# nebarnix/Project-Desert-Tortoise

Hardware: AMD Instinct MI355X
Metric: IQ Msamples/s end-to-end (WAV→minorframes), 1-GPU + %HBM roofline (higher is better)
Workload: dtype f32

## Files before the change

include/pdt_dev.h:

```cpp
#ifndef PDT_DEV_H
#define PDT_DEV_H
#include <stdint.h>
#ifdef __cplusplus
extern "C" {
#endif
int pdt_dev_set(const char *name, const char *value);
struct pdt_ctx;
unsigned long long pdt_dev_span_rows(const struct pdt_ctx *ctx, unsigned *n_exits_out, unsigned long long max);
int pdt_dev_ddc(int device, uint32_t in_rate, int decim, double offset_hz, int sample_format, const void *x_dev, long long lo, long long hi,
                uint64_t n_out, uint64_t g0, void *out_dev);
#ifdef __cplusplus
}
#endif
#endif
```

project-desert-tortoise_amd/__init__.py:

```python
from __future__ import annotations

import collections
import ctypes as C
import os
import struct

import numpy as np

_HERE = os.path.dirname(os.path.abspath(__file__))
LIBPDT_PATH = os.environ.get("PDT_LIBPDT_PATH") or os.path.join(_HERE, "csrc", "libpdt.so")
LIBSYNTH_PATH = os.path.join(_HERE, "synth", "libpdtsynth.so")

MODE_POES, MODE_ARGOS = 0, 1
SAMPLER_GARDNER, SAMPLER_MM = 0, 1
CHAIN_FILE, CHAIN_LIVE = 0, 1
ST_PLL, ST_LOCK, ST_FIR, ST_AGC, ST_SYM, ST_SYMIDX, ST_BITS, ST_BITSYM, ST_AGC_RAW, ST_ANALYTIC, ST_CHANNEL = range(11)
FMT_PCM16, FMT_F32, FMT_REAL_PCM16, FMT_REAL_F32 = range(4)


FMT_WB_PCM16, FMT_WB_F32, FMT_WB_CU8, FMT_WB_CS8 = range(16, 20)


class PdtError(RuntimeError):
    pass
# ... 247 lines not shown


def _argos_cfg(min_run, rule=None):
    if min_run is None and rule is None:
        return None
    c = ArgosCfg(rule=int(rule or 0))
    if min_run is not None:
        c.min_run, c.zero_mask = int(min_run), ARGOS_ZERO_MIN_RUN if int(min_run) == 0 else 0
    return c


def argos_run_len(msgs):
    return np.asarray(msgs["reserved_"]) & 0xFF


def argos_slip(msgs):
    return (np.asarray(msgs["reserved_"]) >> 8) & 1


def _bit_string(bits) -> np.ndarray:
    if isinstance(bits, (bytes, bytearray)):
        return np.frombuffer(bytes(bits), dtype=np.uint8)
    return np.ascontiguousarray(bits, dtype=np.uint8).reshape(-1)


def argos_msg_tile() -> int:
    return lib().pdt_argos_msg_tile()


def host_argos_messages(bits, min_run=None, cap: int = 4096, with_count: bool = False, rule=None):
    a, c = _bit_string(bits), _argos_cfg(min_run, rule)
    out, count = np.zeros(max(cap, 1), dtype=ARGOS_MSG_DTYPE), C.c_int(0)
    _check(lib().pdt_host_argos_messages(a.ctypes.data, a.size, C.byref(c) if c else None, out.ctypes.data, cap, C.byref(count)),
           "pdt_host_argos_messages")
    got = out[:min(count.value, cap)]
    return (got, count.value) if with_count else got


def argos_messages_batch(ds, min_run=None, cap: int = 4096, rule=None):
    c = _argos_cfg(min_run, rule)
    hs = (C.c_void_p * max(len(ds), 1))(*[d._h for d in ds])
    out, counts = np.zeros((max(len(ds), 1), max(cap, 1)), dtype=ARGOS_MSG_DTYPE), (C.c_int * max(len(ds), 1))()
    _check(lib().pdt_argos_messages_batch(hs, len(ds), C.byref(c) if c else None, out.ctypes.data, cap, counts),
           "pdt_argos_messages_batch")
    return [out[i, :min(counts[i], cap)].copy() for i in range(len(ds))]


class FfCfg(C.Structure):
    _fields_ = [("rate_steps", C.c_int32), ("zero_mask", C.c_uint32), ("rate_step_ppm", C.c_double), ("residual_hz", C.c_double),
                ("flags", C.c_uint32), ("reserved_", C.c_uint32)]


class FfSync(C.Structure):
    _fields_ = [("residual_hz", C.c_double), ("tone_valid", C.c_int32), ("step", C.c_uint32), ("tau", C.c_int32), ("rate", C.c_int32),
                ("period", C.c_int64), ("metric", C.c_uint64), ("nbits", C.c_uint64)]


FF_ZERO_RATE_STEPS, FF_RESIDUAL_GIVEN = 1, 1
FF_SYNC_DTYPE = np.dtype([("residual_hz", "<f8"), ("tone_valid", "<i4"), ("step", "<u4"), ("tau", "<i4"), ("rate", "<i4"), ("period", "<i8"),
                          ("metric", "<u8"), ("nbits", "<u8")])
assert FF_SYNC_DTYPE.itemsize == C.sizeof(FfSync) == 48 and C.sizeof(FfCfg) == 32
FfBits = collections.namedtuple("FfBits", "sync bits soft index")


def _ff_cfg(rate_steps=None, rate_step_ppm=None, residual_hz=None):
    if rate_steps is None and rate_step_ppm is None and residual_hz is None:
        return None
    c = FfCfg()
    if rate_steps is not None:
        c.rate_steps, c.zero_mask = int(rate_steps), FF_ZERO_RATE_STEPS if int(rate_steps) == 0 else 0
    if rate_step_ppm is not None:
        c.rate_step_ppm = float(rate_step_ppm)
    if residual_hz is not None:
        c.residual_hz, c.flags = float(residual_hz), FF_RESIDUAL_GIVEN
    return c


def ff_max_bits(rate: int, n: int) -> int:
    return min(n, 2 * rate) * 800 // (rate * 18 // 10) + 2 if rate >= 800 else 2


def host_ff_mix(rate: int, residual_hz: float, iq: np.ndarray) -> np.ndarray:
    a = np.ascontiguousarray(iq, dtype="<f4").reshape(-1)
    out = np.zeros(max(a.size, 2), dtype="<f4")
    _check(lib().pdt_host_ff_mix(rate, float(residual_hz), a.ctypes.data, a.size // 2, out.ctypes.data), "pdt_host_ff_mix")
    return out[:a.size // 2 * 2].reshape(-1, 2)


def host_ff_bits(rate: int, iq: np.ndarray, rate_steps=None, rate_step_ppm=None, residual_hz=None) -> FfBits:
    a = np.ascontiguousarray(iq, dtype="<f4").reshape(-1)
    c, n = _ff_cfg(rate_steps, rate_step_ppm, residual_hz), a.size // 2
    cap = ff_max_bits(rate, n)
    sync, count = np.zeros(1, dtype=FF_SYNC_DTYPE), C.c_uint64(0)
    bits, soft, index = np.zeros(cap, dtype=np.uint8), np.zeros(cap, dtype="<f4"), np.zeros(cap, dtype="<i8")
    _check(lib().pdt_host_ff_bits(rate, a.ctypes.data, n, C.byref(c) if c else None, sync.ctypes.data, bits.ctypes.data, soft.ctypes.data,
                                  index.ctypes.data, cap, C.byref(count)), "pdt_host_ff_bits")
    k = min(count.value, cap)
    return FfBits(sync[0], bits[:k], soft[:k], index[:k])


def ff_bits_batch(ds, rate_steps=None, rate_step_ppm=None, residual_hz=None) -> np.ndarray:
    c = _ff_cfg(rate_steps, rate_step_ppm, residual_hz)
    hs = (C.c_void_p * max(len(ds), 1))(*[d._h for d in ds])
    syncs = np.zeros(max(len(ds), 1), dtype=FF_SYNC_DTYPE)
    _check(lib().pdt_ff_bits_batch(hs, len(ds), C.byref(c) if c else None, syncs.ctypes.data), "pdt_ff_bits_batch")
    return syncs[:len(ds)]


def ff_messages_batch(ds, min_run=None, cap: int = 64, rule=None, rate_steps=None, rate_step_ppm=None, residual_hz=None, with_sync: bool = False):
    c, a = _ff_cfg(rate_steps, rate_step_ppm, residual_hz), _argos_cfg(min_run, rule)
    hs = (C.c_void_p * max(len(ds), 1))(*[d._h for d in ds])
    syncs = np.zeros(max(len(ds), 1), dtype=FF_SYNC_DTYPE)
    out, counts = np.zeros((max(len(ds), 1), max(cap, 1)), dtype=ARGOS_MSG_DTYPE), (C.c_int * max(len(ds), 1))()
    _check(lib().pdt_ff_messages_batch(hs, len(ds), C.byref(c) if c else None, C.byref(a) if a else None, syncs.ctypes.data, out.ctypes.data, cap,
                                       counts), "pdt_ff_messages_batch")
    got = [out[i, :min(counts[i], cap)].copy() for i in range(len(ds))]
    return (got, syncs[:len(ds)]) if with_sync else got


def format_argos_messages(msgs: np.ndarray) -> bytes:
    a = np.ascontiguousarray(msgs, dtype=ARGOS_MSG_DTYPE)
    L = lib()
    n = L.pdt_format_argos_messages(a.ctypes.data, len(a), None, 0)
    buf = C.create_string_buffer(n + 1)
    L.pdt_format_argos_messages(a.ctypes.data, len(a), buf, n)
    return buf.raw[:n]


def _carriers(rec, count: int):
    return [Carrier(rec[i].offset_hz, rec[i].peak_db, rec[i].floor_power) for i in range(count)]


ABI_SYMBOLS = [
    "pdt_abi_version", "pdt_build_tag", "pdt_strerror", "pdt_device_count", "pdt_open", "pdt_close", "pdt_set_stream",
    "pdt_demod_pcm16", "pdt_demod_device", "pdt_demod_f32", "pdt_demod_device_f32", "pdt_demod_batch_device", "pdt_num_frames", "pdt_frames", "pdt_get_stats",
    "pdt_format_frames", "pdt_read_stage", "pdt_stage_len", "pdt_kernel_times", "pdt_make_lpf",
    "pdt_wav_parse_header", "pdt_time_axis", "pdt_stage_bytesync", "pdt_tip_check", "pdt_tip_frames",
    "pdt_stream_begin", "pdt_stream_push_pcm16", "pdt_stream_push_f32", "pdt_stream_end", "pdt_stream_frames",
    "pdt_keep_quality", "pdt_chunk_reports", "pdt_stage_manchester", "pdt_stage_fir", "pdt_stage_agc", "pdt_stage_squelch", "pdt_stage_pll", "pdt_stage_gardner", "pdt_stage_static_gain", "pdt_stage_mm",
    "pdt_keep_presquelch", "pdt_keep_pll", "pdt_stage_bytesync_from", "pdt_demod_fd", "pdt_format_records", "pdt_stream_retained", "pdt_host_math", "pdt_get_device",
    "pdt_write_frames", "pdt_write_records", "pdt_demod_file", "pdt_set_loop_params", "pdt_set_progress",
    "pdt_set_real_input", "pdt_demod_real", "pdt_demod_device_real", "pdt_stream_push_real", "pdt_host_analytic",
    "pdt_set_channel", "pdt_demod_channel", "pdt_demod_device_channel", "pdt_demod_channels_device", "pdt_demod_channels", "pdt_stream_push_channel", "pdt_host_ddc",
    "pdt_survey", "pdt_survey_device", "pdt_survey_spectrum", "pdt_host_survey",
    "pdt_bursts", "pdt_bursts_device", "pdt_burst_carriers", "pdt_waterfall_rows", "pdt_bursts_shape", "pdt_burst_peaks", "pdt_host_bursts",
    "pdt_device_math", "pdt_device_math_layout",
    "pdt_burst_windows", "pdt_demod_windows_device", "pdt_demod_windows", "pdt_demod_windows_held",
    "pdt_tones", "pdt_tones_batch", "pdt_host_tones",
    "pdt_argos_messages", "pdt_argos_messages_batch", "pdt_stage_argos_messages", "pdt_host_argos_messages", "pdt_argos_msg_tile",
    "pdt_format_argos_messages", "pdt_write_argos_messages",
    "pdt_ff_bits", "pdt_ff_bits_batch", "pdt_ff_read", "pdt_ff_messages", "pdt_ff_messages_batch", "pdt_stage_ff_bits", "pdt_host_ff_bits",
    "pdt_host_ff_mix",
]
DEV_SYMBOLS = ["pdt_dev_set", "pdt_dev_span_rows", "pdt_dev_ddc"]

_lib = None


def _share_torch_hip_runtime():
    import importlib.util
    import sys
    if "torch" in sys.modules:
        return
    try:
        spec = importlib.util.find_spec("torch")
    except (ImportError, ValueError):
        return
    if spec is None or not spec.submodule_search_locations:
        return
    path = os.path.join(list(spec.submodule_search_locations)[0], "lib", "libamdhip64.so")
    if os.path.exists(path):
        try:
            C.CDLL(path, mode=C.RTLD_GLOBAL)
        except OSError:
            pass


def lib():
    global _lib
    if _lib is not None:
        return _lib
    if not os.path.exists(LIBPDT_PATH):
        raise PdtError(
            f"{LIBPDT_PATH} is missing: build it with `make` (hipcc --offload-arch=gfx950). "
            "There is no CPU implementation to fall back to."
        )
    _share_torch_hip_runtime()
    L = C.CDLL(LIBPDT_PATH)
    L.pdt_abi_version.restype = C.c_int
    L.pdt_build_tag.restype = C.c_char_p
    L.pdt_strerror.restype = C.c_char_p
    L.pdt_strerror.argtypes = [C.c_int]
    L.pdt_device_count.restype = C.c_int
    L.pdt_open.argtypes = [C.POINTER(Config), C.POINTER(C.c_void_p)]
    L.pdt_close.argtypes = [C.c_void_p]
    L.pdt_close.restype = None
    L.pdt_set_stream.argtypes = [C.c_void_p, C.c_void_p]
    L.pdt_demod_pcm16.argtypes = [C.c_void_p, C.c_void_p, C.c_uint64]
    L.pdt_demod_device.argtypes = [C.c_void_p, C.c_void_p, C.c_uint64]
    L.pdt_demod_f32.argtypes = [C.c_void_p, C.c_void_p, C.c_uint64]
    L.pdt_demod_device_f32.argtypes = [C.c_void_p, C.c_void_p, C.c_uint64]
    L.pdt_demod_fd.argtypes = [C.c_void_p, C.c_int, C.c_uint64, C.c_uint64, C.c_int]
    L.pdt_format_records.argtypes = [C.c_void_p, C.c_uint64, C.c_char_p, C.c_uint64]
    L.pdt_format_records.restype = C.c_uint64
    L.pdt_num_frames.argtypes = [C.c_void_p]
    L.pdt_num_frames.restype = C.c_uint64
    L.pdt_frames.argtypes = [C.c_void_p, C.POINTER(Frame), C.c_uint64]
    L.pdt_frames.restype = C.c_uint64
    L.pdt_get_stats.argtypes = [C.c_void_p, C.POINTER(Stats)]
    L.pdt_format_frames.argtypes = [C.c_void_p, C.c_char_p, C.c_uint64]
    L.pdt_format_frames.restype = C.c_uint64
    L.pdt_read_stage.argtypes = [C.c_void_p, C.c_int, C.c_uint64, C.c_uint64, C.c_void_p]
    L.pdt_read_stage.restype = C.c_int64
    L.pdt_stage_len.argtypes = [C.c_void_p, C.c_int]
    L.pdt_stage_len.restype = C.c_uint64
    L.pdt_kernel_times.argtypes = [C.c_void_p, C.POINTER(KernelTime), C.c_int]
    L.pdt_make_lpf.argtypes = [C.c_int, C.c_uint32, C.c_void_p, C.POINTER(C.c_int), C.POINTER(C.c_int)]
    L.pdt_wav_parse_header.argtypes = [C.c_char_p] + [C.POINTER(C.c_uint32)] * 5
    L.pdt_time_axis.argtypes = [C.c_int, C.c_uint32, C.c_uint64]
    L.pdt_time_axis.restype = C.c_double
    L.pdt_stage_bytesync.argtypes = [C.c_void_p, C.c_void_p, C.c_uint64]
    L.pdt_demod_batch_device.argtypes = [C.POINTER(C.c_void_p), C.POINTER(C.c_void_p), C.POINTER(C.c_uint64), C.c_int]
    L.pdt_stream_begin.argtypes = [C.c_void_p]
    L.pdt_stream_push_pcm16.argtypes = [C.c_void_p, C.c_void_p, C.c_uint64, C.POINTER(C.c_uint64)]
    L.pdt_stream_push_f32.argtypes = [C.c_void_p, C.c_void_p, C.c_uint64, C.POINTER(C.c_uint64)]
    L.pdt_stream_end.argtypes = [C.c_void_p, C.POINTER(C.c_uint64)]
    L.pdt_stream_frames.argtypes = [C.c_void_p, C.c_void_p, C.c_uint64]
    L.pdt_stream_frames.restype = C.c_uint64
    L.pdt_host_math.argtypes = [C.c_int, C.c_void_p, C.c_uint64, C.c_void_p, C.c_void_p]
    L.pdt_stream_retained.argtypes = [C.c_void_p]
    L.pdt_stream_retained.restype = C.c_uint64
    L.pdt_stage_manchester.argtypes = [C.c_void_p, C.c_void_p, C.c_uint64, C.c_double, C.c_void_p, C.c_void_p, C.c_void_p, C.c_void_p]
    L.pdt_stage_manchester.restype = C.c_int
    L.pdt_stage_pll.argtypes = [C.c_void_p, C.c_void_p, C.c_uint64, C.c_int, C.c_void_p, C.c_void_p, C.c_void_p, C.c_void_p]
    L.pdt_stage_pll.restype = C.c_int
    L.pdt_stage_gardner.argtypes = [C.c_void_p, C.c_void_p, C.c_uint64, C.c_uint64, C.c_void_p, C.c_void_p, C.c_void_p, C.c_void_p,
                                    C.c_void_p]
    L.pdt_stage_gardner.restype = C.c_int
    L.pdt_stage_static_gain.argtypes = [C.c_void_p, C.c_void_p, C.c_uint64, C.c_int, C.c_double, C.c_void_p]
    L.pdt_stage_static_gain.restype = C.c_int
    L.pdt_stage_mm.argtypes = [C.c_void_p, C.c_void_p, C.c_uint64, C.c_void_p, C.c_void_p, C.c_void_p, C.c_void_p]
    L.pdt_stage_mm.restype = C.c_int
    L.pdt_stage_agc.argtypes = [C.c_void_p, C.c_void_p, C.c_uint64, C.c_double, C.c_double, C.c_double, C.c_void_p]
    L.pdt_stage_agc.restype = C.c_int
    L.pdt_stage_squelch.argtypes = [C.c_void_p, C.c_void_p, C.c_void_p, C.c_uint64, C.c_double]
    L.pdt_stage_squelch.restype = C.c_int
    L.pdt_stage_fir.argtypes = [C.c_void_p, C.c_void_p, C.c_uint64, C.c_void_p, C.c_void_p]
    L.pdt_stage_fir.restype = C.c_int
    L.pdt_keep_quality.argtypes = [C.c_void_p, C.c_int]
    L.pdt_keep_quality.restype = C.c_int
    L.pdt_keep_pll.argtypes = [C.c_void_p, C.c_int]
    L.pdt_keep_pll.restype = C.c_int
    L.pdt_chunk_reports.argtypes = [C.c_void_p, C.c_void_p, C.c_uint64]
    L.pdt_chunk_reports.restype = C.c_uint64
    L.pdt_set_progress.argtypes = [C.c_void_p, C.c_void_p, C.c_void_p]
    L.pdt_tip_check.argtypes = [C.c_void_p, C.POINTER(TipSummary)]
    L.pdt_tip_frames.argtypes = [C.c_void_p, C.c_void_p, C.c_uint64]
    L.pdt_tip_frames.restype = C.c_uint64
    L.pdt_write_frames.argtypes = [C.c_void_p, C.c_int, C.POINTER(C.c_uint64)]
    L.pdt_write_records.argtypes = [C.c_void_p, C.c_uint64, C.c_int, C.POINTER(C.c_uint64)]
    L.pdt_dev_set.argtypes = [C.c_char_p, C.c_char_p]
    L.pdt_set_loop_params.argtypes = [C.c_void_p, C.POINTER(LoopParams)]
    L.pdt_demod_file.argtypes = [C.c_void_p, C.c_int, C.c_uint64, C.c_uint64, C.c_int, C.c_int, C.POINTER(C.c_uint64)]
    L.pdt_set_real_input.argtypes = [C.c_void_p, C.c_double]
    L.pdt_demod_real.argtypes = [C.c_void_p, C.c_void_p, C.c_uint64, C.c_int]
    L.pdt_demod_device_real.argtypes = [C.c_void_p, C.c_void_p, C.c_uint64, C.c_int]
    L.pdt_stream_push_real.argtypes = [C.c_void_p, C.c_void_p, C.c_uint64, C.c_int, C.POINTER(C.c_uint64)]
    L.pdt_host_analytic.argtypes = [C.c_uint32, C.c_double, C.c_void_p, C.c_uint64, C.c_int, C.c_void_p]
    L.pdt_set_channel.argtypes = [C.c_void_p, C.c_int, C.c_double]
    L.pdt_demod_channel.argtypes = [C.c_void_p, C.c_void_p, C.c_uint64, C.c_int]
    L.pdt_demod_device_channel.argtypes = [C.c_void_p, C.c_void_p, C.c_uint64, C.c_int]
    L.pdt_demod_channels_device.argtypes = [C.POINTER(C.c_void_p), C.c_int, C.c_void_p, C.c_uint64, C.c_int]
    L.pdt_demod_channels.argtypes = [C.POINTER(C.c_void_p), C.c_int, C.c_void_p, C.c_uint64, C.c_int]
    L.pdt_stream_push_channel.argtypes = [C.c_void_p, C.c_void_p, C.c_uint64, C.c_int, C.POINTER(C.c_uint64)]
    L.pdt_host_ddc.argtypes = [C.c_uint32, C.c_int, C.c_double, C.c_void_p, C.c_uint64, C.c_int, C.c_void_p]
    L.pdt_dev_ddc.argtypes = [C.c_int, C.c_uint32, C.c_int, C.c_double, C.c_int, C.c_void_p, C.c_longlong, C.c_longlong, C.c_uint64, C.c_uint64, C.c_void_p]
    L.pdt_survey.argtypes = [C.c_void_p, C.c_void_p, C.c_uint64, C.c_int, C.POINTER(SurveyCfg), C.POINTER(CarrierRec), C.c_int, C.POINTER(C.c_int)]
    L.pdt_survey_device.argtypes = L.pdt_survey.argtypes
    L.pdt_survey_spectrum.argtypes = [C.c_void_p, C.c_void_p, C.c_int]
    L.pdt_bursts.argtypes = [C.c_void_p, C.c_void_p, C.c_uint64, C.c_int, C.POINTER(BurstsCfg), C.POINTER(BurstRec), C.c_int, C.POINTER(C.c_int)]
    L.pdt_bursts_device.argtypes = L.pdt_bursts.argtypes
    L.pdt_burst_carriers.argtypes = [C.POINTER(BurstRec), C.c_int, C.c_double, C.POINTER(CarrierRec), C.c_int, C.POINTER(C.c_int)]
    L.pdt_waterfall_rows.argtypes = [C.c_void_p, C.c_uint64, C.c_uint64, C.c_void_p]
    L.pdt_bursts_shape.argtypes = [C.c_void_p, C.POINTER(C.c_int), C.POINTER(C.c_int), C.POINTER(C.c_uint64)]
    L.pdt_burst_peaks.argtypes = [C.c_void_p, C.c_uint64, C.c_uint64, C.c_void_p, C.c_void_p]
    L.pdt_host_bursts.argtypes = [C.c_uint32, C.c_double, C.c_uint32, C.c_int, C.c_void_p, C.c_uint64, C.POINTER(BurstsCfg), C.c_void_p, C.c_void_p,
                                  C.c_void_p, C.POINTER(BurstRec), C.c_int, C.POINTER(C.c_int)]
    L.pdt_host_survey.argtypes = [C.c_uint32, C.c_double, C.c_uint32, C.c_int, C.c_void_p, C.c_uint64, C.POINTER(SurveyCfg), C.c_void_p,
                                  C.POINTER(CarrierRec), C.c_int, C.POINTER(C.c_int)]
    L.pdt_burst_windows.argtypes = [C.POINTER(BurstRec), C.c_int, C.c_uint32, C.c_uint64, C.c_double, C.c_double, C.POINTER(WindowRec)]
    L.pdt_demod_windows_device.argtypes = [C.POINTER(C.c_void_p), C.c_int, C.POINTER(WindowRec), C.c_void_p, C.c_uint64, C.c_int]
    L.pdt_demod_windows.argtypes = L.pdt_demod_windows_device.argtypes
    L.pdt_demod_windows_held.argtypes = [C.c_void_p, C.POINTER(C.c_void_p), C.c_int, C.POINTER(WindowRec)]
    L.pdt_tones.argtypes = [C.c_void_p, C.POINTER(ToneCfg), C.c_void_p, C.c_int, C.POINTER(C.c_int)]
    L.pdt_tones_batch.argtypes = [C.POINTER(C.c_void_p), C.c_int, C.POINTER(ToneCfg), C.c_void_p, C.c_int, C.POINTER(C.c_int)]
    L.pdt_host_tones.argtypes = [C.c_uint32, C.c_double, C.c_void_p, C.c_uint64, C.POINTER(ToneCfg), C.c_void_p, C.c_int, C.POINTER(C.c_int)]
    L.pdt_argos_messages.argtypes = [C.c_void_p, C.POINTER(ArgosCfg), C.c_void_p, C.c_int, C.POINTER(C.c_int)]
    L.pdt_argos_messages_batch.argtypes = [C.POINTER(C.c_void_p), C.c_int, C.POINTER(ArgosCfg), C.c_void_p, C.c_int, C.POINTER(C.c_int)]
    L.pdt_stage_argos_messages.argtypes = [C.c_void_p, C.c_void_p, C.c_uint64, C.POINTER(ArgosCfg), C.c_void_p, C.c_int, C.POINTER(C.c_int)]
    L.pdt_host_argos_messages.argtypes = [C.c_void_p, C.c_uint64, C.POINTER(ArgosCfg), C.c_void_p, C.c_int, C.POINTER(C.c_int)]
    L.pdt_format_argos_messages.argtypes = [C.c_void_p, C.c_uint64, C.c_char_p, C.c_uint64]
    L.pdt_format_argos_messages.restype = C.c_uint64
    L.pdt_write_argos_messages.argtypes = [C.c_void_p, C.c_uint64, C.c_int, C.POINTER(C.c_uint64)]
    L.pdt_ff_bits.argtypes = [C.c_void_p, C.POINTER(FfCfg), C.c_void_p]
    L.pdt_ff_bits_batch.argtypes = [C.POINTER(C.c_void_p), C.c_int, C.POINTER(FfCfg), C.c_void_p]
    L.pdt_ff_read.argtypes = [C.c_void_p, C.c_void_p, C.c_void_p, C.c_void_p, C.c_void_p, C.c_uint64, C.POINTER(C.c_uint64)]
    L.pdt_ff_messages.argtypes = [C.c_void_p, C.POINTER(FfCfg), C.POINTER(ArgosCfg), C.c_void_p, C.c_void_p, C.c_int, C.POINTER(C.c_int)]
# ... 712 lines not shown
```

project-desert-tortoise_amd/csrc/pdt_api.hip:

```cpp
#include "pdt_rt.h"
#include "pdt_analytic.h"
#include "pdt_ddc.h"
#include "pdt_survey.h"
#include "pdt_bursts.h"
#include "pdt_tone.h"
#include "pdt_argos_msg.h"
#include "pdt_ff.h"

#include <sys/stat.h>

namespace pdtrt {
PDT_CHAIN_INSTANCES(extern, float)
PDT_CHAIN_INSTANCES(extern, double)
std::atomic<long long> g_alloc_ns{0};
hipError_t analytic_launch(hipStream_t st, int fmt, const void *x, long long lo, long long hi, unsigned long long n_out, unsigned long long g0,
                           uint32_t step, const float *tab_dev, void *out);
size_t survey_part_floats(uint64_t nseg, int nfft);
hipError_t survey_launch(hipStream_t st, int fmt, const void *x, uint64_t nseg, int nfft, const float *win, const float *tw, float *part, float *out);
int survey_plan(const pdt_survey_cfg *cfg, double mode_range_hz, double channel_rate, uint64_t nframes, int cap, pdt::SurveyPlan *p);
int survey_carriers(const float *P, const pdt::SurveyPlan &p, double in_rate, pdt_carrier *found);
hipError_t waterfall_launch(hipStream_t st, int fmt, const void *x, uint64_t nrows, int rows_per, int nfft, const float *win, const float *tw, float *rows);
hipError_t row_peaks_launch(hipStream_t st, const float *rows, uint64_t nrows, int nfft, float level, int gb, void *peaks, int *counts);
int bursts_plan(const pdt_bursts_cfg *cfg, double mode_range_hz, double channel_rate, double in_rate, uint64_t nframes, int cap, pdt::BurstPlan *p);
pdt::SurveyPlan bursts_survey_plan(const pdt::BurstPlan &p, const pdt_bursts_cfg *cfg, uint64_t nframes);
int bursts_link(const void *peaks, const int *counts, bool compact, const pdt::BurstPlan &p, double floor, double in_rate, pdt_burst *found, int cap);
hipError_t tones_launch(hipStream_t st, int nfft, const void *segs_dev, uint64_t nsegs, int lo, int hi, const float *win, const float *tw, void *out);
int tone_plan(const pdt_tone_cfg *cfg, double fs, double range_hz, uint64_t len, int cap, pdt::TonePlan *p);
void tone_sums(int nfft, double *sw, double *sw2);
void tones_derive(const void *raw, const pdt::TonePlan &p, double fs, double offset_hz, double sw, double sw2, pdt_tone *out);
hipError_t argos_msgs_launch(hipStream_t st, const void *table_dev, int nctx, long long tiles, int K, int rule, hipEvent_t mid);
int argos_min_run(const pdt_argos_cfg *cfg, int *K, int *rule);
hipError_t ff_launch(hipStream_t st, const void *table_dev, int nwin, long long mix_tiles, long long groups, const long long *periods_dev, int R,
                     int H, long long pmax, const float *tab_dev, void *metric_dev, size_t metric_bytes, void *syncs_dev, hipEvent_t *ev);
int ff_plan(const pdt_ff_cfg *cfg, uint32_t rate, int *H, int *R, double *ppm, int *given, double *residual);
long long ddc_windows_table(int decim, pdt::DdcWindow *win, int count, std::vector<unsigned char> &table);
hipError_t ddc_windows_launch(hipStream_t st, int fmt, int decim, const float *taps_dev, const float *tab_dev, const void *table_dev, int count,
                              long long tiles);
hipError_t ddc_launch(hipStream_t st, int fmt, int decim, const float *taps_dev, const float *tab_dev, pdt::DdcWindow w);
}

static std::mutex g_dev_mu;
static std::map<std::string, std::string> g_dev;
void Tuning::load()
{
    std::lock_guard<std::mutex> lock(g_dev_mu);
    if (g_dev.empty()) return;
    auto get = [&](const char *n) -> const char * { auto it = g_dev.find(n); return it == g_dev.end() ? nullptr : it->second.c_str(); };
    if (const char *e = get("PDT_PLL_WARM_SCALE")) pll_warm_scale = atof(e);
    if (const char *e = get("PDT_HEAD_TAUS")) head_taus = atof(e);
    if (const char *e = get("PDT_BAND_PAD")) band_pad = atof(e);
    if (const char *e = get("PDT_PLL_WARM_S")) pll_warm_s = atof(e);
    if (const char *e = get("PDT_AGC_WARM_S")) agc_warm_s = atof(e);
    if (const char *e = get("PDT_AGC_K")) agc_k = atof(e);
    if (const char *e = get("PDT_AGC_TPB")) agc_tpb = std::max(1, atoi(e));
    if (const char *e = get("PDT_PLL_BLOCK")) pll_block = atoi(e);
    if (const char *e = get("PDT_HBM_LIMIT_MB")) hbm_limit_mb = std::max(1ll, atoll(e));
    if (const char *e = get("PDT_BURST_SLAB_ROWS")) burst_slab_rows = std::max(1ll, atoll(e));
    if (const char *e = get("PDT_WINDOW_PIECE")) window_piece = std::max(1ll, atoll(e));
    if (const char *e = get("PDT_SCOUT_SYMS")) scout_syms = std::max(16, atoi(e));
    if (const char *e = get("PDT_FIR_WG_PER_CU")) fir_wg_per_cu = std::min(4096, std::max(1, atoi(e)));
    if (const char *e = get("PDT_INGEST_THREADS")) ingest_threads = std::min(128, std::max(1, atoi(e)));
    if (const char *e = get("PDT_INGEST_SPAN_MB")) ingest_span_mb = std::min(256, std::max(1, atoi(e)));
    if (const char *e = get("PDT_INGEST_STREAMS")) ingest_streams = std::min(4, std::max(1, atoi(e)));
    if (const char *e = get("PDT_INGEST_DIRECT")) ingest_direct = atoi(e) ? 1 : 0;
    if (const char *e = get("PDT_INGEST_NUMA")) ingest_numa = atoi(e) ? 1 : 0;
    if (const char *e = get("PDT_FIX_PASSES")) fix_passes = atoi(e);
    if (const char *e = get("PDT_GSEG")) gseg = std::min(64, std::max(2, atoi(e)));
    if (const char *e = get("PDT_GSPAN")) gspan = std::min(256, std::max(1, atoi(e)));
    if (const char *e = get("PDT_GSPAN_CAP")) gspan_cap = std::max(64, atoi(e));
    fir_generic = get("PDT_FIR_GENERIC") != nullptr;
    mix_unfused = get("PDT_MIX_UNFUSED") != nullptr;
    quality_inline = get("PDT_QUALITY_INLINE") != nullptr;
    gardner_nostride = get("PDT_GARDNER_NOSTRIDE") != nullptr;
    gemit_groups = get("PDT_GEMIT_GROUPS") != nullptr;
    agc_unfused = get("PDT_AGC_UNFUSED") != nullptr;
    manch_3pass = get("PDT_MANCH_3PASS") != nullptr;
    sync_serial = get("PDT_SYNC_SERIAL") != nullptr;
    agc_lanes = get("PDT_AGC_LANES") != nullptr;
    no_excl = get("PDT_NO_EXCL") != nullptr;
    gardner_onebuf = get("PDT_GARDNER_ONEBUF") != nullptr;
    gardner_noring = get("PDT_GARDNER_NORING") != nullptr;
    ema_noguess = get("PDT_EMA_NOGUESS") != nullptr;
    gardner_sequential = get("PDT_GARDNER_SEQUENTIAL") != nullptr;
    seg_sequential = get("PDT_SEG_SEQUENTIAL") != nullptr;
    overlap = get("PDT_NO_OVERLAP") == nullptr;
    if (const char *e = get("PDT_OVERLAP_SPLIT")) {
        int k = 0;
        for (const char *q = e; *q && k < 8; k++) {
            char *end = nullptr;
            overlap_split[k] = strtod(q, &end);
            if (end == q) break;
            q = (*end == ',') ? end + 1 : end;
        }
    }
    chain_one_range = get("PDT_CHAIN_ONE_RANGE") != nullptr;
    debug_overlap = get("PDT_DEBUG_OVERLAP") != nullptr;
    if (const char *e = get("PDT_OVERLAP_SEGMENTS")) overlap_segments = std::min(64, std::max(1, atoi(e)));
    if (const char *e = get("PDT_OVERLAP_MIN_MB")) overlap_min_mb = std::min(1 << 20, std::max(1, atoi(e)));
    debug_sync = get("PDT_DEBUG_SYNC") != nullptr;
    pll_noshort = get("PDT_PLL_NOSHORT") != nullptr;
    pll_nockpt = get("PDT_PLL_NOCKPT") != nullptr;
    pll_noconsensus = get("PDT_PLL_NOCONSENSUS") != nullptr;
    pll_notail = get("PDT_PLL_NOTAIL") != nullptr;
    seg_plain = get("PDT_SEG_PLAIN") != nullptr;
    sync_block = get("PDT_SYNC_BLOCK") != nullptr;
}

namespace pdtrt {

int execute_plans(pdt_ctx *const *ctxs, int M)
{
    pdt_ctx *L0 = ctxs[0];
    HIP_TRY(hipSetDevice(L0->cfg.device));
    const Plan &P0 = L0->plan;
    for (int m = 1; m < M; m++)
        if (!P0.same_shape(ctxs[m]->plan)) return PDT_ERR_STATE;
    const size_t per = P0.packs.size();
    const size_t total = per * (size_t)M;
    int rc;
    if ((rc = L0->packs_dev.ensure(total + 64))) return rc;
    if (total + 64 > L0->packs_pin_cap) {
        if (L0->packs_pin) (void)hipHostFree(L0->packs_pin);
        L0->packs_pin = nullptr;
        L0->packs_pin_cap = 0;
        const size_t want = 2 * total + 4096;
        if (timed_host_malloc((void **)&L0->packs_pin, want) != hipSuccess) { (void)hipGetLastError(); return PDT_ERR_NOMEM; }
        L0->packs_pin_cap = want;
    }
    unsigned char *pin = (unsigned char *)L0->packs_pin;
    for (const PlanOp &o : P0.ops) {
        if (o.op != OP_LAUNCH) continue;
        for (int m = 0; m < M; m++)
            memcpy(pin + (size_t)M * o.pack_off + (size_t)m * o.pack_size, ctxs[m]->plan.packs.data() + o.pack_off, o.pack_size);
    }
    hipStream_t st[2] = { L0->stream, L0->stream2 };
    if (total) HIP_TRY(hipMemcpyAsync(L0->packs_dev.p, pin, total, hipMemcpyHostToDevice, st[0]));
    Launcher T(L0);
    const unsigned char *dev = (const unsigned char *)L0->packs_dev.p;
    for (size_t i = 0; i < P0.ops.size(); i++) {
        const PlanOp &o = P0.ops[i];
        switch (o.op) {
        case OP_LAUNCH: {
            dim3 g = o.grid;
            for (int m = 1; m < M; m++) {
                const dim3 gm = ctxs[m]->plan.ops[i].grid;
                g.x = std::max(g.x, gm.x);
                g.y = std::max(g.y, gm.y);
            }
            g.z = (unsigned)M;
            o.go(g, o.block, o.shmem, st[o.side], dev + (size_t)M * o.pack_off);
            if (L0->tune.debug_sync) {
                const hipError_t e = hipStreamSynchronize(st[o.side]);
                fprintf(stderr, "libpdt: [%zu] %s grid (%u,%u,%u) block %u lds %zu: %s\n", i, o.name, g.x, g.y, g.z, o.block.x, o.shmem,
                        hipGetErrorString(e));
            }
            break;
        }
        case OP_MEMSET:
            for (int m = 0; m < M; m++) {
                const PlanOp &om = ctxs[m]->plan.ops[i];
                if (om.bytes) HIP_TRY(hipMemsetAsync(om.dst, om.value, om.bytes, st[om.side]));
            }
            T.gap();
            break;
        case OP_D2H:
        case OP_H2D:
            for (int m = 0; m < M; m++) {
                const PlanOp &om = ctxs[m]->plan.ops[i];
                if (om.bytes)
                    HIP_TRY(hipMemcpyAsync(om.dst, om.src, om.bytes, o.op == OP_D2H ? hipMemcpyDeviceToHost : hipMemcpyHostToDevice, st[0]));
            }
            T.gap();
            break;
        case OP_FORK:
            HIP_TRY(hipEventRecord(L0->ev_fork, st[0]));
            HIP_TRY(hipStreamWaitEvent(st[1], L0->ev_fork, 0));
            break;
        case OP_JOIN_RECORD: HIP_TRY(hipEventRecord(L0->ev_join, st[1])); break;
        case OP_JOIN_WAIT: HIP_TRY(hipStreamWaitEvent(st[0], L0->ev_join, 0)); break;
        case OP_TBEGIN: T.begin(o.name, st[o.side]); break;
        case OP_TEND: T.end(); break;
        case OP_TGAP: T.gap(); break;
        case OP_EV0: HIP_TRY(hipEventRecord(L0->ev0, st[0])); break;
        case OP_EV1: HIP_TRY(hipEventRecord(L0->ev1, st[0])); break;
        }
    }
    HIP_TRY(hipGetLastError());
    for (int m = 0; m < M; m++) ctxs[m]->leader = L0;
    return PDT_OK;
}

void launch_bytesync(pdt_ctx *ctx, Plan &PL, hipStream_t st, const SyncParams &SP, DevScalars *d_sc, long long bit_cap, uint32_t hit_cap,
                     uint32_t frame_cap, long long min_pos)
{
    unsigned char *d_bits = (unsigned char *)ctx->bits.p;
    unsigned *d_bitsym = (unsigned *)ctx->bitsym.p;
    long long *d_symidx = (long long *)ctx->symidx.p;
    unsigned *d_hits = (unsigned *)ctx->hits.p;
    FrameRec *d_frames = (FrameRec *)ctx->frames.p;
    const long long n_stiles = (bit_cap + 4095) / 4096;
    SyncTile *d_stiles = (SyncTile *)ctx->stiles.p;
    PDT_LAUNCH(256, k_sync_hits_tile, dim3((unsigned)n_stiles), dim3(256), 0, st, d_bits, &d_sc->nbits, SP, d_stiles,
                       &d_sc->sync_overflow, min_pos);
    unsigned *d_scr = (unsigned *)ctx->sync_scr.p;
    if (ctx->tune.sync_serial) {
        PDT_LAUNCH(PDT_SYNC_THREADS, k_sync_frames_tiles, dim3(1), dim3(PDT_SYNC_THREADS), 0, st, (const SyncTile *)d_stiles, &d_sc->nbits, SP, d_hits,
                           hit_cap, d_frames, &d_sc->nframes, frame_cap, &d_sc->sync_overflow, d_scr);
    } else {
        const unsigned n_batch = (unsigned)std::min<long long>(256, ((long long)hit_cap + PDT_SYNC_PB - 1) / PDT_SYNC_PB);
        PDT_LAUNCH(PDT_SYNC_THREADS, k_sync_dense, dim3(1), dim3(PDT_SYNC_THREADS), 0, st, (const SyncTile *)d_stiles, &d_sc->nbits, n_stiles,
                           hit_cap, &d_sc->sync_overflow, d_scr);
        PDT_LAUNCH(256, k_sync_gather, dim3((unsigned)std::min<long long>(1024, (n_stiles + 255) / 256)), dim3(256), 0, st,
                           (const SyncTile *)d_stiles, &d_sc->nbits, n_stiles, d_hits, hit_cap, &d_sc->sync_overflow, (const unsigned *)d_scr);
        PDT_LAUNCH(PDT_SYNC_PT, k_sync_links, dim3(n_batch), dim3(PDT_SYNC_PT), 0, st, SP, (const unsigned *)d_hits, &d_sc->sync_overflow, d_scr,
                           hit_cap);
        PDT_LAUNCH(PDT_SYNC_PT, k_sync_mark, dim3(n_batch), dim3(PDT_SYNC_PT), 0, st, SP, (const unsigned *)d_hits, d_frames, &d_sc->nframes,
                           frame_cap, &d_sc->sync_overflow, (const unsigned *)d_scr, hit_cap);
    }
    const long long grid = std::min<long long>(2048, (bit_cap + 255) / 256);
    PDT_LAUNCH(256, k_sync_hits, dim3((unsigned)grid), dim3(256), 0, st, d_bits, &d_sc->nbits, SP, d_hits, &d_sc->nhits, hit_cap,
                       &d_sc->sync_overflow, min_pos);
    PDT_LAUNCH(256, k_sync_frames, dim3(1), dim3(256), 0, st, d_hits, &d_sc->nhits, hit_cap, SP, d_frames, &d_sc->nframes,
                       frame_cap, &d_sc->sync_overflow);
    PDT_LAUNCH(128, k_frame_pack, dim3(std::min<uint32_t>(frame_cap, 16384)), dim3(128), 0, st, d_bits, &d_sc->nbits, d_bitsym, d_symidx, SP,
                       d_frames, &d_sc->nframes, frame_cap);
}

void chunk_reports_range(const pdt_ctx *ctx, uint64_t c0, uint64_t c1, uint64_t total, pdt_chunk_report *out, const pdt_frame *open_frame)
{
    const bool argos = ctx->cfg.mode == PDT_MODE_ARGOS;
    const uint64_t chunk = ctx->cfg.chunk;
    uint64_t sym_prev = c0 ? ctx->chunk_host[(size_t)c0 - 1].sym_upto : 0, bits_prev = c0 ? ctx->chunk_host[(size_t)c0 - 1].bits_upto : 0;
    size_t f = 0;
    if (c0) {
        size_t lo = 0, hi = ctx->frames_host.size();
        while (lo < hi) {
            const size_t mid = (lo + hi) / 2;
            if ((uint64_t)ctx->frames_host[mid].bit_index < bits_prev) lo = mid + 1; else hi = mid;
        }
        f = lo;
    }
    for (uint64_t c = c0; c < c1; c++) {
        const pdt::ChunkInfo &ci = ctx->chunk_host[(size_t)c];
        pdt_chunk_report &o = out[c - c0];
        memset(&o, 0, sizeof o);
        o.samples = std::min<uint64_t>(chunk, total - c * chunk);
        o.avg_phase = ci.avg_phase;
        o.symbols = ci.sym_upto - sym_prev;
        o.bits = ci.bits_upto - bits_prev;
        while (f < ctx->frames_host.size() && (uint64_t)ctx->frames_host[f].bit_index < ci.bits_upto) { o.frames++; f++; }
        if (open_frame && (uint64_t)open_frame->bit_index >= bits_prev && (uint64_t)open_frame->bit_index < ci.bits_upto) o.frames++;
        o.time0 = (argos && ctx->elem == 8) ? const_cast<pdt_ctx *>(ctx)->axis_d.at((uint64_t)ci.t0_src + 1)
                  : argos ? (double)const_cast<pdt_ctx *>(ctx)->axis_f.at((uint64_t)ci.t0_src + 1)
                          : (double)const_cast<pdt_ctx *>(ctx)->axis_f.at(c * chunk + 1);
        sym_prev = ci.sym_upto;
        bits_prev = ci.bits_upto;
    }
}


}

extern "C" {

int pdt_abi_version(void) { return PDT_ABI_VERSION; }
#ifndef PDT_BUILD_TAG
#define PDT_BUILD_TAG "untagged"
#endif
const char *pdt_build_tag(void) { return PDT_BUILD_TAG; }

int pdt_dev_set(const char *name, const char *value)
{
    try {
        std::lock_guard<std::mutex> lock(g_dev_mu);
        if (!name) g_dev.clear();
        else if (!value) g_dev.erase(name);
        else g_dev[name] = value;
    } catch (const std::exception &) { return PDT_ERR_NOMEM; }
    return PDT_OK;
}

unsigned long long pdt_dev_span_rows(const pdt_ctx *ctx, unsigned *n_exits_out, unsigned long long max)
{
    if (!ctx || ctx->gspan_nrows <= 0 || !ctx->gspan_rows.p) return 0;
    const unsigned long long n = (unsigned long long)ctx->gspan_nrows, m = std::min(n, max);
    if (n_exits_out && m) {
        std::vector<GardnerSpanRow> rows((size_t)m);
        if (hipSetDevice(ctx->cfg.device) != hipSuccess ||
            hipMemcpy(rows.data(), ctx->gspan_rows.p, (size_t)m * sizeof(GardnerSpanRow), hipMemcpyDeviceToHost) != hipSuccess) {
            (void)hipGetLastError();
            return 0;
        }
        for (size_t k = 0; k < (size_t)m; k++) n_exits_out[k] = rows[k].n;
    }
    return n;
}

int pdt_dev_ddc(int device, uint32_t in_rate, int decim, double offset_hz, int sample_format, const void *x_dev, long long lo, long long hi,
                uint64_t n_out, uint64_t g0, void *out_dev)
{
    if (in_rate == 0 || decim < DDC_MIN_DECIM || decim > DDC_MAX_DECIM || !ddc_fmt(sample_format) || !x_dev || !out_dev) return PDT_ERR_ARG;
    if (!(std::isfinite(offset_hz) && std::fabs(offset_hz) < 0.5 * (double)in_rate)) return PDT_ERR_ARG;
    HIP_TRY(hipSetDevice(device));
    const std::vector<float> taps = ddc_taps(decim);
    std::vector<float> tab(2 * AN_TAB);
    analytic_table(tab.data());
    DevBuf dtaps, dtab;
    auto run = [&]() -> int {
        int rc;
        if ((rc = dtaps.ensure(taps.size() * sizeof(float) + 16)) || (rc = dtab.ensure(tab.size() * sizeof(float) + 16))) return rc;
        HIP_TRY(hipMemcpy(dtaps.p, taps.data(), taps.size() * sizeof(float), hipMemcpyHostToDevice));
        HIP_TRY(hipMemcpy(dtab.p, tab.data(), tab.size() * sizeof(float), hipMemcpyHostToDevice));
        const DdcWindow r = { x_dev, out_dev, lo, hi, (long long)n_out, ddc_step((double)in_rate, offset_hz), (uint32_t)g0, 0 };
        HIP_TRY(ddc_launch(nullptr, sample_format, decim, (const float *)dtaps.p, (const float *)dtab.p, r));
        HIP_TRY(hipStreamSynchronize(nullptr));
        return PDT_OK;
    };
    const int rc = run();
    dtaps.release();
    dtab.release();
    return rc;
}

const char *pdt_strerror(int code)
{
    switch (code) {
    case PDT_OK: return "ok";
    case PDT_ERR_ARG: return "bad argument";
    case PDT_ERR_NOGPU: return "no usable HIP device / HIP runtime error";
    case PDT_ERR_NOMEM: return "out of device memory";
    case PDT_ERR_FORMAT: return "unsupported WAV format (need 16-bit PCM, 2 channels)";
    case PDT_ERR_RATE: return "sample rate too high: interpolation factor would be 0";
    case PDT_ERR_STATE: return "call sequence / internal capacity error";
    case PDT_ERR_IO: return "read error on the capture file";
    default: return "unknown error";
    }
}

int pdt_get_device(const pdt_ctx *ctx) { return ctx ? ctx->cfg.device : -1; }

int pdt_device_count(void)
{
    int n = 0;
    if (hipGetDeviceCount(&n) != hipSuccess) {
        (void)hipGetLastError();
        return 0;
    }
    return n;
}

int pdt_host_math(int fn, const double *x, uint64_t n, double *out0, double *out1)
{
    if (!x || !out0) return PDT_ERR_ARG;
    for (uint64_t i = 0; i < n; i++) {
        switch (fn) {
        case 0: { double sv, cv; sincos_glibc(x[i], sv, cv); out0[i] = sv; if (out1) out1[i] = cv; break; }
        case 1: out0[i] = sin_glibc(x[i]); break;
        case 2: out0[i] = cos_glibc(x[i]); break;
        case 3: { float sf, cf; sincosf_glibc((float)x[i], sf, cf); out0[i] = sf; if (out1) out1[i] = cf; break; }
        case 4: out0[i] = hypot_glibc(x[2 * i], x[2 * i + 1]); break;
        case 5: out0[i] = hypotf_glibc((float)x[2 * i], (float)x[2 * i + 1]); break;
        case 6: { float sf, cf; sincosf_flat((float)x[i], sf, cf); out0[i] = sf; if (out1) out1[i] = cf; break; }
        case 7: out0[i] = pll_wrap_error_f32((float)x[i]); break;
        case 8: out0[i] = pll_wrap_phase_f32((float)x[i]); break;
        case 9: { const float v = (float)x[i]; out0[i] = ((double)v > M_PI) ? (float)((double)v - 2 * M_PI) : ((double)v < -M_PI) ? (float)((double)v + 2 * M_PI) : v; break; }
        case 10: out0[i] = (x[i] > M_PI) ? x[i] - 2 * M_PI : (x[i] < -M_PI) ? x[i] + 2 * M_PI : x[i]; break;
        case 11: out0[i] = arctan2_ref((float)x[2 * i], (float)x[2 * i + 1]); break;
        case 12: out0[i] = arctan2_ref(x[2 * i], x[2 * i + 1]); break;
        case 13: out0[i] = q_rsqrt((float)x[i]); break;
        default: return PDT_ERR_ARG;
        }
    }
    return PDT_OK;
}

int pdt_make_lpf(int mode, uint32_t sample_rate, void *taps_out, int *ntaps, int *interp)
{
    if (!sample_rate) return PDT_ERR_ARG;
    if (mode == PDT_MODE_ARGOS) {
        if (ntaps) *ntaps = 50;
        if (interp) *interp = 1;
        if (taps_out) make_lpf<double>((double *)taps_out, 50, 700.0, (double)sample_rate, 1);
        return PDT_OK;
    }
    const int ip = poes_interp(sample_rate);
    if (ip < 1) return PDT_ERR_RATE;
    const int N = 26 * ip;
    if (ntaps) *ntaps = N;
    if (interp) *interp = ip;
    if (taps_out) {
        const float Fs = (float)sample_rate;
        make_lpf<float>((float *)taps_out, N, (float)11000.0, Fs * (float)ip, ip);
    }
    return PDT_OK;
}

int pdt_wav_parse_header(const uint8_t h[44], uint32_t *sample_rate, uint32_t *channels, uint32_t *bits_per_sample,
                         uint32_t *format, uint32_t *data_bytes)
{
    if (!h) return PDT_ERR_ARG;
    auto r32 = [&](int o) { return (uint32_t)h[o] | ((uint32_t)h[o + 1] << 8) | ((uint32_t)h[o + 2] << 16) | ((uint32_t)h[o + 3] << 24); };
    auto r16 = [&](int o) { return (uint32_t)h[o] | ((uint32_t)h[o + 1] << 8); };
    if (format) *format = r16(20);
    if (channels) *channels = r16(22);
    if (sample_rate) *sample_rate = r32(24);
    if (bits_per_sample) *bits_per_sample = r16(34);
    if (data_bytes) *data_bytes = r32(40);
    return PDT_OK;
}

double pdt_time_axis(int mode, uint32_t sample_rate, uint64_t m)
{
    if (mode == PDT_MODE_ARGOS) {
        TimeAxis<double> ax;
        ax.init(1.0 / (double)sample_rate);
        return ax.at(m);
    }
    TimeAxis<float> ax;
    ax.init((float)(1.0 / (double)(float)sample_rate));
    return (double)ax.at(m);
}

int pdt_open(const pdt_config *cfg, pdt_ctx **out)
{
    if (!cfg || !out) return PDT_ERR_ARG;
    if (cfg->mode != PDT_MODE_POES && cfg->mode != PDT_MODE_ARGOS) return PDT_ERR_ARG;
    if (!cfg->sample_rate) return PDT_ERR_ARG;
    if (cfg->chain != PDT_CHAIN_FILE && cfg->chain != PDT_CHAIN_LIVE) return PDT_ERR_ARG;
    int ndev = 0;
    if (hipGetDeviceCount(&ndev) != hipSuccess || ndev <= 0) {
        (void)hipGetLastError();
        fprintf(stderr, "libpdt: no HIP device available -- this library has no CPU path\n");
        return PDT_ERR_NOGPU;
    }
    if (cfg->device < 0 || cfg->device >= ndev) return PDT_ERR_ARG;
    HIP_TRY(hipSetDevice(cfg->device));
    pdt_ctx *ctx = new pdt_ctx();
    ctx->cfg = *cfg;
    ctx->tune.load();
    if (ctx->tune.pll_block && !ctx->cfg.pll_block) ctx->cfg.pll_block = (uint32_t)ctx->tune.pll_block;
    if (ctx->tune.pll_warm_s > 0 && !ctx->cfg.pll_warm) ctx->cfg.pll_warm = (uint32_t)(ctx->tune.pll_warm_s * cfg->sample_rate);
    if (ctx->tune.agc_warm_s > 0 && !ctx->cfg.agc_warm) ctx->cfg.agc_warm = (uint32_t)(ctx->tune.agc_warm_s * cfg->sample_rate);
    if (!ctx->cfg.chunk) ctx->cfg.chunk = (cfg->mode == PDT_MODE_ARGOS || cfg->chain == PDT_CHAIN_LIVE) ? 2400 : 10000;
    const bool argos_twin = cfg->mode == PDT_MODE_ARGOS && cfg->chain == PDT_CHAIN_LIVE;
    ctx->elem = (int)((cfg->mode == PDT_MODE_ARGOS && !argos_twin) ? sizeof(double) : sizeof(float));
    int nt = 0, ip = 0;
    int rc = pdt_make_lpf(cfg->mode, cfg->sample_rate, nullptr, &nt, &ip);
    if (rc) { pdt_close(ctx); return rc; }
    ctx->interp = (uint32_t)ip;
    ctx->ntaps = (uint32_t)nt;
    ctx->taps_host.resize((size_t)nt * ctx->elem);
    if (argos_twin)
        make_lpf<float>((float *)ctx->taps_host.data(), 50, (float)700, (float)cfg->sample_rate, 1);
    else
    pdt_make_lpf(cfg->mode, cfg->sample_rate, ctx->taps_host.data(), nullptr, nullptr);
    if ((rc = ctx->taps.ensure(ctx->taps_host.size()))) { pdt_close(ctx); return rc; }
    if (hipMemcpy(ctx->taps.p, ctx->taps_host.data(), ctx->taps_host.size(), hipMemcpyHostToDevice) != hipSuccess) {
        pdt_close(ctx);
        return PDT_ERR_NOGPU;
    }
    if (cfg->mode == PDT_MODE_POES && nt == 26 * ip) {
        const int K = 26, rs = ip;
        const int cs = (K * rs + 15) & ~15;
        std::vector<float> rot((size_t)K * cs, 0.0f);
        const float *h = (const float *)ctx->taps_host.data();
        for (int c = 0; c < K; c++)
            for (int t = 0; t < K; t++)
                for (int r = 0; r < ip; r++) rot[(size_t)c * cs + (size_t)t * rs + r] = h[nt - 1 - r - ((c - t + K) % K) * ip];
        if ((rc = ctx->taps_rot.ensure(rot.size() * sizeof(float)))) { pdt_close(ctx); return rc; }
        if (hipMemcpy(ctx->taps_rot.p, rot.data(), rot.size() * sizeof(float), hipMemcpyHostToDevice) != hipSuccess) {
            pdt_close(ctx);
            return PDT_ERR_NOGPU;
        }
    }
    std::thread side_stream_task;
    auto make_side_stream = [ctx]() {
        if (hipSetDevice(ctx->cfg.device) != hipSuccess) { (void)hipGetLastError(); return; }
        int least = 0, greatest = 0;
        (void)hipDeviceGetStreamPriorityRange(&least, &greatest);
        if (hipStreamCreateWithPriority(&ctx->stream2, hipStreamNonBlocking, greatest) != hipSuccess) {
            (void)hipGetLastError();
            if (hipStreamCreateWithFlags(&ctx->stream2, hipStreamNonBlocking) != hipSuccess) { (void)hipGetLastError(); ctx->stream2 = nullptr; }
        }
    };
    try { side_stream_task = std::thread(make_side_stream); } catch (const std::exception &) { make_side_stream(); }
    auto join_side = [&]() { if (side_stream_task.joinable()) side_stream_task.join(); };
    if (hipStreamCreate(&ctx->stream) != hipSuccess) { ctx->stream = nullptr; join_side(); pdt_close(ctx); return PDT_ERR_NOGPU; }
    ctx->own_stream = true;
    {
        void *small = nullptr;
        if (timed_host_malloc((void **)&small, sizeof(DevScalars) + 128 + 32768) != hipSuccess) { join_side(); pdt_close(ctx); return PDT_ERR_NOMEM; }
        ctx->pend_sc = (DevScalars *)small;
        ctx->pend_info = (unsigned char *)small + ((sizeof(DevScalars) + 15) & ~(size_t)15);
        ctx->seg_pin = ctx->pend_info + 128;
    }
    (void)hipEventCreate(&ctx->ev0);
    (void)hipEventCreate(&ctx->ev1);
    (void)hipEventCreateWithFlags(&ctx->ev_fork, hipEventDisableTiming);
    (void)hipEventCreateWithFlags(&ctx->ev_join, hipEventDisableTiming);
    join_side();
    if (!ctx->stream2) { pdt_close(ctx); return PDT_ERR_NOGPU; }
    memset(&ctx->stats, 0, sizeof ctx->stats);
    memset(ctx->stage_len, 0, sizeof ctx->stage_len);
    ctx->axis_f.init((float)(1.0 / (double)(float)cfg->sample_rate));
    if (argos_twin) ctx->axis_f.init(1 / (float)cfg->sample_rate);
    ctx->axis_d.init(1.0 / (double)cfg->sample_rate);
    ctx->counted = true;
    ingest_open_contexts().fetch_add(1);
    *out = ctx;
    return PDT_OK;
}

void pdt_close(pdt_ctx *ctx)
{
    if (!ctx) return;
    (void)hipSetDevice(ctx->cfg.device);
    DevBuf *bufs[] = { &ctx->pcm, &ctx->pll, &ctx->lock, &ctx->fir, &ctx->agc, &ctx->sym, &ctx->symidx, &ctx->bits, &ctx->bitsym,
                       &ctx->hits, &ctx->frames, &ctx->taps, &ctx->mag, &ctx->seams_pll, &ctx->seams_agc, &ctx->scal, &ctx->lockinfo,
                       &ctx->term, &ctx->seams_ema, &ctx->gtable, &ctx->gentries, &ctx->gcand,
                       &ctx->gmfirst, &ctx->stiles, &ctx->gsegmap, &ctx->gsegstart, &ctx->gbands, &ctx->gclist, &ctx->gspan_keys, &ctx->gspan_tails, &ctx->gspan_rows, &ctx->gspan_items, &ctx->gspan_ctl, &ctx->gspan_recs, &ctx->gcentries, &ctx->gflags, &ctx->agc_maps, &ctx->pll_head, &ctx->taps_rot, &ctx->pll_scratch, &ctx->tip, &ctx->stream_in, &ctx->sync_scr, &ctx->agc_raw, &ctx->agc_ckpt, &ctx->pll_ckpt, &ctx->packs_dev, &ctx->seg_dev, &ctx->lt_theta, &ctx->lt_phi,
                       &ctx->avgph, &ctx->term_ap, &ctx->seams_q, &ctx->chunkinfo, &ctx->an_tab, &ctx->analytic, &ctx->halo.buf[0], &ctx->halo.buf[1],
                       &ctx->ddc_taps, &ctx->channel, &ctx->survey_win, &ctx->survey_tw, &ctx->survey_part, &ctx->survey_out,
                       &ctx->bursts_rows, &ctx->bursts_peaks, &ctx->bursts_counts, &ctx->win_table, &ctx->tone_table, &ctx->tone_out,
                       &ctx->argos_work, &ctx->argos_bits, &ctx->ff_work, &ctx->ff_in, &ctx->ff_out };
    for (DevBuf *b : bufs) b->release();
    for (hipEvent_t e : ctx->event_pool) (void)hipEventDestroy(e);
    if (ctx->pinned) (void)hipHostFree(ctx->pinned);
    if (ctx->qual_pin) (void)hipHostFree(ctx->qual_pin);
    if (ctx->packs_pin) (void)hipHostFree(ctx->packs_pin);
    ctx->ingest.release();
    if (ctx->pend_sc) (void)hipHostFree(ctx->pend_sc);
    for (auto &t : ctx->timers) { if (!t.shared_a) (void)hipEventDestroy(t.a); (void)hipEventDestroy(t.b); }
    if (ctx->ev0) (void)hipEventDestroy(ctx->ev0);
    if (ctx->ev1) (void)hipEventDestroy(ctx->ev1);
    if (ctx->ev_fork) (void)hipEventDestroy(ctx->ev_fork);
    if (ctx->ev_join) (void)hipEventDestroy(ctx->ev_join);
    if (ctx->stream2) (void)hipStreamDestroy(ctx->stream2);
    if (ctx->own_stream && ctx->stream) (void)hipStreamDestroy(ctx->stream);
    if (ctx->counted) ingest_open_contexts().fetch_sub(1);
    delete ctx;
}

int pdt_set_stream(pdt_ctx *ctx, void *hip_stream)
{
    if (!ctx) return PDT_ERR_ARG;
    HIP_TRY(hipSetDevice(ctx->cfg.device));
    if (ctx->own_stream && ctx->stream) (void)hipStreamDestroy(ctx->stream);
    ctx->own_stream = false;
    ctx->stream = (hipStream_t)hip_stream;
    if (!hip_stream) {
        if (hipStreamCreate(&ctx->stream) != hipSuccess) return PDT_ERR_NOGPU;
        ctx->own_stream = true;
    }
    return PDT_OK;
}

int pdt_set_loop_params(pdt_ctx *ctx, const pdt_loop_params *p)
{
    if (!ctx || !p) return PDT_ERR_ARG;
    if (ctx->stream_open) return PDT_ERR_STATE;
    const double v[] = { p->pll_freq_range_hz, p->pll_lock_threshold, p->pll_lock_alpha, p->pll_loopbw_acq, p->pll_loopbw_track, p->agc_attack,
                         p->agc_decay, p->gardner_baud, p->gardner_step_range, p->gardner_kp, p->manchester_threshold };
    for (double x : v)
        if (!(x >= 0.0) || !std::isfinite(x)) return PDT_ERR_ARG;
    if (p->gardner_baud != 0 && (double)ctx->cfg.sample_rate * (double)ctx->interp / p->gardner_baud < 2.0) return PDT_ERR_ARG;
    if (p->pll_freq_range_hz != 0 && p->pll_freq_range_hz >= 0.5 * (double)ctx->cfg.sample_rate) return PDT_ERR_ARG;
    if ((float)p->gardner_step_range > 0.1f) return PDT_ERR_ARG;
    if (p->zero_mask & ~(uint32_t)(PDT_LP_ZERO_LOCK_THRESHOLD | PDT_LP_ZERO_GARDNER_KP | PDT_LP_ZERO_GARDNER_STEP_RANGE | PDT_LP_ZERO_MANCHESTER_THRESHOLD))
        return PDT_ERR_ARG;
    if (p->gardner_baud != 0 && !((double)ctx->cfg.sample_rate * (double)ctx->interp / p->gardner_baud <= 4096.0)) return PDT_ERR_ARG;
    ctx->lp = *p;
    ctx->gcand_key = -1;
    return PDT_OK;
}

int pdt_keep_quality(pdt_ctx *ctx, int enable)
{
    if (!ctx) return PDT_ERR_ARG;
    ctx->keep_quality = enable != 0;
    if (!enable) ctx->chunk_host.clear();
    return PDT_OK;
}

uint64_t pdt_chunk_reports(const pdt_ctx *ctx, pdt_chunk_report *out, uint64_t max_chunks)
{
    if (!ctx) return 0;
    const uint64_t nc = ctx->chunk_host.size();
    if (!out) return nc;
    const uint64_t m = std::min<uint64_t>(nc, max_chunks);
    chunk_reports_range(ctx, 0, m, ctx->report_samples, out, nullptr);
    return m;
}

int pdt_set_progress(pdt_ctx *ctx, pdt_progress_fn fn, void *user)
{
    if (!ctx) return PDT_ERR_ARG;
    ctx->progress_fn = fn;
    ctx->progress_user = user;
    return PDT_OK;
}

int pdt_keep_pll(pdt_ctx *ctx, int enable)
{
    if (!ctx) return PDT_ERR_ARG;
    ctx->keep_pll = enable != 0;
    ctx->keep_pll_asked = enable != 0;
    return PDT_OK;
}

int pdt_keep_presquelch(pdt_ctx *ctx, int enable)
{
    if (!ctx) return PDT_ERR_ARG;
    ctx->keep_agc_raw = enable != 0;
    if (!enable) ctx->stage_len[PDT_ST_AGC_RAW] = 0;
    return PDT_OK;
}

static int demod_common(pdt_ctx *ctx, uint64_t nframes, int phase = RUN_ALL)
{
    if (phase == RUN_ALL) ctx->batch_hint = 1;
    HIP_TRY(hipSetDevice(ctx->cfg.device));
    ctx->n_samples = nframes;
    ctx->n_out = nframes * ctx->interp;
    ctx->stage_len[PDT_ST_ANALYTIC] = ctx->analytic_len;
    ctx->analytic_len = 0;
    if (phase != RUN_FINISH) {
        ctx->stage_len[PDT_ST_CHANNEL] = ctx->channel_len;
        ctx->channel_len = 0;
    }
    if (ctx->elem == 8) return run_capture<double>(ctx, nframes, phase);
    return run_capture<float>(ctx, nframes, phase);
}

static int demod_overlapped(pdt_ctx *ctx, const IngestSrc &src, uint64_t nframes, const InFmt &f, int text_fd, uint64_t *text_bytes);
static int demod_windowed(pdt_ctx *ctx, const IngestSrc &src, uint64_t nframes, const InFmt &f, int text_fd, uint64_t *text_bytes, uint64_t piece);
static int demod_batch(pdt_ctx *const *ctxs, const void *const *iq_device, const uint64_t *nframes, int count, int fmt);
static uint64_t stream_history(const pdt_ctx *ctx);

static int table_upload(pdt_ctx *ctx, const std::vector<float> &host, DevBuf &buf, int key, int *slot)
{
    *slot = 0;
    const int rc = buf.ensure(host.size() * sizeof(float) + 16);
    if (rc) return rc;
    HIP_TRY(hipStreamSynchronize(ctx->stream));
    HIP_TRY(hipMemcpy(buf.p, host.data(), host.size() * sizeof(float), hipMemcpyHostToDevice));
    *slot = key;
    return PDT_OK;
}

static int real_table(pdt_ctx *ctx)
{
    if (ctx->an_tab_ready) return PDT_OK;
    std::vector<float> tab(2 * AN_TAB);
    analytic_table(tab.data());
    return table_upload(ctx, tab, ctx->an_tab, 1, &ctx->an_tab_ready);
}

static int channel_tables(pdt_ctx *ctx)
{
    const int rc = real_table(ctx);
    if (rc || ctx->ddc_taps_decim == ctx->ch_decim) return rc;
    return table_upload(ctx, ddc_taps(ctx->ch_decim), ctx->ddc_taps, ctx->ch_decim, &ctx->ddc_taps_decim);
}

static uint64_t channel_count(const pdt_ctx *ctx, uint64_t n) { return (n + (uint64_t)ctx->ch_decim - 1) / (uint64_t)ctx->ch_decim; }

static int channel_prepare(pdt_ctx *ctx, uint64_t n)
{
    const int rc = ctx->channel.ensure((size_t)channel_count(ctx, n) * 8 + 16);
    return rc ? rc : channel_tables(ctx);
}

static DdcWindow channel_record(const pdt_ctx *ctx, const void *x, long long lo, long long hi, uint64_t n_out, uint64_t g0, void *out)
// ... 2022 lines not shown
```

project-desert-tortoise_amd/csrc/pdt_chain.inc:

```
#include "pdt_rt.h"

namespace pdtrt {
PDT_WIDE_INSTANCES(extern, float)
PDT_WIDE_INSTANCES(extern, double)

template <typename T> int finish_capture(pdt_ctx *ctx, uint64_t n, const FinishArgs &FA)
{
    const bool argos = FA.argos, need_lock = FA.need_lock, fuse_mix = FA.fuse_mix;
    const long long N = FA.N, n_out = FA.n_out, chunk = FA.chunk, chunk_out = FA.chunk_out, first = FA.first, first_out = FA.first_out,
                    sym_cap = FA.sym_cap;
    const int interp = FA.interp, ntaps = FA.ntaps;
    const uint32_t hit_cap = FA.hit_cap, frame_cap = FA.frame_cap;
    const SyncParams &SP = FA.SP;
    const T Fs = (T)ctx->cfg.sample_rate;
    StreamCarry *seg = ctx->sc.active ? &ctx->sc : nullptr;
    FrameRec *d_frames = (FrameRec *)ctx->frames.p;
    (void)first_out;
    if (!ctx->pending || ctx->pend_n != n) return PDT_ERR_STATE;
    ctx->pending = false;
    pdt_ctx *lead = ctx->leader ? ctx->leader : ctx;
    if (seg && seg->in_place && !ctx->tune.sync_block) {
        for (;;) {
            const hipError_t e = hipEventQuery(lead->ev1);
            if (e == hipSuccess) break;
// ... 326 lines not shown
        if (rc) return rc;
        *ckpt = (T *)ctx->agc_ckpt.p;
    }
    PDT_LAUNCH(64, k_agc_block<T>, dim3((unsigned)((nb + 63) / 64)), dim3(64), 0, st, a_in, na, AP, d_norm, Ba, Wa, (const double *)d_guess, a_lock,
               a_out, (AgcSeam<T> *)ctx->seams_agc.p, agc_K, *ckpt);
    return PDT_OK;
}

template <typename T> void rec_agc_fix(pdt_ctx *ctx, Plan &PL, hipStream_t st, const T *a_in, long long na, const AgcParams<T> &AP, long long Ba,
                                       const T *a_lock, T *a_out, DevScalars *d_sc, T *ckpt)
{
    PDT_LAUNCH(1024, k_agc_scan<T>, dim3(1), dim3(1024), 0, st, na, Ba, (const AgcSeam<T> *)ctx->seams_agc.p, &d_sc->agc_first_bad);
    PDT_LAUNCH(64, k_agc_fix<T>, dim3(1), dim3(64), 0, st, a_in, na, AP, Ba, a_lock, a_out, (AgcSeam<T> *)ctx->seams_agc.p, d_sc->counters,
               (const long long *)&d_sc->agc_first_bad, ckpt);
}

template <typename T> void rec_mm(Plan &PL, hipStream_t st, const T *in, const MmParams<T> &MP, T *d_sym, long long *d_symidx, DevScalars *d_sc,
                                  long long sym_cap, const SamplerCarry<T> &carry_in, int have_carry, SamplerCarry<T> *carry_out)
{
    PDT_LAUNCH(PDT_GARDNER_THREADS, (k_mm<T, 8192, 1024>), dim3(1), dim3(PDT_GARDNER_THREADS), 0, st, in, MP, d_sym, d_symidx, &d_sc->nsym, sym_cap,
               carry_in, have_carry, carry_out);
}

template <typename T> void rec_gardner_walk(Plan &PL, hipStream_t st, const T *in, const T *lock, const GardnerParams<T> &GP, T *d_sym, long long *d_symidx,
                                            DevScalars *d_sc, long long sym_cap, const SamplerCarry<T> &carry_in, SamplerCarry<T> *carry_out)
{
    PDT_LAUNCH(256, (k_gardner<T, GardnerLds<T>::LEN, GardnerLds<T>::OUT>), dim3(1), dim3(256), 0, st, in, lock, GP, d_sym, d_symidx, &d_sc->nsym,
               sym_cap, (const GardnerEntry<T> *)nullptr, carry_in, carry_out, 0ll, 1, (const unsigned char *)nullptr);
}

template <typename T> void rec_manch_3pass(Plan &PL, hipStream_t st, const T *d_sym, DevScalars *d_sc, T thr, ManchTile *d_tiles, long long n_tiles,
                                           long long pad, unsigned clock0, unsigned long long bit0, unsigned *clock_out, unsigned char *d_bits,
                                           unsigned *d_bitsym, long long bit_cap)
{
    const unsigned long long *d_nsym = &d_sc->nsym;
    PDT_LAUNCH(PDT_TILE_THREADS, k_manch_tile<T>, dim3((unsigned)n_tiles), dim3(PDT_TILE_THREADS), 0, st, d_sym, d_nsym, thr, d_tiles, pad);
    PDT_LAUNCH(1024, k_manch_scan, dim3(1), dim3(1024), 0, st, d_tiles, d_nsym, &d_sc->nbits, pad, clock0, bit0, clock_out);
    PDT_LAUNCH(PDT_TILE_THREADS, k_manch_emit<T>, dim3((unsigned)n_tiles), dim3(PDT_TILE_THREADS), 0, st, d_sym, d_nsym, thr, d_tiles, d_bits, d_bitsym,
               bit_cap, pad);
}

template <typename T> struct Chain {
    pdt_ctx *ctx;
    uint64_t n;
    int phase;
    Plan &PL;
    PlanGroups L;
    Chain(pdt_ctx *c, uint64_t n_, int ph) : ctx(c), n(n_), phase(ph), PL(c->plan), L{c->plan, c->cfg.profile != 0} {}
    static long long round4(long long v) { return (v + 3) / 4 * 4; }

    bool argos = false;
    bool live = false;
    bool inject = false;
    bool need_lock = false;
    long long N = 0;
    int interp = 0;
    int ntaps = 0;
    long long n_out = 0;
    long long chunk = 0;
    long long chunk_out = 0;
    hipStream_t st = nullptr;
    StreamCarry *seg = nullptr;
    long long first = 0;
    long long first_out = 0;
    T Fs = 0;
    PllParams<T> PP{};
    AgcParams<T> AP{};
    T fsi = 0;
    GardnerParams<T> GP{};
    T baud = 0;
    bool argos_twin = false;
    T manch_thr = 0;
    SyncParams SP{};
    double fs_d = 0;
    long long Bp = 0;
    long long Wp = 0;
    long long Wacq = 0;
    long long Ba = 0;
    long long Wa = 0;
    bool seg_fast = false;
    bool fuse_mix = false;
    long long agc_tiles_per_block = 0;
    long long fused_tiles = 0;
    long long agc_maps_per_block = 0;
    double sym_rate = 0;
    double f_lim = 0;
    int lag = 0;
    long long nb_pll = 0;
    long long nb_agc = 0;
    double min_step = 0;
    long long n_chunks = 0;
    long long sym_cap = 0;
    long long bit_cap = 0;
    uint32_t hit_cap = 0;
    uint32_t frame_cap = 0;
    long long n_tiles = 0;
    long long n0 = 0;
    long long lt_tiles = 0;
    long long lt_elems = 0;
    bool quality = false;
    T avg_alpha = 0;
    long long tau_q = 0;
    long long Bq = 0;
    long long Wq = 0;
    long long nb_q = 0;
    double *d_q_zresp = nullptr;
    double *d_q_guess = nullptr;
    T *d_avgph = nullptr;
    bool ema_guess = false;
    long long We = 0;
    long long Be = 0;
    long long nb_ema = 0;
    double *d_ema_zresp = nullptr;
    double *d_ema_guess = nullptr;
    IqSrc d_pcm{};
    T *d_pll = nullptr;
    T *d_lock = nullptr;
    T *d_fir = nullptr;
    T *d_agc = nullptr;
    T *d_sym = nullptr;
    long long *d_symidx = nullptr;
    unsigned char *d_bits = nullptr;
    unsigned *d_bitsym = nullptr;
    ManchTile *d_tiles = nullptr;
    FrameRec *d_frames = nullptr;
    DevScalars *d_sc = nullptr;
    PllLockInfo<T> *d_info = nullptr;
    T *d_norm = nullptr;
    T *d_taps = nullptr;
    unsigned char *spin = nullptr;
    T *d_theta = nullptr;
    T *d_phi = nullptr;
    long long lt_groups = 0;
    long long grid_pll = 0;
    bool short_pays = false;
    int short_group = 0;
    T pll_consensus = 0;
    long long phase_groups = 0;
    double worst = 0;
    bool slow_wrap = false;
    T *d_ckpt = nullptr;
    PllPhaseHint *d_hint = nullptr;
    bool serial_excl = false;
    long long fix_regions = 0;
    long long fix_region_blocks = 0;
    bool quality_side = false;
    bool quality_term_fused = false;
    bool quality_after_fir = false;
    size_t ops_after_pll = 0;
    long long agc_last_block = 0;
    bool use_mm = false;
    bool use_table = false;
    GardnerDomain GD{};
    SamplerCarry<T> carry_in{};
    SegTail<T> *d_tail = nullptr;
    SamplerCarry<T> *d_carry_out = nullptr;
    long long sym_pad = 0;
    unsigned clock0 = 0;
    unsigned long long bit0 = 0;
    long long sync_min_pos = 0;

    int params()
    {
        int rc = PDT_OK;
        (void)rc;
        argos = ctx->cfg.mode == PDT_MODE_ARGOS;
        live = !argos && ctx->cfg.chain == PDT_CHAIN_LIVE;
        inject = ctx->inj.active && !ctx->sc.active;
        need_lock = argos || live || inject;
        N = (long long)n;
        interp = (int)ctx->interp;
        ntaps = (int)ctx->ntaps;
        n_out = N * interp;
        chunk = (long long)ctx->cfg.chunk;
        chunk_out = chunk * interp;
        st = ctx->stream;
        seg = ctx->sc.active ? &ctx->sc : nullptr;
        first = seg ? seg->first : 0;
        first_out = first * interp;

        Fs = (T)ctx->cfg.sample_rate;
        PP = make_pll_params<T>(ctx);
        if (inject) {
            PP.want_lock = 1;
            if (ctx->inj.started && !ctx->inj.locked) {
                PP.phase0 = (T)ctx->inj.phase; PP.freq0 = (T)ctx->inj.freq; PP.avg0 = (T)ctx->inj.avg; PP.locksig0 = (T)ctx->inj.locksig;
                PP.sweep0 = (T)ctx->inj.sweep; PP.i0 = 0;
            }
        }
        if (seg && first > 0 && !seg->locked) {
            PP.phase0 = (T)seg->phase; PP.freq0 = (T)seg->freq; PP.avg0 = (T)seg->avg; PP.locksig0 = (T)seg->locksig;
            PP.sweep0 = (T)seg->sweep; PP.i0 = first;
        }
        fsi = output_rate<T>(ctx);
        AP = make_agc_params<T>(ctx);
        AP.squelch = argos ? 1 : 0;
        AP.squelch_thr = (T)0.15;
        baud = sampler_baud<T>(ctx);
        GP = make_gardner_params<T>(ctx, n_out, chunk_out);
        if (argos && (size_t)chunk * sizeof(T) < 128 * 1024) {
            const unsigned long long req = (unsigned long long)sizeof(T) * (unsigned long long)chunk;
            const unsigned long long csz = (req + 8 + 15) & ~15ull;
            GP.argos_heap = 1;
            GP.argos_field_bits = csz | 1ull;
            GP.argos_even = (int)((csz - 8 - req) / sizeof(T));
        }
        argos_twin = argos && ctx->cfg.chain == PDT_CHAIN_LIVE;
        manch_thr = manchester_threshold<T>(ctx, argos, live);
        SP = make_sync_params(argos, argos_twin);

        return PDT_OK;
    }

    int geometry()
    {
        int rc = PDT_OK;
        (void)rc;
        fs_d = (double)ctx->cfg.sample_rate;
        Bp = ctx->cfg.pll_block ? ctx->cfg.pll_block : (long long)((argos ? 0.5 : 0.05) * fs_d);
        Wp = ctx->cfg.pll_warm ? ctx->cfg.pll_warm : (long long)((argos ? 2.0 : 0.3) * fs_d);
        if (!ctx->cfg.pll_warm && !argos) {
            const double tau = 2.0 / (double)PP.alpha_trk;
            const double nb = std::max(1.0, (double)N / (double)std::max<long long>(1, Bp));
            double w = 2.82 * tau * log(2000.0 * nb);
            w *= ctx->tune.pll_warm_scale;
            Wp = (long long)std::min(std::max(w, 0.15 * fs_d), 0.6 * fs_d);
        }
        Wacq = (long long)(0.02 * fs_d);
        agc_block_warm(ctx, &Ba, &Wa);
        if (argos && !ctx->cfg.agc_block && ctx->batch_hint >= 8) Ba = (long long)(1.0 * fs_d * interp);
        if (!ctx->cfg.pll_block) {
            const long long groups_max = ctx->batch_hint > 1 ? 240 : 150;
            const long long share = std::max<long long>(1, groups_max / std::max(1, ctx->batch_hint));
            const long long b_min = (N + share * 256 - 1) / (share * 256);
            Bp = std::max(Bp, b_min);
        }
        Bp = std::min<long long>(Bp, std::max<long long>(N, 1));
        Bp = std::max<long long>(64, (Bp + 63) / 64 * 64);
        seg_fast = seg && first_out % PDT_MF_RUN == 0 && first_out % 32 == 0 && !ctx->tune.seg_plain;
        fuse_mix = false;
        if constexpr (std::is_same<T, float>::value) {
            fuse_mix = !argos && !live && !inject && (!seg || seg_fast) && interp == 1 && ntaps == 26 && ctx->taps_rot.p && !ctx->tune.fir_generic &&
                       !ctx->tune.mix_unfused && N >= 832;
            if (fuse_mix && !ctx->cfg.pll_block) Bp = (Bp + 831) / 832 * 832;
            if (fuse_mix && Bp % 832 != 0) fuse_mix = false;
        }
        Ba = std::max<long long>(64, round4(Ba));
        agc_tiles_per_block = 0;
        fused_tiles = 0;
        agc_maps_per_block = 0;
        if (!argos && !ctx->cfg.agc_block && ntaps == 26 * interp && ctx->taps_rot.p && !ctx->tune.fir_generic &&
            !ctx->tune.agc_unfused && (!seg || (seg_fast && first_out % (64ll * 26 * interp) == 0) || (seg_fast && fuse_mix))) {
            const long long tile_out = 64ll * 26 * interp;
            agc_tiles_per_block = std::max<long long>(1, (Ba + tile_out / 2) / tile_out);
            {
                const long long tiles = (n_out - first_out + tile_out - 1) / tile_out;
                const long long one_round = (tiles + 500ll * 64 - 1) / (500ll * 64);
                if (ctx->batch_hint <= 1 && tiles / agc_tiles_per_block > 512ll * 64 && one_round <= 4 * agc_tiles_per_block)
                    agc_tiles_per_block = one_round;
            }
            if (ctx->tune.agc_tpb) agc_tiles_per_block = ctx->tune.agc_tpb;
            Ba = agc_tiles_per_block * tile_out;
        }
        Wp = round4(Wp);
        Wa = round4(Wa);
        Wacq = round4(Wacq);
        sym_rate = (double)baud;
        f_lim = (double)PP.max_freq * fs_d / (2.0 * M_PI);
        lag = (int)ceil(fs_d / sym_rate);
        lag = std::max(1, std::min(lag, (int)(fs_d / (2.2 * f_lim))));
        lag = std::min(lag, 64);
        nb_pll = N / Bp + 2;
        nb_agc = (n_out - first_out + Ba - 1) / Ba + 1;

        return PDT_OK;
    }

    int allocate()
    {
        int rc = PDT_OK;
        (void)rc;
        min_step = (double)GP.step - 0.25;
        if (ctx->cfg.sampler == PDT_SAMPLER_MM) {
            if ((rc = make_mm_params<T>(ctx, n_out, chunk_out, nullptr))) return rc;
            min_step = (double)(int)fsi / ((double)baud + mm_step_range(ctx)) * 0.999;
        }
        n_chunks = chunk_out > 0 ? (n_out + chunk_out - 1) / chunk_out : 0;
        sym_cap = (long long)((double)n_out / min_step) + n_chunks + 64 + (seg ? 2 * PDT_SEG_KEEP : 0);
        bit_cap = sym_cap;
        hit_cap = next_pow2((uint32_t)(bit_cap / 10 + 4096));
        frame_cap = (uint32_t)(bit_cap / SP.span + 16);
        n_tiles = (sym_cap + PDT_TILE - 1) / PDT_TILE;
        n0 = std::min<long long>(chunk, N);

        if (seg) {
            if ((rc = ctx->pll.ensure_keep((size_t)(N + 1) * sizeof(T), (size_t)first * sizeof(T)))) return rc;
            if (need_lock && (rc = ctx->lock.ensure_keep((size_t)(N + 1) * sizeof(T), (size_t)first * sizeof(T)))) return rc;
        }
        if ((rc = ctx->pll.ensure((size_t)(N + 1) * sizeof(T)))) return rc;
        if (need_lock && (rc = ctx->lock.ensure((size_t)(N + 1) * sizeof(T)))) return rc;
        lt_tiles = (N / Bp + 1 + 63) / 64;
        lt_elems = lt_tiles * 64 * Bp + 48 * 64 * (16 / (long long)sizeof(T)) + 64;
        if (seg) {
            if ((rc = ctx->agc.ensure_keep((size_t)(n_out + 1) * sizeof(T), (size_t)first_out * sizeof(T)))) return rc;
            if ((rc = ctx->lt_theta.ensure((size_t)(lt_elems + 1) * sizeof(T)))) return rc;
            if ((rc = ctx->lt_phi.ensure((size_t)(lt_elems + 1) * sizeof(T)))) return rc;
// ... 295 lines not shown
                quality_side = !inject && !ctx->tune.quality_inline;
                quality_term_fused = quality_side && fuse_mix && std::is_same<T, float>::value;
                }
            if (quality && !quality_term_fused) rec_quality_walkers(true);
            quality_after_fir = quality && quality_term_fused;
            if (live) {
                L.begin("squelch");
                rec_squelch<T>(PL, st, d_pll, d_lock, N, (T)0.05);
                L.end();
            }
        }

        return PDT_OK;
    }

    void rec_quality_walkers(bool term_here)
    {
        hipStream_t sq = quality_side ? ctx->stream2 : st;
        if (quality_side) PL.simple(OP_FORK);
        L.begin("quality", sq);
        T *d_tap = (T *)ctx->term_ap.p;
        if (term_here)
        PDT_LAUNCH(256, (k_pll_mix<T, false, true>), dim3((unsigned)lt_groups), dim3(256), 0, sq, d_pcm, d_phi, N, Bp, PP,
                           d_info, (T *)nullptr, d_tap);
        if (quality_side && term_here) PL.simple(OP_JOIN_RECORD);
        PDT_LAUNCH(64, k_lock_ema_zero_wave<T>, dim3((unsigned)nb_q), dim3(64), 0, sq, (const T *)d_tap, N,
                           avg_alpha, d_info, Bq, d_q_zresp);
        PDT_LAUNCH(1024, (k_lock_ema_guess<T, true>), dim3(1), dim3(1024), 0, sq, (const double *)d_q_zresp, N, avg_alpha, d_info, Bq,
                           pow(1.0 - (double)avg_alpha, (double)Bq), d_q_guess);
        PDT_LAUNCH(64, (k_lock_ema<T, true>), dim3((unsigned)((nb_q + 63) / 64)), dim3(64), 0, sq, (const T *)d_tap, N, avg_alpha,
                           d_info, Bq, Wq, d_avgph, (EmaSeam<T> *)ctx->seams_q.p, (const double *)d_q_guess, (long long)chunk);
        PDT_LAUNCH(64, k_lock_ema_fix<T>, dim3(1), dim3(64), 0, sq, (const T *)d_tap, N, avg_alpha, d_info,
                           Bq, d_avgph, (EmaSeam<T> *)ctx->seams_q.p, &d_sc->pad0_);
        L.end();
    }

    int rec_fir()
    {
        int rc = PDT_OK;
        (void)rc;
        if (n_out > 0) {
            L.begin(fuse_mix ? "mix_fir" : "fir");
            bool done = false;
            AgcMap *fir_tile_maps = nullptr;
            if (!argos && agc_tiles_per_block > 0) {
                const int K = ntaps / interp;
                const long long tiles_rt = (N + 64ll * K - 1) / (64ll * K);
                if ((rc = ctx->agc_maps.ensure((size_t)(tiles_rt + 1) * sizeof(AgcMap) + (size_t)(nb_agc + 2) * (sizeof(double) + sizeof(AgcMap))))) return rc;
                fir_tile_maps = (AgcMap *)ctx->agc_maps.p;
                fused_tiles = tiles_rt;
            }
            if constexpr (std::is_same<T, float>::value) if (fuse_mix) {
                const long long runs_nat = (N + PDT_MF_RUN - 1) / PDT_MF_RUN;
                AgcMap *run_maps = nullptr;
                if (agc_tiles_per_block > 0) {
                    if ((rc = ctx->agc_maps.ensure((size_t)(runs_nat + 1) * sizeof(AgcMap) + (size_t)(nb_agc + 2) * (sizeof(double) + sizeof(AgcMap))))) return rc;
                    run_maps = (AgcMap *)ctx->agc_maps.p;
                    fused_tiles = runs_nat;
                    agc_maps_per_block = agc_tiles_per_block * (64 * 26 / PDT_MF_RUN);
                }
                const unsigned mf_grid = (unsigned)(lt_tiles * (Bp / PDT_MF_RUN));
                float *mf_pll = (ctx->keep_pll || seg) ? (float *)d_pll : (float *)nullptr;
                const long long mf_pll_from = (seg && !ctx->keep_pll) ? std::max<long long>(0, N - 256) : 0ll;
#define PDT_MF_ARGS d_pcm, (const float *)d_phi, (const float *)d_pll, N, Bp, (const PllLockInfo<float> *)d_info, (const float *)ctx->taps_rot.p, (float *)d_fir, mf_pll, run_maps, (float)AP.decay
                if (quality_after_fir) {
                    float *d_tap = (float *)ctx->term_ap.p;
                    if (d_pcm.fmt == 0) PDT_LAUNCH(512, (k_mix_fir<26, 0, 8, true>), dim3(mf_grid), dim3(512), 0, st, PDT_MF_ARGS, d_tap, mf_pll_from);
                    else PDT_LAUNCH(512, (k_mix_fir<26, 1, 8, true>), dim3(mf_grid), dim3(512), 0, st, PDT_MF_ARGS, d_tap, mf_pll_from);
                } else {
                    if (d_pcm.fmt == 0) PDT_LAUNCH(512, (k_mix_fir<26, 0, 8>), dim3(mf_grid), dim3(512), 0, st, PDT_MF_ARGS, (float *)nullptr, mf_pll_from);
                    else PDT_LAUNCH(512, (k_mix_fir<26, 1, 8>), dim3(mf_grid), dim3(512), 0, st, PDT_MF_ARGS, (float *)nullptr, mf_pll_from);
                }
#undef PDT_MF_ARGS
                done = true;
            }
            if (!done) done = rec_fir_unfused<T>(ctx, PL, st, (const T *)d_pll, N, d_fir, fir_tile_maps, AP.decay);
            if (!done) fused_tiles = 0;
            L.end();
        }

        return PDT_OK;
    }

    int rec_agc()
    {
        int rc = PDT_OK;
        (void)rc;
        agc_last_block = -1;
        if (n_out - first_out > 0) {
            const long long na = n_out - first_out;
            const T *a_in = d_fir + first_out;
            T *a_out = d_agc + first_out;
            const T *a_lock = d_lock ? d_lock + first_out : nullptr;
            AgcParams<T> APs = AP;
            if (APs.raw_out) APs.raw_out += first_out;
            const long long nb = (na + Ba - 1) / Ba;
            agc_last_block = nb - 1;
            const bool fused = fused_tiles > 0;
            if (!fused && (rc = ctx->agc_maps.ensure((size_t)(nb + 1) * (sizeof(AgcMap) + sizeof(double))))) return rc;
            AgcMap *d_maps = (AgcMap *)ctx->agc_maps.p;
            double *d_guess = (double *)(d_maps + (fused ? fused_tiles : nb) + 1);
            const long long map_len_fused = fuse_mix ? (long long)PDT_MF_RUN : 64ll * 26 * interp;
            const long long map_first = fused ? first_out / map_len_fused : 0;
            const AgcMap *d_maps_in = d_maps + map_first;
            const long long n_maps_in = fused ? fused_tiles - map_first : nb;
            if (quality_side && !quality_term_fused) PL.simple(OP_JOIN_WAIT);
            L.begin("agc_block");
            if (agc_maps_per_block == 0) agc_maps_per_block = agc_tiles_per_block;
            if (fused && agc_maps_per_block > 1) {
                AgcMap *d_bmaps = (AgcMap *)(d_guess + nb + 1);
                PDT_LAUNCH(256, k_agc_blockmaps, dim3((unsigned)((nb + 255) / 256)), dim3(256), 0, st, d_maps_in, nb,
                                   (int)agc_maps_per_block, n_maps_in, d_bmaps);
                PDT_LAUNCH(1024, k_agc_guess<T>, dim3(1), dim3(1024), 0, st, (const AgcMap *)d_bmaps, nb, (const T *)d_norm, d_guess, 1, nb);
            } else if (fused)
                PDT_LAUNCH(1024, k_agc_guess<T>, dim3(1), dim3(1024), 0, st, d_maps_in, nb, (const T *)d_norm, d_guess, (int)agc_maps_per_block, n_maps_in);
            bool agc_tr = false;
            float *agc_ckpt = nullptr;
            if constexpr (std::is_same<T, float>::value) {
                agc_tr = fused && !ctx->tune.agc_lanes && !APs.squelch && !APs.raw_out && first_out % 32 == 0 && Ba % 32 == 0 &&
                         agc_maps_per_block > 0 && Ba % agc_maps_per_block == 0;
                if (agc_tr) {
                    const long long tile_len = 64ll * 26 * interp;
                    const long long map_len = Ba / agc_maps_per_block;
                    agc_tr = tile_len % 32 == 0 && tile_len % map_len == 0 && Ba % tile_len == 0;
                    if (agc_tr) {
                        const double agc_K = ctx->tune.agc_k > 0 ? ctx->tune.agc_k : 12.0;
                        const size_t ck_bytes = (size_t)(nb + 64) * (size_t)(Ba / PDT_AGC_CKPT + 1) * sizeof(float);
                        if ((rc = ctx->agc_ckpt.ensure(ck_bytes))) return rc;
                        agc_ckpt = (float *)ctx->agc_ckpt.p;
                        PDT_LAUNCH(64, (k_agc_block_tr<PDT_AGC_TR_R>), dim3((unsigned)((nb + 63) / 64)), dim3(64), 0, st, (const float *)a_in, na, APs,
                                   (const float *)d_norm, Ba, Wa, (const double *)d_guess, d_maps_in, (int)agc_maps_per_block,
                                   (int)(tile_len / map_len), n_maps_in, tile_len, (float *)a_out, (AgcSeam<float> *)ctx->seams_agc.p, agc_K, agc_ckpt);
                    }
                }
            }
            T *agc_ckpt_any = (T *)agc_ckpt;
            if (!agc_tr && (rc = rec_agc_lanes<T>(ctx, PL, st, a_in, na, APs, d_norm, Ba, Wa, !fused, d_maps, d_guess, a_lock, a_out, &agc_ckpt_any))) return rc;
            L.end();
            L.begin("agc_fix");
            rec_agc_fix<T>(ctx, PL, st, a_in, na, APs, Ba, a_lock, a_out, d_sc, agc_ckpt_any);
            L.end();
        }

        return PDT_OK;
    }

    int sampler_domain()
    {
        int rc = PDT_OK;
        (void)rc;
        use_mm = ctx->cfg.sampler == PDT_SAMPLER_MM;
        use_table = false;
        GD.q_min = 0; GD.u = 0; GD.n_q = 0; GD.n_cand = 0; GD.pad_q = 0; GD.idx_bits = 20; GD.span = 1;
        if constexpr (std::is_same<T, float>::value) {
            const int table_len = 1 << 22;
            const float nT = (float)chunk_out, stepf = (float)GP.step;
            const long long seg_c_first = (seg && chunk > 0) ? first / chunk : 0;
            if (!argos && !use_mm && !ctx->tune.gardner_sequential && n_chunks - seg_c_first >= 4 && chunk_out >= 256 &&
                !(seg && ctx->tune.seg_sequential) &&
                chunk_out + 2 * (long long)stepf + 24 <= table_len && 8 * (long long)stepf + 256 < PDT_GTAB_WIN && chunk_out < (1 << 22)) {
                int e;
                (void)frexpf(nT - stepf - 1.0f, &e);
                const float u = ldexpf(1.0f, e - 24);
                const float q_min = u * floorf((nT - stepf - 1.0f) / u);
                const int n_q = (int)ceilf((stepf + 1.8f) / u);
                const float q_max = q_min + (float)n_q * u;
                const double max_count = (double)chunk_out / ((double)stepf - 0.11) + 2.0;
                int idx_bits = 1;
                while ((1ll << idx_bits) < 2 * (long long)n_q) idx_bits++;
                if (q_min >= ldexpf(1.0f, e - 1) && q_max < ldexpf(1.0f, e) && idx_bits <= 20 &&
                    max_count < (double)((1u << (32 - idx_bits)) - 2u) && max_count < 65000.0) {
                    use_table = true;
                    GD.q_min = q_min;
                    GD.u = u;
                    GD.n_q = n_q;
                    GD.idx_bits = idx_bits;
                    const double pad = ctx->cfg.gardner_band_pad > 0 ? ctx->cfg.gardner_band_pad : (ctx->tune.band_pad > 0 ? ctx->tune.band_pad : 1.0 / 8.0);
                    GD.pad_q = std::max(2, (int)(pad / (double)u));
                    const int span_fit = (int)std::min(16.0, std::max(2.0, std::round(std::sqrt(138000.0 / ((double)chunk_out / (double)stepf)))));
                    int span = ctx->tune.gspan > 0 ? ctx->tune.gspan : ((n_chunks - seg_c_first >= 4096 && (!seg || seg_fast)) ? span_fit : 1);
                    if (2 * n_q > 32 * PDT_GSPAN_BITMAP_WORDS || 8 * (long long)stepf + 256 >= PDT_GSUB_WIN) span = 1;
                    while (span > 1 && ((double)span * max_count >= (double)((1u << (32 - idx_bits)) - 2u) || (n_chunks - 1) / span - seg_c_first / span < 4))
                        span /= 2;
                    auto row_aligned = [&](int sp) { return !seg || seg_c_first % sp == 0; };
                    if (span >= 3 && !ctx->tune.gspan) {
                        int best = span;
                        long long best_left = row_aligned(span) ? n_chunks - ((n_chunks - 1) / span) * span : (1ll << 62);
                        for (int sp = span - std::max(1, span / 4); sp <= span + std::max(1, span / 4); sp++) {
                            const long long left = n_chunks - ((n_chunks - 1) / sp) * sp;
                            if (left < best_left && row_aligned(sp) && (double)sp * max_count < (double)((1u << (32 - idx_bits)) - 2u)) { best = sp; best_left = left; }
                        }
                        span = best;
                    }
                    if (!row_aligned(span)) span = 1;
                    GD.span = span;
                }
            }
        }
        return PDT_OK;
    }

    int sampler_carry()
    {
        int rc = PDT_OK;
        (void)rc;
        ctx->gardner_mode = use_table ? 1 : 0;
        ctx->gspan_nrows = (use_table && GD.span > 1 && chunk_out > 0) ? (n_out + chunk_out - 1) / chunk_out > 0 ? ((n_out + chunk_out - 1) / chunk_out - 1) / GD.span : 0 : 0;
        carry_in.a = 0; carry_in.b = 0; carry_in.c = 0; carry_in.c_first = 0; carry_in.count0 = 0;
        d_tail = seg ? (SegTail<T> *)ctx->seg_dev.p : nullptr;
        d_carry_out = seg ? &d_tail->sampler : nullptr;
        sym_pad = 0;
        clock0 = 0;
        bit0 = 0;
        sync_min_pos = 0;
        if (seg) {
            sym_pad = 2 + (long long)(seg->nsym_total & 1u);
            carry_in.c_first = chunk > 0 ? first / chunk : 0;
            carry_in.count0 = sym_pad;
            if (seg->have_sampler) { carry_in.a = (T)seg->sa; carry_in.b = (T)seg->sb; carry_in.c = (T)seg->sc; }
            T hist[4] = { 0, 0, 0, 0 };
            hist[sym_pad - 2] = (T)seg->sym_m2;
            hist[sym_pad - 1] = (T)seg->sym_m1;
            memcpy(spin + 256, hist, sizeof hist);
            PL.copy(OP_H2D, d_sym, spin + 256, (size_t)sym_pad * sizeof(T));
            if (quality) PL.memset_async(d_symidx, 0, (size_t)sym_pad * sizeof(long long));
            clock0 = seg->clockmod;
            bit0 = seg->kept_bits.size();
            if (bit0) {
                memcpy(spin + 512, seg->kept_bits.data(), (size_t)bit0);
                PL.copy(OP_H2D, d_bits, spin + 512, (size_t)bit0);
                PL.memset_async(d_bitsym, 0, (size_t)bit0 * sizeof(unsigned));
            }
            sync_min_pos = std::max<long long>(0, seg->next_free - (long long)seg->bit_base);
            if (seg->bit_base > 0) sync_min_pos = std::max<long long>(sync_min_pos, (long long)SP.len - 1);
        }
        return PDT_OK;
    }

    int rec_sampler_table()
    {
        int rc = PDT_OK;
        (void)rc;
        if constexpr (std::is_same<T, float>::value) {
            std::vector<unsigned> cand;
            std::vector<int> mfirst((size_t)GD.n_q + 1);
            cand.reserve((size_t)GD.n_q * 2);
            for (int m = 0; m < GD.n_q; m++) {
                mfirst[(size_t)m] = (int)cand.size();
                const float q = GD.q_min + (float)m * GD.u;
                const float fr = q - floorf(q);
                if (fr <= 0.61f) cand.push_back((unsigned)(2 * m));
                if (fr >= 0.39f) cand.push_back((unsigned)(2 * m + 1));
            }
            mfirst[(size_t)GD.n_q] = (int)cand.size();
            GD.n_cand = (int)cand.size();
            const long long key = chunk_out * 1000003ll + (long long)llround((double)GP.step * 4096.0);
            if ((rc = ctx->gcand.ensure(cand.size() * sizeof(unsigned)))) return rc;
            if ((rc = ctx->gmfirst.ensure(mfirst.size() * sizeof(int)))) return rc;
            if (ctx->gcand_key != key) {
                HIP_TRY(hipMemcpyAsync(ctx->gcand.p, cand.data(), cand.size() * sizeof(unsigned), hipMemcpyHostToDevice, st));
                HIP_TRY(hipMemcpyAsync(ctx->gmfirst.p, mfirst.data(), mfirst.size() * sizeof(int), hipMemcpyHostToDevice, st));
                HIP_TRY(hipStreamSynchronize(st));
                ctx->gcand_key = key;
            }
            const long long n_tab = (n_chunks - 1) / GD.span;
            const long long n_groups = n_tab + 1;
            SamplerCarry<float> tab_carry;
            tab_carry.a = (float)carry_in.a; tab_carry.b = (float)carry_in.b; tab_carry.c = (float)carry_in.c;
            tab_carry.c_first = carry_in.c_first; tab_carry.count0 = carry_in.count0;
            SamplerCarry<float> chain_carry = tab_carry;
            chain_carry.c_first = tab_carry.c_first / GD.span;
            const long long g_first = chain_carry.c_first;
            if ((rc = ctx->gtable.ensure((size_t)n_tab * (size_t)(2 * GD.n_q) * sizeof(unsigned)))) return rc;
            if ((rc = ctx->gentries.ensure((size_t)n_chunks * sizeof(GardnerEntry<float>)))) return rc;
            if ((rc = ctx->gbands.ensure((size_t)n_tab * sizeof(GardnerBand)))) return rc;
            L.begin("gardner_table");
            if ((rc = ctx->gclist.ensure((size_t)n_tab * PDT_GTAB_LIST * sizeof(unsigned)))) return rc;
            const int scout_syms = ctx->tune.scout_syms > 0 ? ctx->tune.scout_syms : 455;
            const int scout_tail = (int)std::min<long long>(PDT_GTAB_TAIL, std::max<long long>(256, (long long)((double)scout_syms * (double)GP.step) + 16));
            PDT_LAUNCH(64, k_gardner_scout, dim3((unsigned)n_tab), dim3(64), 0, st, (const float *)d_agc, GP, GD, n_tab,
                               (const int *)ctx->gmfirst.p, (const unsigned *)ctx->gcand.p, (unsigned *)ctx->gtable.p,
                               (GardnerBand *)ctx->gbands.p, (unsigned *)ctx->gclist.p, d_sc->gstats, scout_tail);
            {
                {
                    const unsigned parts = (unsigned)((GD.n_cand + PDT_GTM_SLOTS - 1) / PDT_GTM_SLOTS);
                    PDT_LAUNCH(PDT_GTM_THREADS, (k_gardner_table_merge<PDT_GTAB_WIN>), dim3((unsigned)n_tab, parts), dim3(PDT_GTM_THREADS), 0, st,
                                       (const float *)d_agc, GP, GD, n_tab, (const unsigned *)ctx->gcand.p,
                                       (const GardnerBand *)ctx->gbands.p, (const unsigned *)ctx->gclist.p,
                                       (unsigned *)ctx->gtable.p, d_sc->gstats);
                }
                if (GD.span > 1) {
                    const unsigned cap_keys = ctx->tune.gspan_cap ? (unsigned)ctx->tune.gspan_cap
                                                                  : (unsigned)std::min<long long>(std::max<long long>(n_tab * 128, 1ll << 20), 1ll << 28);
                    const size_t cap_items = (size_t)cap_keys / PDT_GSUB_KEYS + (size_t)n_tab + 1;
                    if ((rc = ctx->gspan_keys.ensure((size_t)cap_keys * sizeof(unsigned)))) return rc;
                    if ((rc = ctx->gspan_tails.ensure((size_t)cap_keys * sizeof(unsigned)))) return rc;
                    if ((rc = ctx->gspan_recs.ensure((size_t)cap_keys * (size_t)(GD.span - 1) * sizeof(GardnerSpanRec)))) return rc;
                    if ((rc = ctx->gspan_rows.ensure((size_t)n_tab * sizeof(GardnerSpanRow)))) return rc;
                    if ((rc = ctx->gspan_items.ensure(cap_items * sizeof(GardnerSpanItem)))) return rc;
                    if ((rc = ctx->gspan_ctl.ensure(sizeof(GardnerSpanCtl)))) return rc;
                    PL.memset_async(ctx->gspan_ctl.p, 0, sizeof(GardnerSpanCtl));
                    PDT_LAUNCH(256, k_gardner_span_keys, dim3((unsigned)n_tab), dim3(256), 0, st, GD, n_tab, (const unsigned *)ctx->gcand.p,
                                       (GardnerBand *)ctx->gbands.p, (const unsigned *)ctx->gclist.p, (const unsigned *)ctx->gtable.p,
                                       (unsigned *)ctx->gspan_keys.p, cap_keys, (GardnerSpanRow *)ctx->gspan_rows.p,
                                       (GardnerSpanItem *)ctx->gspan_items.p, (GardnerSpanCtl *)ctx->gspan_ctl.p);
                    const unsigned walkers = (unsigned)std::min<long long>(n_tab / PDT_GSUB + 64, 256ll * 16);
                    PDT_LAUNCH(64, (k_gardner_span_walk<PDT_GSUB_WIN>), dim3(walkers), dim3(64), 0, st, (const float *)d_agc, GP, GD,
                                       (const unsigned *)ctx->gspan_keys.p, (const GardnerSpanItem *)ctx->gspan_items.p,
                                       (GardnerSpanCtl *)ctx->gspan_ctl.p, (unsigned *)ctx->gspan_tails.p, (GardnerSpanRec *)ctx->gspan_recs.p);
                    PDT_LAUNCH(128, k_gardner_span_join, dim3((unsigned)n_tab), dim3(128), 0, st, GD, n_tab, (const unsigned *)ctx->gcand.p,
                                       (const GardnerBand *)ctx->gbands.p, (const unsigned *)ctx->gclist.p, (unsigned *)ctx->gtable.p,
                                       (const unsigned *)ctx->gspan_keys.p, (const unsigned *)ctx->gspan_tails.p,
                                       (const GardnerSpanRow *)ctx->gspan_rows.p, d_sc->gstats);
                }
            }
            L.end();
            int G = (n_groups < 8000) ? 32 : 64;
            if (ctx->tune.gseg) G = ctx->tune.gseg;
            const long long n_seg = (n_groups + G - 1) / G;
            if ((rc = ctx->gsegmap.ensure((size_t)n_seg * (size_t)(2 * GD.n_q) * sizeof(GardnerSegCell)))) return rc;
            if ((rc = ctx->gsegstart.ensure((size_t)n_seg * sizeof(GardnerSegStart)))) return rc;
            L.begin("gardner_chain");
            PL.memset_async(ctx->gsegstart.p, 0, (size_t)n_seg * sizeof(GardnerSegStart));
            PDT_LAUNCH(1024, k_gardner_segmap, dim3((unsigned)n_seg), dim3(1024), 0, st, (const unsigned *)ctx->gtable.p, GD, n_groups,
                               G, (GardnerSegCell *)ctx->gsegmap.p, (const GardnerBand *)ctx->gbands.p);
            const int n_ranges = (!seg && n_groups >= 8192 && GD.span == 1 && !ctx->tune.chain_one_range) ? 4 : 1;
            if ((rc = ctx->gchain.ensure(sizeof(GardnerChainState)))) return rc;
            const bool side = n_ranges > 1;
            hipStream_t st_emit = side ? ctx->stream2 : st;
            L.end();
            long long c_lo = 0;
            for (int r = 0; r < n_ranges; r++) {
                const long long c_hi = (r == n_ranges - 1) ? n_groups : (n_groups * (r + 1) / n_ranges) / G * G;
                L.begin("gardner_chain");
                PDT_LAUNCH(256, k_gardner_chain, dim3(1), dim3(256), 0, st,
                                   (const float *)d_agc, GP, GD, n_groups,
                                   (const unsigned *)ctx->gtable.p, (const GardnerSegCell *)ctx->gsegmap.p, G,
                                   (GardnerSegStart *)ctx->gsegstart.p, (GardnerEntry<float> *)ctx->gentries.p, d_sc->gstats,
                                   (const GardnerBand *)ctx->gbands.p, n_tab, chain_carry, (seg && seg->have_sampler) ? 1 : 0, c_hi,
                                   (GardnerChainState *)ctx->gchain.p, r == 0 ? 1 : 0,
                                   (const unsigned *)(GD.span > 1 ? ctx->gspan_keys.p : nullptr), (const unsigned *)(GD.span > 1 ? ctx->gspan_tails.p : nullptr),
                                   (const GardnerSpanRow *)(GD.span > 1 ? ctx->gspan_rows.p : nullptr));
                L.end();
                if (side) PL.simple(OP_FORK);
                const long long s_lo = c_lo / G, s_hi = (c_hi + G - 1) / G;
                L.begin("gardner", st_emit);
                if (s_hi > s_lo)
                    PDT_LAUNCH(64, k_gardner_segfill, dim3((unsigned)(s_hi - s_lo)), dim3(64), 0, st_emit, (const float *)d_agc, GP, GD, n_groups,
                                       (const unsigned *)ctx->gtable.p, G, (const GardnerSegStart *)ctx->gsegstart.p,
                                       (GardnerEntry<float> *)ctx->gentries.p, s_lo);
                const unsigned char *d_flags = nullptr;
                if (GD.span > 1 && 8 * (long long)GP.step + 256 < PDT_GEMIT_SUB_WIN && !ctx->tune.gemit_groups &&
                    (double)PDT_GEMIT_SUB_WIN / ((double)GP.step - 0.2) + 2.0 < (double)PDT_GSUB_OUT) {
                    if ((rc = ctx->gcentries.ensure((size_t)n_chunks * sizeof(GardnerEntry<float>)))) return rc;
                    if ((rc = ctx->gflags.ensure((size_t)n_groups + 64))) return rc;
                    PL.memset_async(ctx->gflags.p, 1, (size_t)n_groups, PL.side_of(st_emit));
                    PDT_LAUNCH(64, (k_gardner_emit_first<PDT_GEMIT_SUB_WIN>), dim3((unsigned)((n_tab - g_first + 3) / 4)), dim3(64), 0, st_emit, (const float *)d_agc, GP, GD,
                                       n_tab, (const GardnerEntry<float> *)ctx->gentries.p, (const unsigned *)ctx->gspan_keys.p,
                                       (const GardnerSpanRow *)ctx->gspan_rows.p, (const GardnerSpanRec *)ctx->gspan_recs.p,
                                       (GardnerEntry<float> *)ctx->gcentries.p, (unsigned char *)ctx->gflags.p, (float *)d_sym, d_symidx, sym_cap, g_first);
                    PDT_LAUNCH(64, (k_gardner_emit_rest<PDT_GEMIT_SUB_WIN>), dim3((unsigned)(((n_tab - g_first) * (GD.span - 1) + 3) / 4)), dim3(64), 0, st_emit,
                                       (const float *)d_agc, GP, GD, n_tab, (const GardnerEntry<float> *)ctx->gcentries.p,
                                       (const unsigned char *)ctx->gflags.p, (float *)d_sym, d_symidx, sym_cap, g_first);
                    d_flags = (const unsigned char *)ctx->gflags.p;
                }
                if (c_hi > c_lo)
                    PDT_LAUNCH(256, (k_gardner<float, PDT_GEMIT_LEN, PDT_GEMIT_OUT>), dim3((unsigned)(c_hi - c_lo)), dim3(PDT_GARDNER_THREADS), 0, st_emit,
                                       (const float *)d_agc, (const float *)d_lock, GP, (float *)d_sym, d_symidx, &d_sc->nsym, sym_cap,
                                       (const GardnerEntry<float> *)ctx->gentries.p, tab_carry, (SamplerCarry<float> *)d_carry_out, c_lo, GD.span, d_flags);
                L.end();
                c_lo = c_hi;
            }
            if (side) {
                PL.simple(OP_JOIN_RECORD);
                PL.simple(OP_JOIN_WAIT);
            }
        }
        return PDT_OK;
    }

    int rec_sampler()
    {
        int rc = PDT_OK;
        (void)rc;
        if (use_table) {
            if ((rc = rec_sampler_table())) return rc;
        } else if (use_mm) {
            MmParams<T> MP;
            if ((rc = make_mm_params<T>(ctx, n_out, chunk_out, &MP))) return rc;
            L.begin("gardner");
            if (seg && !seg->have_sampler) carry_in.b = MP.step0;
            rec_mm<T>(PL, st, d_agc, MP, d_sym, d_symidx, d_sc, sym_cap, carry_in, seg ? 1 : 0, d_carry_out);
            L.end();
        } else {
            L.begin("gardner");
            constexpr int SMALL_LEN = 32768 / (int)sizeof(T), SMALL_OUT = 1024;
            const long long small_need = chunk_out + 2 * (long long)GP.step + 24;
            const double small_syms = (double)chunk_out / ((double)GP.step - 0.25) + 4.0;
            constexpr int RING_LEN = 20480 / (int)sizeof(T), RING_NB = 6, RING_OUT = 256;
            if (small_need <= RING_LEN && small_syms < RING_OUT && chunk_out >= 4 * (long long)GP.step + 8 && n_chunks >= 8 && !seg &&
                !ctx->tune.gardner_onebuf && !ctx->tune.gardner_noring) {
                const size_t need_bytes = ((size_t)n_chunks + 64 + 15) & ~(size_t)15;
                if ((rc = ctx->gneed.ensure(need_bytes + (size_t)n_chunks * sizeof(CalmEntry<T>)))) return rc;
                CalmEntry<T> *d_calm = (CalmEntry<T> *)((char *)ctx->gneed.p + need_bytes);
                PDT_LAUNCH(256, k_chunk_need<T>, dim3((unsigned)n_chunks), dim3(256), 0, st, (const T *)d_agc, n_out, chunk_out, n_chunks,
                                   (unsigned char *)ctx->gneed.p);
                T gran_scale = 0;
                if (!ctx->tune.gardner_nostride) {
                    const double top = (double)chunk_out + 2.0 * (double)GP.step + 2.0;
                    const int E = ilogb(top) + 1, p = sizeof(T) == 8 ? 53 : 24;
                    const T sc = (T)ldexp(1.0, p - E);
                    const T gstep = GP.step * sc;
                    if (E < p && gstep == (T)rint((double)gstep) && (double)gstep < ldexp(1.0, p - 1)) gran_scale = sc;
                }
                PDT_LAUNCH(64 * (RING_NB + 1), (k_gardner_ring<T, RING_LEN, RING_NB, RING_OUT>), dim3(1), dim3(64 * (RING_NB + 1)), 0, st,
                                   (const T *)d_agc, (const T *)d_lock, GP, (const unsigned char *)ctx->gneed.p, d_sym, d_symidx, &d_sc->nsym,
                                   sym_cap, d_calm, gran_scale);
                PDT_LAUNCH(256, k_calm_emit<T>, dim3((unsigned)((n_chunks + 255) / 256)), dim3(256), 0, st, (const unsigned char *)ctx->gneed.p,
                                   (const CalmEntry<T> *)d_calm, GP, d_sym, d_symidx, sym_cap);
            } else if (small_need <= SMALL_LEN && small_syms < SMALL_OUT && !ctx->tune.gardner_onebuf && !seg)
                PDT_LAUNCH(256, (k_gardner_small<T, SMALL_LEN, SMALL_OUT>), dim3(1), dim3(256), 0, st, (const T *)d_agc, (const T *)d_lock, GP,
                                   d_sym, d_symidx, &d_sc->nsym, sym_cap);
            else
                rec_gardner_walk<T>(PL, st, d_agc, d_lock, GP, d_sym, d_symidx, d_sc, sym_cap, carry_in, d_carry_out);
            L.end();
        }

        return PDT_OK;
    }

    int rec_bits()
    {
        int rc = PDT_OK;
        (void)rc;
        L.begin("manchester");
        if (ctx->tune.manch_3pass) {
            rec_manch_3pass<T>(PL, st, d_sym, d_sc, manch_thr, d_tiles, n_tiles, sym_pad, clock0, bit0, seg ? &d_tail->clock : (unsigned *)nullptr,
                               d_bits, d_bitsym, bit_cap);
        } else {
            constexpr int ONE_NT = ManchOnePass<T>::NT, ONE_TILE = ManchOnePass<T>::TILE;
            const long long n_one = (sym_cap + ONE_TILE - 1) / ONE_TILE;
            unsigned long long *d_mstat = (unsigned long long *)d_tiles;
            PL.memset_async(d_mstat, 0, (size_t)(n_one + 1) * sizeof(unsigned long long), PL.side_of(st));
            PDT_LAUNCH(ONE_NT, k_manch_onepass<T>, dim3((unsigned)n_one), dim3(ONE_NT), 0, st, d_sym, &d_sc->nsym,
                               manch_thr, d_mstat, d_bits, d_bitsym, bit_cap, sym_pad, clock0, bit0, &d_sc->nbits,
                               seg ? &d_tail->clock : (unsigned *)nullptr, sym_cap);
        }
        L.end();

        L.begin("bytesync");
        launch_bytesync(ctx, PL, st, SP, d_sc, bit_cap, hit_cap, frame_cap, sync_min_pos);
        L.end();
        if (seg) {
            const long long last_pll = (N > 0) ? (N - 1) / Bp : -1;
            PDT_LAUNCH(256, (k_seg_tail<T, PllSeam<T>, AgcSeam<T>>), dim3(1), dim3(256), 0, st, (const PllSeam<T> *)ctx->seams_pll.p, last_pll,
                       (const T *)d_lock, N, (const AgcSeam<T> *)ctx->seams_agc.p, agc_last_block, (const T *)d_sym, &d_sc->nsym,
                       (const unsigned char *)d_bits, (const unsigned *)d_bitsym, (const long long *)d_symidx, &d_sc->nbits,
                       (long long)bit0, d_tail);
            PL.copy(OP_D2H, spin + 4096, d_tail, sizeof(SegTail<T>));
        }
        ctx->pend_chunks = 0;
        if (inject) {
// ... 417 lines not shown
```

project-desert-tortoise_amd/csrc/pdt_kernels_back.h:

```cpp
#pragma once
#include "pdt_device_math.h"

namespace pdt {

template <typename T> struct alignas(16) Vec16 {
    static constexpr int N = 16 / sizeof(T);
    T v[N];
};

template <typename T> struct GardnerParams {
    T step, kp, lim;
    long long n_total;
    long long chunk_out;
    int argos_heap;
    unsigned long long argos_field_bits;
    int argos_even;
};

template <typename T>
__device__ __forceinline__ T gardner_beyond(const T *__restrict__ in, const T *__restrict__ lock, const GardnerParams<T> &P,
                                            long long c, long long n_cur, long long idx)
{
    const long long C = P.chunk_out;
    if (idx < C)
// ... 1067 lines not shown
#pragma unroll
                for (int l = 0; l < 2; l++) {
                    const float rn = __builtin_rintf(L[l].ns);
                    if (rn < nT) {
                        const unsigned i_cur = (unsigned)rn;
                        const unsigned i_half = (unsigned)__builtin_rintf(L[l].half);
                        const float cur = win[i_cur];
                        float mid;
                        if (i_half < (unsigned)WIN) mid = win[i_half];
                        else mid = (i_half < (unsigned)n_cur) ? in[base + i_half]
                                                              : gardner_beyond(in, (const float *)nullptr, P, c, (long long)n_cur, (long long)i_half);
                        const float err = __builtin_amdgcn_fmed3f(kp * (cur - L[l].prev) * mid, -lim, lim);
                        L[l].ns = L[l].ns - err;
                        L[l].q_last = L[l].ns;
                        L[l].half = L[l].ns + hs;
                        L[l].ns = L[l].ns + step;
                        L[l].prev = cur;
                        L[l].i_last = i_cur;
                        L[l].count = 1;
                    }
                }
            }
            if (L[0].count >= 1 && L[1].count >= 1) {
                int k_min = (int)((stop - 4.0f - enter_hi) / (step + 0.101f)) - 1;
                if (k_min < 0) k_min = 0;
                if (two) {
                    for (int it = 0; it < k_min; it++) {
                        gardner_lane_step(L[0], wrel, kp, lim, hs, step);
                        gardner_lane_step(L[1], wrel, kp, lim, hs, step);
                    }
                    L[0].count += (unsigned)k_min;
                    L[1].count += (unsigned)k_min;
                    gardner_lane_tail(L[0], wrel, stop, kp, lim, hs, step);
                    gardner_lane_tail(L[1], wrel, stop, kp, lim, hs, step);
                } else {
                    for (int it = 0; it < k_min; it++) gardner_lane_step(L[0], wrel, kp, lim, hs, step);
                    L[0].count += (unsigned)k_min;
                    gardner_lane_tail(L[0], wrel, stop, kp, lim, hs, step);
                }
            }
        }
        if (last_window) break;
        enter_hi = stop + step + 1.2f;
        wbase = wend - margin - back;
        if (n_alive <= 64) continue;
        __syncthreads();
#pragma unroll
        for (int l = 0; l < 2; l++) {
            const int p = tid + l * PDT_GTM_THREADS;
            if (p < n_alive) { x_ns[p] = L[l].ns; x_prev[p] = L[l].prev; x_half[p] = L[l].half; x_cnt[p] = L[l].count; }
        }
        for (int t = tid; t < PDT_GTM_HASH; t += PDT_GTM_THREADS) htab[t] = 0xffffffffu;
        __syncthreads();
        bool surv[2];
#pragma unroll
        for (int l = 0; l < 2; l++) {
            const int p = tid + l * PDT_GTM_THREADS;
            surv[l] = false;
            if (p < n_alive) {
                const unsigned a = __float_as_uint(L[l].ns), b = __float_as_uint(L[l].half), d = __float_as_uint(L[l].prev);
                unsigned h = (a * 2654435761u) ^ (b * 40503u) ^ (d * 2246822519u);
                h = (h >> 7) & (PDT_GTM_HASH - 1);
                for (;;) {
                    const unsigned old = atomicCAS(&htab[h], 0xffffffffu, (unsigned)p);
                    if (old == 0xffffffffu) { dupof[p] = (unsigned short)p; surv[l] = true; break; }
                    if (__float_as_uint(x_ns[old]) == a && __float_as_uint(x_half[old]) == b && __float_as_uint(x_prev[old]) == d) {
                        dupof[p] = (unsigned short)old;
                        break;
                    }
                    h = (h + 1) & (PDT_GTM_HASH - 1);
                }
            }
        }
        unsigned long long bal[2];
        bal[0] = __ballot(surv[0]);
        bal[1] = __ballot(surv[1]);
        if ((tid & 63) == 0) {
            s_wcnt[wave] = (unsigned)__popcll(bal[0]);
            s_wcnt[PDT_GTM_THREADS / 64 + wave] = (unsigned)__popcll(bal[1]);
        }
        __syncthreads();
#pragma unroll
        for (int l = 0; l < 2; l++) {
            const int q = tid + l * PDT_GTM_THREADS;
            if (q < n_slots) {
                const unsigned o = own[q];
                const unsigned dd = dupof[o];
                if (dd != o) {
                    extra[q] += (int)x_cnt[o] - (int)x_cnt[dd];
                    own[q] = (unsigned short)dd;
                }
            }
        }
        unsigned before[2] = {0, 0};
        unsigned total = 0;
        for (int g = 0; g < 2 * (PDT_GTM_THREADS / 64); g++) {
            const unsigned v = s_wcnt[g];
            if (g < wave) before[0] += v;
            if (g < PDT_GTM_THREADS / 64 + wave) before[1] += v;
            total += v;
        }
        const unsigned long long lt = (1ull << (tid & 63)) - 1ull;
        unsigned np[2];
        np[0] = before[0] + (unsigned)__popcll(bal[0] & lt);
        np[1] = before[1] + (unsigned)__popcll(bal[1] & lt);
#pragma unroll
        for (int l = 0; l < 2; l++)
            if (surv[l]) newidx[tid + l * PDT_GTM_THREADS] = (unsigned short)np[l];
        __syncthreads();
#pragma unroll
        for (int l = 0; l < 2; l++) {
            if (surv[l]) {
                const unsigned q = np[l];
                x_ns[q] = L[l].ns; x_prev[q] = L[l].prev; x_half[q] = L[l].half; x_q[q] = L[l].q_last;
                x_cnt[q] = L[l].count; x_il[q] = L[l].i_last;
            }
            const int q = tid + l * PDT_GTM_THREADS;
            if (q < n_slots) own[q] = newidx[own[q]];
        }
        __syncthreads();
        n_alive = (int)total;
#pragma unroll
        for (int l = 0; l < 2; l++) {
            const int p = tid + l * PDT_GTM_THREADS;
            const int src = (p < n_alive) ? p : 0;
            L[l].ns = x_ns[src]; L[l].prev = x_prev[src]; L[l].half = x_half[src]; L[l].q_last = x_q[src];
            L[l].count = x_cnt[src]; L[l].i_last = x_il[src];
        }
    }
    __syncthreads();
#pragma unroll
    for (int l = 0; l < 2; l++) {
        const int p = tid + l * PDT_GTM_THREADS;
        if (p < n_alive) { x_q[p] = L[l].q_last; x_il[p] = L[l].i_last; x_cnt[p] = L[l].count; }
    }
    __syncthreads();
#pragma unroll
    for (int l = 0; l < 2; l++) {
        const int q = tid + l * PDT_GTM_THREADS;
        if (q < n_slots) {
            const unsigned o = own[q];
            const unsigned cnt = (unsigned)((int)x_cnt[o] + extra[q]);
            const unsigned cell = gardner_encode_exit(D, x_q[o], x_il[o], cnt);
            if (cell == PDT_GTAB_MISS) atomicAdd(&stats[0], 1u);
            row[my_k[l]] = cell;
        }
    }
}

#define PDT_GSPAN_BITMAP_WORDS 8192
#define PDT_GSUB 1
#define PDT_GSUB_WIN 2048
#define PDT_GSUB_KEYS (64 / PDT_GSUB)
struct GardnerSpanRow { unsigned off, n; };
struct GardnerSpanItem { unsigned row, first, cnt; };
struct GardnerSpanRec { float ns, prev, half; unsigned count; };
struct GardnerSpanCtl { unsigned long long keys; unsigned items, cursor, overflow, pad_; };

__device__ __forceinline__ void k_gardner_span_keys(GardnerDomain D, long long n_rows, const unsigned *__restrict__ cand_k,
                                                    GardnerBand *__restrict__ bands, const unsigned *__restrict__ clist,
                                                    const unsigned *__restrict__ table, unsigned *__restrict__ keys,
                                                    unsigned cap_keys, GardnerSpanRow *__restrict__ rows,
                                                    GardnerSpanItem *__restrict__ items, GardnerSpanCtl *__restrict__ ctl)
{
    __shared__ unsigned s_bits[PDT_GSPAN_BITMAP_WORDS];
    __shared__ unsigned s_scan[256];
    __shared__ unsigned s_off, s_item;
    const long long r = blockIdx.x;
    if (r >= n_rows) return;
    const long long c0 = r * D.span;
    const GardnerBand bd = bands[r];
    const unsigned *cand = bd.listed ? (clist + (size_t)r * PDT_GTAB_LIST) : cand_k;
    const unsigned *row = table + (size_t)r * (size_t)(2 * D.n_q);
    const int tid = threadIdx.x;
    const int n_words = (2 * D.n_q + 31) >> 5;
    const unsigned kmask = (1u << D.idx_bits) - 1u;
    for (int t = tid; t < n_words; t += 256) s_bits[t] = 0u;
    __syncthreads();
    for (int j = bd.j_lo + tid; j < bd.j_hi; j += 256) {
        const unsigned cell = row[(c0 == 0) ? 0u : cand[j]];
        if (cell != PDT_GTAB_MISS) {
            const unsigned k1 = cell & kmask;
            atomicOr(&s_bits[k1 >> 5], 1u << (k1 & 31u));
        }
    }
    __syncthreads();
    const int per = (n_words + 255) / 256;
    const int w0 = tid * per, w1 = (w0 + per < n_words) ? w0 + per : n_words;
    unsigned mine = 0;
    for (int t = w0; t < w1; t++) mine += (unsigned)__popc(s_bits[t]);
    s_scan[tid] = mine;
    __syncthreads();
    for (int d = 1; d < 256; d <<= 1) {
        const unsigned v = (tid >= d) ? s_scan[tid - d] : 0u;
        __syncthreads();
        s_scan[tid] += v;
        __syncthreads();
    }
    const unsigned total = s_scan[255];
    if (tid == 0) {
        unsigned off = ~0u;
        {
            const unsigned long long got = atomicAdd(&ctl->keys, (unsigned long long)total);
            if (got + total <= (unsigned long long)cap_keys) off = (unsigned)got;
        }
        if (off == ~0u) atomicAdd(&ctl->overflow, 1u);
        else s_item = atomicAdd(&ctl->items, (total + (unsigned)PDT_GSUB_KEYS - 1u) / (unsigned)PDT_GSUB_KEYS);
        s_off = off;
    }
    __syncthreads();
    const unsigned off = s_off;
    if (off == ~0u) {
        if (tid == 0) {
            GardnerSpanRow rw;
            rw.off = 0; rw.n = ~0u;
            rows[r] = rw;
            GardnerBand nb = bd;
            nb.k_lo = 1u; nb.k_hi = 0u;
            bands[r] = nb;
        }
        return;
    }
    unsigned at = off + s_scan[tid] - mine;
    for (int t = w0; t < w1; t++) {
        unsigned bits = s_bits[t];
        while (bits) {
            const int b = __ffs((int)bits) - 1;
            bits &= bits - 1u;
            keys[at++] = ((unsigned)t << 5) + (unsigned)b;
        }
    }
    for (unsigned q = tid; q < (total + (unsigned)PDT_GSUB_KEYS - 1u) / (unsigned)PDT_GSUB_KEYS; q += 256u) {
        GardnerSpanItem it;
        it.row = (unsigned)r;
        it.first = off + (unsigned)PDT_GSUB_KEYS * q;
        it.cnt = (total - (unsigned)PDT_GSUB_KEYS * q < (unsigned)PDT_GSUB_KEYS) ? total - (unsigned)PDT_GSUB_KEYS * q : (unsigned)PDT_GSUB_KEYS;
        items[s_item + q] = it;
    }
    if (tid == 0) {
        GardnerSpanRow rw;
        rw.off = off; rw.n = total;
        rows[r] = rw;
    }
}

#define PDT_GSUB_OUT 64
template <int WIN, int NSUB, bool EMIT>
__device__ __forceinline__ void gardner_sub_chunk(float *win, const float *__restrict__ in, const GardnerParams<float> &P,
                                                  const long long (&c_sub)[NSUB], GardnerLane &L, float *__restrict__ sym,
                                                  long long *__restrict__ symidx, long long sym_at, long long sym_cap,
                                                  float *o_val = nullptr, unsigned *o_idx = nullptr )
{
    constexpr int SUBW = 64 / NSUB;
    const int lane = (int)threadIdx.x;
    const int mysub = lane / SUBW;
    float *ov = o_val + mysub * PDT_GSUB_OUT;
    unsigned *oi = o_idx + mysub * PDT_GSUB_OUT;
    int nout = 0;
    const long long C = P.chunk_out;
    const int n_cur = (int)C;
    const float hs = (float)((double)P.step / 2.0);
    const float kp = P.kp, lim = P.lim, step = P.step, nT = (float)n_cur;
    const int margin = 2 * (int)step + 24;
    const int back = (int)step + 8;
    long long my_base = 0;
#pragma unroll
    for (int u = 0; u < NSUB; u++) my_base = (mysub == u) ? c_sub[u] * C : my_base;
    int wbase = 0;
    float enter_hi = step + 1.2f;
    auto emit = [&](float cur, unsigned i_cur) {
        if (EMIT) {
            ov[nout] = cur;
            oi[nout] = i_cur;
            nout++;
        }
    };
    auto flush = [&]() {
        if (EMIT) {
            const long long k0 = sym_at + (long long)L.count - (long long)nout;
            if (L.active)
                for (int t = lane % SUBW; t < nout; t += SUBW) {
                    const long long k = k0 + t;
                    if (k < sym_cap) {
                        sym[k] = ov[t];
                        symidx[k] = my_base + (long long)oi[t];
                    }
                }
            nout = 0;
        }
    };
#pragma unroll 1
    for (;;) {
        __syncthreads();
        if (wbase + WIN <= n_cur) {
            struct __attribute__((packed, aligned(4))) Q { float v[4]; };
#pragma unroll
            for (int u = 0; u < NSUB; u++) {
                const float *src = in + c_sub[u] * C + wbase;
                float *wu = win + u * WIN;
#pragma unroll
                for (int v = 0; v < WIN / 256; v++) {
                    const int t = (v * 64 + lane) * 4;
                    const Q r = *reinterpret_cast<const Q *>(src + t);
                    *reinterpret_cast<float4 *>(wu + t) = make_float4(r.v[0], r.v[1], r.v[2], r.v[3]);
                }
            }
        } else {
#pragma unroll 1
            for (int t = lane; t < NSUB * WIN; t += 64) {
                const int u = t / WIN, tt = t - u * WIN;
                long long cu = c_sub[0];
#pragma unroll
                for (int q = 1; q < NSUB; q++) cu = (u == q) ? c_sub[q] : cu;
                const int idx = wbase + tt;
                float r = 0.0f;
                if (idx < n_cur) r = in[cu * C + idx];
                else if (idx < n_cur + margin) r = gardner_beyond(in, (const float *)nullptr, P, cu, (long long)n_cur, (long long)idx);
                win[t] = r;
            }
        }
        __syncthreads();
        const int wend = wbase + WIN;
        const bool last_window = (wend - margin >= n_cur);
        const float stop = last_window ? nT : (float)(wend - margin);
        const float *wrel = win + mysub * WIN - wbase;
        if (wbase == 0) {
            const float rn = __builtin_rintf(L.ns);
            const unsigned i_cur = (unsigned)rn;
            const unsigned i_half = (unsigned)__builtin_rintf(L.half);
            const float cur = wrel[i_cur];
            float mid;
            if (i_half < (unsigned)WIN) mid = wrel[i_half];
            else mid = (i_half < (unsigned)n_cur) ? in[my_base + i_half]
                                                  : gardner_beyond(in, (const float *)nullptr, P, my_base / C, (long long)n_cur, (long long)i_half);
            emit(cur, i_cur);
            const float err = __builtin_amdgcn_fmed3f(kp * (cur - L.prev) * mid, -lim, lim);
            L.ns = L.ns - err;
            L.q_last = L.ns;
            L.half = L.ns + hs;
            L.ns = L.ns + step;
            L.prev = cur;
            L.i_last = i_cur;
            L.count += 1;
        }
        int k_min = (int)((stop - 4.0f - enter_hi) / (step + 0.101f)) - 1;
        if (k_min < 0) k_min = 0;
#pragma unroll 4
        for (int it = 0; it < k_min; it++) {
            if (EMIT) {
                const int ic = rint_index(L.ns);
                const float cur = lds_rel_at(wrel, L.ns);
                const float mid = lds_rel_at(wrel, L.half);
                emit(cur, (unsigned)ic);
                const float err = __builtin_amdgcn_fmed3f(kp * (cur - L.prev) * mid, -lim, lim);
                L.ns = L.ns - err;
                L.half = L.ns + hs;
                L.ns = L.ns + step;
                L.prev = cur;
                L.count += 1;
            } else
                gardner_lane_step(L, wrel, kp, lim, hs, step);
        }
        if (!EMIT) L.count += (unsigned)k_min;
        for (;;) {
            const float rn = __builtin_rintf(L.ns);
            if (!(rn < stop)) break;
            const float cur = wrel[(int)rn];
            const float mid = wrel[rint_index(L.half)];
            emit(cur, (unsigned)rn);
            const float err = __builtin_amdgcn_fmed3f(kp * (cur - L.prev) * mid, -lim, lim);
            L.ns = L.ns - err;
            L.q_last = L.ns;
            L.half = L.ns + hs;
            L.ns = L.ns + step;
            L.prev = cur;
            L.i_last = (unsigned)rn;
            L.count++;
        }
        flush();
        if (last_window) break;
        enter_hi = stop + step + 1.2f;
        wbase = wend - margin - back;
    }
}


template <int WIN>
__device__ __forceinline__ void k_gardner_span_walk(const float *__restrict__ in, GardnerParams<float> P, GardnerDomain D,
                                                    const unsigned *__restrict__ keys, const GardnerSpanItem *__restrict__ items,
                                                    GardnerSpanCtl *__restrict__ ctl, unsigned *__restrict__ tails,
                                                    GardnerSpanRec *__restrict__ recs )
{
    __shared__ __attribute__((aligned(16))) float win[PDT_GSUB * WIN];
    __shared__ float s_ref[3];
    __shared__ unsigned s_next;
    const int lane = threadIdx.x;
    const int mysub = lane / PDT_GSUB_KEYS, sublane = lane % PDT_GSUB_KEYS;
    const float nT = (float)P.chunk_out;
    const unsigned n_items = ctl->items;
    for (;;) {
        __syncthreads();
        if (lane == 0) s_next = atomicAdd(&ctl->cursor, (unsigned)PDT_GSUB);
        __syncthreads();
        const unsigned q0 = s_next;
        if (q0 >= n_items) break;
        long long c_sub[PDT_GSUB];
        GardnerSpanItem mine = items[q0];
#pragma unroll
        for (int u = 0; u < PDT_GSUB; u++) {
            const GardnerSpanItem it = (q0 + (unsigned)u < n_items) ? items[q0 + u] : items[q0];
            c_sub[u] = (long long)it.row * D.span + 1;
            if (mysub == u) {
                mine = it;
                if (q0 + (unsigned)u >= n_items) mine.cnt = 0;
            }
        }
        GardnerLane L;
        L.q_last = 0; L.i_last = 0; L.count = 0; L.k = 0;
        L.active = (unsigned)sublane < mine.cnt;
        L.ns = L.prev = L.half = 0;
        long long my_c = 0;
#pragma unroll
        for (int u = 0; u < PDT_GSUB; u++) my_c = (mysub == u) ? c_sub[u] : my_c;
        if (L.active) gardner_entry_from_candidate(in, P, D, my_c, (int)keys[mine.first + sublane], L.ns, L.prev, L.half);
        if (lane == 0) { s_ref[0] = L.ns; s_ref[1] = L.prev; s_ref[2] = L.half; }
        __syncthreads();
        if (!L.active) { L.ns = s_ref[0]; L.prev = s_ref[1]; L.half = s_ref[2]; }
        for (int g = 1; g < D.span; g++) {
            long long cc[PDT_GSUB];
#pragma unroll
            for (int u = 0; u < PDT_GSUB; u++) cc[u] = c_sub[u] + (g - 1);
            if (L.active) {
                GardnerSpanRec rc;
                rc.ns = L.ns; rc.prev = L.prev; rc.half = L.half; rc.count = L.count;
                recs[(size_t)(mine.first + sublane) * (size_t)(D.span - 1) + (size_t)(g - 1)] = rc;
            }
            gardner_sub_chunk<WIN, PDT_GSUB, false>(win, in, P, cc, L, nullptr, nullptr, 0, 0);
            if (g + 1 < D.span) L.ns = L.ns - nT;
        }
        if (L.active) tails[mine.first + sublane] = gardner_encode_exit(D, L.q_last, L.i_last, L.count);
    }
}

#define PDT_GEMIT_SUB_WIN 512
template <int WIN>
__device__ __forceinline__ void k_gardner_emit_first(const float *__restrict__ in, GardnerParams<float> P, GardnerDomain D,
                                                     long long n_rows, const GardnerEntry<float> *__restrict__ entries,
                                                     const unsigned *__restrict__ keys, const GardnerSpanRow *__restrict__ rows,
                                                     const GardnerSpanRec *__restrict__ recs,
                                                     GardnerEntry<float> *__restrict__ centries, unsigned char *__restrict__ flags,
                                                     float *__restrict__ sym, long long *__restrict__ symidx, long long sym_cap,
                                                     long long g_first = 0 )
{
    __shared__ __attribute__((aligned(16))) float win[4 * WIN];
    const int lane = threadIdx.x;
    const int mysub = lane >> 4;
    const long long g0 = g_first + (long long)blockIdx.x * 4;
    if (g0 >= n_rows) return;
    long long c_sub[4];
#pragma unroll
    for (int u = 0; u < 4; u++) c_sub[u] = ((g0 + u < n_rows) ? g0 + u : g0) * D.span;
    const long long my_g = (g0 + mysub < n_rows) ? g0 + mysub : g0;
    const GardnerEntry<float> e = entries[my_g];
    GardnerLane L;
    L.ns = e.ns; L.prev = e.prev; L.half = e.half; L.q_last = 0; L.i_last = 0; L.count = 0; L.k = 0;
    L.active = g0 + mysub < n_rows;
    __shared__ float o_val[4 * PDT_GSUB_OUT];
    __shared__ unsigned o_idx[4 * PDT_GSUB_OUT];
    gardner_sub_chunk<WIN, 4, true>(win, in, P, c_sub, L, sym, symidx, e.offset, sym_cap, o_val, o_idx);
    if (L.active && (lane & 15) == 0) {
        unsigned char flag = 1;
        const GardnerSpanRow rw = rows[my_g];
        const unsigned cell = gardner_encode_exit(D, L.q_last, L.i_last, L.count);
        if (rw.n != ~0u && rw.n > 0 && cell != PDT_GTAB_MISS) {
            const unsigned k1 = cell & ((1u << D.idx_bits) - 1u);
            unsigned lo = 0, hi = rw.n;
            while (lo < hi) {
                const unsigned mid = (lo + hi) >> 1;
                if (keys[rw.off + mid] < k1) lo = mid + 1;
                else hi = mid;
            }
            if (lo < rw.n && keys[rw.off + lo] == k1) {
                const GardnerSpanRec *rc = recs + (size_t)(rw.off + lo) * (size_t)(D.span - 1);
                for (int q = 1; q < D.span; q++) {
                    GardnerEntry<float> ce;
                    ce.ns = rc[q - 1].ns; ce.prev = rc[q - 1].prev; ce.half = rc[q - 1].half;
                    ce.offset = e.offset + (long long)L.count + (long long)rc[q - 1].count;
                    centries[my_g * D.span + q] = ce;
                }
                flag = 0;
            }
        }
        flags[my_g] = flag;
    }
}

template <int WIN>
__device__ __forceinline__ void k_gardner_emit_rest(const float *__restrict__ in, GardnerParams<float> P, GardnerDomain D,
                                                    long long n_rows, const GardnerEntry<float> *__restrict__ centries,
                                                    const unsigned char *__restrict__ flags, float *__restrict__ sym,
                                                    long long *__restrict__ symidx, long long sym_cap, long long g_first = 0)
{
    __shared__ __attribute__((aligned(16))) float win[4 * WIN];
    const int lane = threadIdx.x;
    const int mysub = lane >> 4;
    const long long per = D.span - 1;
    const long long total = n_rows * per;
    const long long i0 = g_first * per + (long long)blockIdx.x * 4;
    if (i0 >= total) return;
    long long c_sub[4];
    bool live[4];
    long long c_any = -1;
#pragma unroll
    for (int u = 0; u < 4; u++) {
        const long long i = i0 + u;
        const long long g = (i < total) ? i / per : 0;
        live[u] = i < total && !flags[g];
        c_sub[u] = g * D.span + 1 + (i - g * per);
        if (live[u] && c_any < 0) c_any = c_sub[u];
    }
    if (c_any < 0) return;
#pragma unroll
    for (int u = 0; u < 4; u++) c_sub[u] = live[u] ? c_sub[u] : c_any;
    long long my_c = c_any;
    bool mine_live = false;
#pragma unroll
    for (int u = 0; u < 4; u++)
        if (mysub == u) { my_c = c_sub[u]; mine_live = live[u]; }
    const GardnerEntry<float> e = centries[my_c];
    GardnerLane L;
    L.ns = e.ns; L.prev = e.prev; L.half = e.half; L.q_last = 0; L.i_last = 0; L.count = 0; L.k = 0;
    L.active = mine_live;
    __shared__ float o_val[4 * PDT_GSUB_OUT];
    __shared__ unsigned o_idx[4 * PDT_GSUB_OUT];
    gardner_sub_chunk<WIN, 4, true>(win, in, P, c_sub, L, sym, symidx, e.offset, sym_cap, o_val, o_idx);
}

__device__ __forceinline__ void k_gardner_span_join(GardnerDomain D, long long n_rows, const unsigned *__restrict__ cand_k,
                                                    const GardnerBand *__restrict__ bands, const unsigned *__restrict__ clist,
                                                    unsigned *__restrict__ table, const unsigned *__restrict__ keys,
                                                    const unsigned *__restrict__ tails, const GardnerSpanRow *__restrict__ rows,
                                                    unsigned *__restrict__ stats )
{
    const long long r = blockIdx.x;
    if (r >= n_rows) return;
    const GardnerSpanRow rw = rows[r];
    if (rw.n == ~0u) return;
    const long long c0 = r * D.span;
    const GardnerBand bd = bands[r];
    const unsigned *cand = bd.listed ? (clist + (size_t)r * PDT_GTAB_LIST) : cand_k;
    unsigned *row = table + (size_t)r * (size_t)(2 * D.n_q);
    const unsigned kmask = (1u << D.idx_bits) - 1u;
    for (int j = bd.j_lo + (int)threadIdx.x; j < bd.j_hi; j += (int)blockDim.x) {
        const unsigned k = (c0 == 0) ? 0u : cand[j];
        const unsigned cell = row[k];
        if (cell == PDT_GTAB_MISS) continue;
        const unsigned k1 = cell & kmask;
        unsigned lo = 0, hi = rw.n;
        while (lo < hi) {
            const unsigned mid = (lo + hi) >> 1;
            if (keys[rw.off + mid] < k1) lo = mid + 1;
            else hi = mid;
        }
        unsigned out = PDT_GTAB_MISS;
        if (lo < rw.n && keys[rw.off + lo] == k1) {
            const unsigned tail = tails[rw.off + lo];
            if (tail != PDT_GTAB_MISS) {
                const unsigned cnt = (cell >> D.idx_bits) + (tail >> D.idx_bits);
                if (cnt < (1u << (32 - D.idx_bits)) - 1u) out = (tail & kmask) | (cnt << D.idx_bits);
            }
        }
        if (out == PDT_GTAB_MISS) atomicAdd(&stats[0], 1u);
        row[k] = out;
    }
}

__device__ __forceinline__ unsigned gardner_cell(const unsigned *__restrict__ table, size_t stride, const GardnerBand &b,
                                                 long long c, unsigned key)
{
    const unsigned cell = table[(size_t)c * stride + key];
    return (key >= b.k_lo && key <= b.k_hi) ? cell : PDT_GTAB_MISS;
}

struct GardnerSegCell { unsigned next, count; };
struct GardnerSegStart { unsigned key; unsigned hopped; long long offset; };

__device__ __forceinline__ void k_gardner_segmap(const unsigned *__restrict__ table, GardnerDomain D, long long n_groups,
                                                          int G, GardnerSegCell *__restrict__ segmap,
                                                          const GardnerBand *__restrict__ bands)
{
    const long long s = blockIdx.x;
    const long long c0 = s * G;
    if (c0 + G > n_groups - 1) return;
// ... 1310 lines not shown
```

project-desert-tortoise_amd/csrc/pdt_rt.h:

```cpp
#ifndef PDT_RT_H
#define PDT_RT_H
#include <hip/hip_runtime.h>
#include <math.h>
#include <stdio.h>
#include <stdlib.h>
#include <string.h>

#include <errno.h>
#include <fcntl.h>
#include <unistd.h>

#include <algorithm>
#include <functional>
#include <map>
#include <mutex>
#include <atomic>
#include <chrono>
#include <memory>
#include <new>
#include <string>
#include <thread>
#include <type_traits>
#include <vector>

// ... 74 lines not shown
struct KTimer {
    std::string name;
    hipEvent_t a, b;
    bool shared_a = false;
};

struct DevScalars {
    unsigned long long nsym;
    unsigned long long nbits;
    unsigned nhits;
    unsigned nframes;
    unsigned counters[4];
    unsigned sync_overflow;
    unsigned pad0_;
    unsigned gstats[4];
    double norm;
    long long agc_first_bad;
    PllPhaseHint phase_hint;
    PllTailList tail_list;
};

template <typename... A> struct Pack {};
template <typename H, typename... R> struct Pack<H, R...> { H h; Pack<R...> r; };
template <typename Sig> struct BodyTraits;
template <typename... P> struct BodyTraits<void (*)(P...)> { using pack = Pack<P...>; };

template <typename H> __device__ __forceinline__ H as_global(H v)
{
    if constexpr (std::is_pointer<H>::value) {
        using E = typename std::remove_pointer<H>::type;
        __attribute__((address_space(1))) E *g = (__attribute__((address_space(1))) E *)v;
        asm("" : "+s"(g));
        return (H)g;
    } else {
        return v;
    }
}
__device__ __forceinline__ IqSrc as_global(IqSrc v)
{
    v.p = as_global(v.p);
    return v;
}
template <typename T> __device__ __forceinline__ AgcParams<T> as_global(AgcParams<T> v)
{
    v.raw_out = as_global(v.raw_out);
    return v;
}

template <auto Body, typename... Done>
__device__ __forceinline__ void call_body(const Pack<> &, Done... d) { Body(d...); }
template <auto Body, typename H, typename... R, typename... Done>
__device__ __forceinline__ void call_body(const Pack<H, R...> &p, Done... d) { call_body<Body>(p.r, d..., as_global(p.h)); }

template <auto Body, int TB>
__global__ void __launch_bounds__(TB) k_run(const typename BodyTraits<decltype(Body)>::pack *__restrict__ packs)
{
    call_body<Body>(packs[blockIdx.z]);
}

template <auto Body, int TB> void go_fn(dim3 g, dim3 b, size_t sh, hipStream_t st, const void *dp)
{
    hipLaunchKernelGGL((k_run<Body, TB>), g, b, sh, st, (const typename BodyTraits<decltype(Body)>::pack *)dp);
}

inline void pack_fill(Pack<> &) {}
template <typename H, typename... R, typename A0, typename... AR> void pack_fill(Pack<H, R...> &p, A0 &&a0, AR &&...ar)
{
    p.h = (H)a0;
    pack_fill(p.r, ar...);
}

typedef void (*GoFn)(dim3, dim3, size_t, hipStream_t, const void *);
enum { OP_LAUNCH, OP_MEMSET, OP_FORK, OP_JOIN_RECORD, OP_JOIN_WAIT, OP_TBEGIN, OP_TEND, OP_TGAP, OP_D2H, OP_H2D, OP_EV0, OP_EV1 };
struct PlanOp {
    int op = OP_LAUNCH, side = 0;
    GoFn go = nullptr;
    dim3 grid, block;
    size_t shmem = 0, pack_off = 0, pack_size = 0;
    void *dst = nullptr;
    const void *src = nullptr;
    int value = 0;
    size_t bytes = 0;
    const char *name = nullptr;
};
struct Plan {
    std::vector<PlanOp> ops;
    std::vector<unsigned char> packs;
    hipStream_t side_stream = nullptr;
    void clear() { ops.clear(); packs.clear(); }
    int side_of(hipStream_t s) const { return (side_stream && s == side_stream) ? 1 : 0; }
    template <auto Body, int TB, typename... A> void launch(const char *kname, dim3 grid, dim3 block, size_t shmem, int side, A &&...args)
    {
        using PackT = typename BodyTraits<decltype(Body)>::pack;
        static_assert(std::is_trivially_copyable<PackT>::value, "kernel arguments travel as plain bytes");
        PackT pk;
        memset((void *)&pk, 0, sizeof pk);
        pack_fill(pk, args...);
        PlanOp o;
        o.op = OP_LAUNCH;
        o.name = kname;
        o.side = side;
        o.grid = grid;
        o.block = block;
        o.shmem = shmem;
        o.pack_off = (packs.size() + 15) & ~(size_t)15;
        o.pack_size = sizeof(PackT);
        static_assert(alignof(PackT) <= 16, "pack alignment");
        packs.resize(o.pack_off + o.pack_size, 0);
        memcpy(packs.data() + o.pack_off, &pk, sizeof pk);
        o.go = &go_fn<Body, TB>;
        ops.push_back(o);
    }
    void simple(int op, int side = 0, const char *name = nullptr)
    {
        PlanOp o;
        o.op = op; o.side = side; o.name = name;
        ops.push_back(o);
    }
    void memset_async(void *dst, int value, size_t bytes, int side = 0)
    {
        PlanOp o;
        o.op = OP_MEMSET; o.side = side; o.dst = dst; o.value = value; o.bytes = bytes;
        ops.push_back(o);
    }
    void copy(int op, void *dst, const void *src, size_t bytes)
    {
        PlanOp o;
        o.op = op; o.dst = dst; o.src = src; o.bytes = bytes;
        ops.push_back(o);
    }
    bool same_shape(const Plan &o) const
    {
        if (ops.size() != o.ops.size() || packs.size() != o.packs.size()) return false;
        for (size_t i = 0; i < ops.size(); i++) {
            const PlanOp &a = ops[i], &b = o.ops[i];
            if (a.op != b.op || a.side != b.side || a.go != b.go || a.block.x != b.block.x || a.block.y != b.block.y ||
                a.shmem != b.shmem || a.pack_off != b.pack_off || a.pack_size != b.pack_size)
                return false;
        }
        return true;
    }
};
#define PDT_LAUNCH(TB, KERNEL, grid, block, shmem, stream, ...) \
    PL.launch<&KERNEL, TB>(#KERNEL, grid, block, shmem, PL.side_of(stream), __VA_ARGS__)

}
using namespace pdtrt;

struct Tuning {
    double band_pad = 0.0, pll_warm_scale = 1.0, head_taus = 0.0, agc_k = 0.0, pll_warm_s = 0.0, agc_warm_s = 0.0;
    double overlap_split[8] = { 0, 0, 0, 0, 0, 0, 0, 0 };
    long long hbm_limit_mb = 0, window_piece = 0, burst_slab_rows = 0;
    int ingest_direct = -1, ingest_numa = -1;
    int scout_syms = 0, gspan = 0, gspan_cap = 0, ingest_threads = 0, ingest_span_mb = 0, ingest_streams = 0, overlap_segments = 0, overlap_min_mb = 0, fir_wg_per_cu = 0, agc_tpb = 0, gseg = 0, pll_block = 0, fix_passes = 2;
    bool fir_generic = false, mix_unfused = false, quality_inline = false, gemit_groups = false, agc_unfused = false, no_excl = false, gardner_onebuf = false, gardner_noring = false, gardner_sequential = false, seg_sequential = false, agc_lanes = false, overlap = true, debug_overlap = false, chain_one_range = false, ema_noguess = false, debug_sync = false, pll_noshort = false, pll_nockpt = false, pll_noconsensus = false, pll_notail = false, seg_plain = false, sync_block = false, gardner_nostride = false, manch_3pass = false, sync_serial = false;
    void load();
};

struct StreamCarry {
    bool active = false;
    bool final_seg = false;
    bool in_place = false;
    uint64_t place_align = 0;
    bool quality = false;
    long long first = 0;
    uint64_t origin = 0;
    bool have_norm = false;
    double norm_factor = 0, gain = 0;
    bool locked = false;
    double phase = 0, freq = 0, avg = 0, locksig = 0, sweep = 0;
    int64_t lock_sample = -1;
    double lock_freq_hz = 0, avg_at_lock = 0;
    bool have_sampler = false;
    double sa = 0, sb = 0, sc = 0;
    double sym_m2 = 0, sym_m1 = 0;
    unsigned clockmod = 0;
    uint64_t nsym_total = 0;
    std::vector<unsigned char> kept_bits;
    std::vector<long long> kept_src;
    uint64_t bit_base = 0;
    uint64_t nbits_total = 0;
    long long next_free = 0;
    bool have_pending = false;
    pdt_frame pending;
    std::vector<pdt_frame> seg_frames;
    uint64_t seg_new_symbols = 0, seg_new_bits = 0;
};

enum { IN_NONE = 0, IN_IQ, IN_REAL, IN_WB };
struct InFmt {
    int kind;
    int code;
    int bytes;
    int pcm_fmt;
    int pcm_bytes;
};
inline InFmt in_fmt(int sample_format)
{
    switch (sample_format) {
    case PDT_FMT_PCM16: return { IN_IQ, sample_format, 4, 0, 4 };
    case PDT_FMT_F32: return { IN_IQ, sample_format, 8, 1, 8 };
    case PDT_FMT_REAL_PCM16: return { IN_REAL, sample_format, 2, 1, 8 };
    case PDT_FMT_REAL_F32: return { IN_REAL, sample_format, 4, 1, 8 };
    case PDT_FMT_WB_PCM16: return { IN_WB, sample_format, 4, 1, 8 };
    case PDT_FMT_WB_F32: return { IN_WB, sample_format, 8, 1, 8 };
    case PDT_FMT_WB_CU8:
    case PDT_FMT_WB_CS8: return { IN_WB, sample_format, 2, 1, 8 };
    }
    return { IN_NONE, sample_format, 0, 0, 0 };
}

struct HaloCarry {
    DevBuf buf[2];
    int cur = 0;
    uint64_t left = 0, pending = 0, in = 0, out = 0;
};

struct IngestRes {
    void *pin = nullptr;
    size_t pin_cap = 0;
    hipStream_t copy[4] = { nullptr, nullptr, nullptr, nullptr };
    hipEvent_t all_queued[4] = { nullptr, nullptr, nullptr, nullptr };
    std::vector<hipEvent_t> slot_ev, mark_ev;
    int was_direct = 0, numa_node = -1;
    void release();
};

struct pdt_ctx {
    pdt_config cfg;
    pdt_loop_params lp = {};
    Tuning tune;
    StreamCarry sc;
    int elem;
    uint32_t interp, ntaps;
    hipStream_t stream = nullptr;
    bool own_stream = false;
    hipEvent_t ev0 = nullptr, ev1 = nullptr, ev_fork = nullptr, ev_join = nullptr;
    hipStream_t stream2 = nullptr;

    DevBuf pcm, pll, lock, fir, agc, sym, symidx, bits, bitsym, hits, frames, taps, mag, seams_pll, seams_agc, scal, lockinfo, term, seams_ema, gtable, gentries, gcand, gmfirst, stiles, gsegmap, gsegstart, gbands, gclist, gneed, gchain, gspan_keys, gspan_tails, gspan_rows, gspan_items, gspan_ctl, gspan_recs, gcentries, gflags, agc_maps, pll_head, taps_rot, pll_scratch, tip, sync_scr, agc_raw, agc_ckpt, pll_ckpt;
    bool counted = false;
    bool keep_agc_raw = false;
    bool keep_quality = false;
    bool keep_pll_asked = false;
    bool keep_pll = true;
    DevBuf avgph, term_ap, seams_q, chunkinfo;
    struct PllInject {
        bool active = false, started = false, locked = false;
        double phase = 0, freq = 0, avg = 0, locksig = 0, sweep = 0;
    } inj;
    long long last_pll_block = 0;
    void *qual_pin = nullptr;
    size_t qual_pin_cap = 0;
    uint64_t pend_chunks = 0;
    std::vector<pdt::ChunkInfo> chunk_host;
    uint64_t report_samples = 0;
    pdt_progress_fn progress_fn = nullptr;
    void *progress_user = nullptr;
    long long gcand_key = -1;
    int gardner_mode = 0;
    long long gspan_nrows = 0;
    const void *pcm_dev = nullptr;
    int pcm_fmt = 0;

    std::vector<unsigned char> taps_host;
    uint64_t n_samples = 0, n_out = 0;
    std::vector<pdt_frame> frames_host;
    std::vector<pdt_tip_frame> tip_host;
    uint32_t frames_on_device = 0;
    bool have_frames = false;
    Plan plan;
    DevBuf packs_dev;
    void *packs_pin = nullptr;
    size_t packs_pin_cap = 0;
    pdt_ctx *leader = nullptr;
    int batch_hint = 1;
    IngestRes ingest;
    double stream_gpu_ms = 0;
    double ingest_ms = 0;
    DevBuf stream_in, seg_dev, lt_theta, lt_phi;
    uint64_t stream_have = 0, stream_done = 0;
    uint64_t stream_total = 0;
    int stream_fmt = -1;
    bool stream_open = false;
    std::vector<pdt_frame> stream_new;
    uint32_t real_step = 1u << 30;
    double real_center = 0;
    DevBuf an_tab, analytic;
    int an_tab_ready = 0;
    uint64_t analytic_len = 0;
    int ch_decim = 0;
    double ch_offset = 0;
    uint32_t ch_step = 0;
    DevBuf ddc_taps, channel;
    int ddc_taps_decim = 0;
    uint64_t channel_len = 0;
    HaloCarry halo;
    DevBuf survey_win, survey_tw, survey_part, survey_out;
    int survey_tab_nfft = 0;
    std::vector<float> survey_spec;
    DevBuf bursts_rows, bursts_peaks, bursts_counts;
    int bursts_nfft = 0, bursts_rows_per = 0;
    uint64_t bursts_first = 0, bursts_nrows = 0;
    bool bursts_done = false;
    const void *bursts_src = nullptr;
    int bursts_fmt = 0;
    std::vector<pdt_row_peak> bursts_pk;
    std::vector<int> bursts_cnt;
    DevBuf win_table;
    DevBuf tone_table, tone_out;
    int tone_sum_nfft = 0;
    double tone_sw = 0, tone_sw2 = 0;
    DevBuf argos_work, argos_bits;
    bool bits_whole = false;
    std::function<double(long long)> bit_time;
    DevBuf ff_work, ff_in, ff_out;
    uint64_t ff_cap = 0;
    uint32_t ff_rate = 0;
    const void *held_src = nullptr;
    uint64_t held_frames = 0;
    int held_fmt = 0;
    void pcm_retaken()
    {
        bursts_done = bursts_done && bursts_src != pcm.p;
        if (held_src == pcm.p) held_src = nullptr;
    }
    unsigned char *seg_pin = nullptr;
    pdt_stats stats;
    std::vector<pdt_kernel_time> ktimes;
    std::vector<KTimer> timers;
    std::vector<hipEvent_t> event_pool;
    void *pinned = nullptr;
    size_t pinned_cap = 0;
    uint32_t last_nframes = 0;
    DevScalars *pend_sc = nullptr;
    unsigned char *pend_info = nullptr;
    uint32_t pend_got_frames = 0;
    uint64_t pend_n = 0;
    bool pending = false;
    uint64_t stage_len[PDT_ST_COUNT];
    TimeAxis<float> axis_f;
    TimeAxis<double> axis_d;
};

namespace pdtrt {

int ingest_capture(pdt_ctx *ctx, const IngestSrc &src, size_t bytes, void *dst, IngestJob *job = nullptr);
int ingest_wait_mark(pdt_ctx *ctx, IngestJob &job, size_t m, hipStream_t stream);
int ingest_join(IngestJob &job);
std::atomic<int> &ingest_open_contexts();
std::mutex &ingest_link(int device);

template <typename T> void make_lpf(T *h, int N, T Fc, T Fs, int interp)
{
    const T Tt = (T)(1.0 / (double)Fs);
    const T wc = (T)(2.0 * M_PI * (double)Fc * (double)Tt);
    const T tou = (T)((N - 1.0) / 2.0);
    for (int n = 0; n < N; n++) {
        const T arg = wc * ((T)n - tou);
        T sv;
        if (sizeof(T) == 4) {
            float sf, cf;
            sincosf_glibc((float)arg, sf, cf);
            sv = (T)sf;
        } else {
            sv = (T)sin_glibc((double)arg);
        }
        T hd = (T)((double)sv / (M_PI * (double)((T)n - tou)));
        if (((T)n == tou) && ((N / 2) * 2 != N)) hd = (T)((double)wc / M_PI);
        const T wn = (T)(0.42 - 0.5 * cos_glibc((2 * M_PI * n) / (N - 1)) + 0.08 * cos_glibc((4 * M_PI * n) / (N - 1)));
        h[n] = hd * wn * (T)interp;
    }
}

inline int poes_interp(uint32_t rate) { return (int)rint(150000.0 / (double)(float)rate); }

class Launcher {
  public:
    Launcher(pdt_ctx *c) : ctx(c) {}
    void begin(const char *name, hipStream_t s = nullptr)
    {
        if (!ctx->cfg.profile) return;
        KTimer t;
        t.name = name;
        cur = s ? s : ctx->stream;
        if (have_last && last_stream == cur) {
            t.a = last_b;
            t.shared_a = true;
        } else {
            t.a = take();
            t.shared_a = false;
            (void)hipEventRecord(t.a, cur);
        }
        t.b = take();
        ctx->timers.push_back(t);
        open_idx = ctx->timers.size() - 1;
        have_last = false;
    }
    void end()
    {
        if (!ctx->cfg.profile) return;
        (void)hipEventRecord(ctx->timers[open_idx].b, cur);
        last_b = ctx->timers[open_idx].b;
        last_stream = cur;
        have_last = true;
    }
    void gap() { have_last = false; }

  private:
    hipEvent_t take()
    {
        hipEvent_t e;
        if (!ctx->event_pool.empty()) { e = ctx->event_pool.back(); ctx->event_pool.pop_back(); }
        else (void)hipEventCreate(&e);
// ... 220 lines not shown
```

Before: 51740.

## Deduplicate converged Gardner span walker states mid-span and re-walk only representatives

Adds a two-stage Gardner span walk. The first stage stops at a rekey point inside the span and records each walker's state. A new rekey kernel finds walkers whose states are identical and builds a compacted list of representatives. Only those representatives walk the rest of the span in a second stage with a different sub-group width and window; a spread kernel then copies their records and tails back to the duplicates with count offsets. This aims to cut redundant sampler walking where many candidate starting states converge, at the cost of extra kernels, buffers, an atomic and an O(n^2) per-row dedup. The change also adds register prefetching of window loads in the non-emitting walker.

```diff
diff --git a/include/pdt_dev.h b/include/pdt_dev.h
--- a/include/pdt_dev.h
+++ b/include/pdt_dev.h
@@ -7,6 +7,7 @@
 int pdt_dev_set(const char *name, const char *value);
 struct pdt_ctx;
 unsigned long long pdt_dev_span_rows(const struct pdt_ctx *ctx, unsigned *n_exits_out, unsigned long long max);
+unsigned long long pdt_dev_span_rekey(const struct pdt_ctx *ctx, unsigned *out, unsigned long long max);
 int pdt_dev_ddc(int device, uint32_t in_rate, int decim, double offset_hz, int sample_format, const void *x_dev, long long lo, long long hi,
                 uint64_t n_out, uint64_t g0, void *out_dev);
 #ifdef __cplusplus
diff --git a/project-desert-tortoise_amd/__init__.py b/project-desert-tortoise_amd/__init__.py
--- a/project-desert-tortoise_amd/__init__.py
+++ b/project-desert-tortoise_amd/__init__.py
@@ -423,7 +423,7 @@
     "pdt_ff_bits", "pdt_ff_bits_batch", "pdt_ff_read", "pdt_ff_messages", "pdt_ff_messages_batch", "pdt_stage_ff_bits", "pdt_host_ff_bits",
     "pdt_host_ff_mix",
 ]
-DEV_SYMBOLS = ["pdt_dev_set", "pdt_dev_span_rows", "pdt_dev_ddc"]
+DEV_SYMBOLS = ["pdt_dev_set", "pdt_dev_span_rows", "pdt_dev_span_rekey", "pdt_dev_ddc"]
 
 _lib = None
 
diff --git a/project-desert-tortoise_amd/csrc/pdt_api.hip b/project-desert-tortoise_amd/csrc/pdt_api.hip
--- a/project-desert-tortoise_amd/csrc/pdt_api.hip
+++ b/project-desert-tortoise_amd/csrc/pdt_api.hip
@@ -67,6 +67,10 @@
     if (const char *e = get("PDT_FIX_PASSES")) fix_passes = atoi(e);
     if (const char *e = get("PDT_GSEG")) gseg = std::min(64, std::max(2, atoi(e)));
     if (const char *e = get("PDT_GSPAN")) gspan = std::min(256, std::max(1, atoi(e)));
+    if (const char *e = get("PDT_GSPAN_REKEY")) gspan_rekey = std::min(255, std::max(0, atoi(e)));
+    if (const char *e = get("PDT_GSPAN_SUB")) gspan_sub = atoi(e);
+    if (const char *e = get("PDT_GSPAN_WIN2")) gspan_win2 = atoi(e);
+    if (const char *e = get("PDT_GSPAN_FIT")) gspan_fit = std::min(64, std::max(2, atoi(e)));
     if (const char *e = get("PDT_GSPAN_CAP")) gspan_cap = std::max(64, atoi(e));
     fir_generic = get("PDT_FIR_GENERIC") != nullptr;
     mix_unfused = get("PDT_MIX_UNFUSED") != nullptr;
@@ -296,6 +300,29 @@
     return n;
 }
 
+unsigned long long pdt_dev_span_rekey(const pdt_ctx *ctx, unsigned *out, unsigned long long max)
+{
+    if (!ctx || ctx->gspan_nrows <= 0 || !ctx->gspan_rows.p) return 0;
+    const unsigned long long n = (unsigned long long)ctx->gspan_nrows, m = std::min(n, max);
+    if (out && m) {
+        const bool staged = ctx->gspan_rekey > 0 && ctx->gspan_info.p;
+        std::vector<GardnerSpanRow> rows((size_t)m);
+        std::vector<GardnerSpanRowInfo> info((size_t)m);
+        if (hipSetDevice(ctx->cfg.device) != hipSuccess ||
+            hipMemcpy(rows.data(), ctx->gspan_rows.p, (size_t)m * sizeof(GardnerSpanRow), hipMemcpyDeviceToHost) != hipSuccess ||
+            (staged && hipMemcpy(info.data(), ctx->gspan_info.p, (size_t)m * sizeof(GardnerSpanRowInfo), hipMemcpyDeviceToHost) != hipSuccess)) {
+            (void)hipGetLastError();
+            return 0;
+        }
+        for (size_t k = 0; k < (size_t)m; k++) {
+            out[3 * k] = rows[k].n;
+            out[3 * k + 1] = staged ? info[k].states : 0u;
+            out[3 * k + 2] = staged ? info[k].items : 0u;
+        }
+    }
+    return n;
+}
+
 int pdt_dev_ddc(int device, uint32_t in_rate, int decim, double offset_hz, int sample_format, const void *x_dev, long long lo, long long hi,
                 uint64_t n_out, uint64_t g0, void *out_dev)
 {
@@ -518,7 +545,7 @@
     DevBuf *bufs[] = { &ctx->pcm, &ctx->pll, &ctx->lock, &ctx->fir, &ctx->agc, &ctx->sym, &ctx->symidx, &ctx->bits, &ctx->bitsym,
                        &ctx->hits, &ctx->frames, &ctx->taps, &ctx->mag, &ctx->seams_pll, &ctx->seams_agc, &ctx->scal, &ctx->lockinfo,
                        &ctx->term, &ctx->seams_ema, &ctx->gtable, &ctx->gentries, &ctx->gcand,
-                       &ctx->gmfirst, &ctx->stiles, &ctx->gsegmap, &ctx->gsegstart, &ctx->gbands, &ctx->gclist, &ctx->gspan_keys, &ctx->gspan_tails, &ctx->gspan_rows, &ctx->gspan_items, &ctx->gspan_ctl, &ctx->gspan_recs, &ctx->gcentries, &ctx->gflags, &ctx->agc_maps, &ctx->pll_head, &ctx->taps_rot, &ctx->pll_scratch, &ctx->tip, &ctx->stream_in, &ctx->sync_scr, &ctx->agc_raw, &ctx->agc_ckpt, &ctx->pll_ckpt, &ctx->packs_dev, &ctx->seg_dev, &ctx->lt_theta, &ctx->lt_phi,
+                       &ctx->gmfirst, &ctx->stiles, &ctx->gsegmap, &ctx->gsegstart, &ctx->gbands, &ctx->gclist, &ctx->gspan_keys, &ctx->gspan_tails, &ctx->gspan_rows, &ctx->gspan_items, &ctx->gspan_ctl, &ctx->gspan_recs, &ctx->gspan_rep, &ctx->gspan_list2, &ctx->gspan_items2, &ctx->gspan_info, &ctx->gcentries, &ctx->gflags, &ctx->agc_maps, &ctx->pll_head, &ctx->taps_rot, &ctx->pll_scratch, &ctx->tip, &ctx->stream_in, &ctx->sync_scr, &ctx->agc_raw, &ctx->agc_ckpt, &ctx->pll_ckpt, &ctx->packs_dev, &ctx->seg_dev, &ctx->lt_theta, &ctx->lt_phi,
                        &ctx->avgph, &ctx->term_ap, &ctx->seams_q, &ctx->chunkinfo, &ctx->an_tab, &ctx->analytic, &ctx->halo.buf[0], &ctx->halo.buf[1],
                        &ctx->ddc_taps, &ctx->channel, &ctx->survey_win, &ctx->survey_tw, &ctx->survey_part, &ctx->survey_out,
                        &ctx->bursts_rows, &ctx->bursts_peaks, &ctx->bursts_counts, &ctx->win_table, &ctx->tone_table, &ctx->tone_out,
diff --git a/project-desert-tortoise_amd/csrc/pdt_chain.inc b/project-desert-tortoise_amd/csrc/pdt_chain.inc
--- a/project-desert-tortoise_amd/csrc/pdt_chain.inc
+++ b/project-desert-tortoise_amd/csrc/pdt_chain.inc
@@ -502,6 +502,7 @@
     bool use_mm = false;
     bool use_table = false;
     GardnerDomain GD{};
+    int span_rekey = 0, span_sub = 16, span_win2 = 1024;
     SamplerCarry<T> carry_in{};
     SegTail<T> *d_tail = nullptr;
     SamplerCarry<T> *d_carry_out = nullptr;
@@ -1103,6 +1104,7 @@
         use_mm = ctx->cfg.sampler == PDT_SAMPLER_MM;
         use_table = false;
         GD.q_min = 0; GD.u = 0; GD.n_q = 0; GD.n_cand = 0; GD.pad_q = 0; GD.idx_bits = 20; GD.span = 1;
+        span_rekey = 0;
         if constexpr (std::is_same<T, float>::value) {
             const int table_len = 1 << 22;
             const float nT = (float)chunk_out, stepf = (float)GP.step;
@@ -1128,7 +1130,12 @@
                     GD.idx_bits = idx_bits;
                     const double pad = ctx->cfg.gardner_band_pad > 0 ? ctx->cfg.gardner_band_pad : (ctx->tune.band_pad > 0 ? ctx->tune.band_pad : 1.0 / 8.0);
                     GD.pad_q = std::max(2, (int)(pad / (double)u));
-                    const int span_fit = (int)std::min(16.0, std::max(2.0, std::round(std::sqrt(138000.0 / ((double)chunk_out / (double)stepf)))));
+                    const double chunk_syms = (double)chunk_out / (double)stepf;
+                    const int rekey_rule = (int)std::min(3.0, std::round(1332.0 / chunk_syms));
+                    const int rekey_want = ctx->tune.gspan_rekey >= 0 ? ctx->tune.gspan_rekey : rekey_rule;
+                    int span_fit = rekey_want > 0 ? (int)std::min(24.0, std::max(2.0, std::round(std::sqrt(322000.0 / chunk_syms))))
+                                                  : (int)std::min(16.0, std::max(2.0, std::round(std::sqrt(138000.0 / chunk_syms))));
+                    if (ctx->tune.gspan_fit > 0) span_fit = ctx->tune.gspan_fit;
                     int span = ctx->tune.gspan > 0 ? ctx->tune.gspan : ((n_chunks - seg_c_first >= 4096 && (!seg || seg_fast)) ? span_fit : 1);
                     if (2 * n_q > 32 * PDT_GSPAN_BITMAP_WORDS || 8 * (long long)stepf + 256 >= PDT_GSUB_WIN) span = 1;
                     while (span > 1 && ((double)span * max_count >= (double)((1u << (32 - idx_bits)) - 2u) || (n_chunks - 1) / span - seg_c_first / span < 4))
@@ -1145,6 +1152,19 @@
                     }
                     if (!row_aligned(span)) span = 1;
                     GD.span = span;
+                    span_rekey = 0;
+                    span_sub = (ctx->tune.gspan_sub == 8 || ctx->tune.gspan_sub == 32) ? ctx->tune.gspan_sub : 16;
+                    span_win2 = (ctx->tune.gspan_win2 == 512 || ctx->tune.gspan_win2 == 1024 || ctx->tune.gspan_win2 == 2048)
+                                    ? ctx->tune.gspan_win2 : 1024;
+                    if (span_sub == 32) span_win2 = 2048;
+                    if (span_sub == 8 && span_win2 > 1024) span_win2 = 1024;
+                    if (span >= 3) {
+                        int a = rekey_want;
+                        if (ctx->tune.gspan_rekey < 0 && span - 1 - a < 4) a = 0;
+                        if (a >= span - 1) a = 0;
+                        if (8 * (long long)stepf + 256 >= span_win2) a = 0;
+                        span_rekey = a;
+                    }
                 }
             }
         }
@@ -1156,6 +1176,7 @@
         int rc = PDT_OK;
         (void)rc;
         ctx->gardner_mode = use_table ? 1 : 0;
+        ctx->gspan_rekey = (use_table && GD.span > 1) ? span_rekey : 0;
         ctx->gspan_nrows = (use_table && GD.span > 1 && chunk_out > 0) ? (n_out + chunk_out - 1) / chunk_out > 0 ? ((n_out + chunk_out - 1) / chunk_out - 1) / GD.span : 0 : 0;
         carry_in.a = 0; carry_in.b = 0; carry_in.c = 0; carry_in.c_first = 0; carry_in.count0 = 0;
         d_tail = seg ? (SegTail<T> *)ctx->seg_dev.p : nullptr;
@@ -1255,10 +1276,41 @@
                                        (GardnerBand *)ctx->gbands.p, (const unsigned *)ctx->gclist.p, (const unsigned *)ctx->gtable.p,
                                        (unsigned *)ctx->gspan_keys.p, cap_keys, (GardnerSpanRow *)ctx->gspan_rows.p,
                                        (GardnerSpanItem *)ctx->gspan_items.p, (GardnerSpanCtl *)ctx->gspan_ctl.p);
+                    if (span_rekey > 0) {
+                        if ((rc = ctx->gspan_rep.ensure((size_t)cap_keys * sizeof(unsigned)))) return rc;
+                        if ((rc = ctx->gspan_list2.ensure((size_t)cap_keys * sizeof(unsigned)))) return rc;
+                        if ((rc = ctx->gspan_items2.ensure(((size_t)cap_keys / (size_t)span_sub + (size_t)n_tab + 1) * sizeof(GardnerSpanItem)))) return rc;
+                        if ((rc = ctx->gspan_info.ensure((size_t)n_tab * sizeof(GardnerSpanRowInfo)))) return rc;
+                    }
                     const unsigned walkers = (unsigned)std::min<long long>(n_tab / PDT_GSUB + 64, 256ll * 16);
-                    PDT_LAUNCH(64, (k_gardner_span_walk<PDT_GSUB_WIN>), dim3(walkers), dim3(64), 0, st, (const float *)d_agc, GP, GD,
+                    PDT_LAUNCH(64, (k_gardner_span_walk<PDT_GSUB_WIN, PDT_GSUB, false>), dim3(walkers), dim3(64), 0, st, (const float *)d_agc, GP, GD,
                                        (const unsigned *)ctx->gspan_keys.p, (const GardnerSpanItem *)ctx->gspan_items.p,
-                                       (GardnerSpanCtl *)ctx->gspan_ctl.p, (unsigned *)ctx->gspan_tails.p, (GardnerSpanRec *)ctx->gspan_recs.p);
+                                       (GardnerSpanCtl *)ctx->gspan_ctl.p, (unsigned *)ctx->gspan_tails.p, (GardnerSpanRec *)ctx->gspan_recs.p,
+                                       (const GardnerSpanRow *)ctx->gspan_rows.p, (const unsigned *)nullptr, span_rekey);
+                    if (span_rekey > 0) {
+                        PDT_LAUNCH(64 * PDT_GSPAN_REKEY_ROWS, k_gardner_span_rekey, dim3((unsigned)((n_tab + PDT_GSPAN_REKEY_ROWS - 1) / PDT_GSPAN_REKEY_ROWS)), dim3(64 * PDT_GSPAN_REKEY_ROWS), 0, st, GD, n_tab, (const GardnerSpanRow *)ctx->gspan_rows.p,
+                                           (const GardnerSpanRec *)ctx->gspan_recs.p, span_rekey, (unsigned)span_sub, (unsigned *)ctx->gspan_rep.p,
+                                           (unsigned *)ctx->gspan_list2.p, (GardnerSpanItem *)ctx->gspan_items2.p, (GardnerSpanCtl *)ctx->gspan_ctl.p,
+                                           (GardnerSpanRowInfo *)ctx->gspan_info.p);
+                        const int nsub = 64 / span_sub;
+                        const long long resident = 256ll * std::max(1, (140 * 1024) / (nsub * span_win2 * 4));
+                        const unsigned walkers2 = (unsigned)std::min<long long>(2 * n_tab / nsub + 64, resident);
+#define PDT_SPAN_STAGE2(NSUB, WIN2)                                                                                                          \
+    PDT_LAUNCH(64, (k_gardner_span_walk<WIN2, NSUB, true>), dim3(walkers2), dim3(64), 0, st, (const float *)d_agc, GP, GD,                   \
+               (const unsigned *)ctx->gspan_keys.p, (const GardnerSpanItem *)ctx->gspan_items2.p, (GardnerSpanCtl *)ctx->gspan_ctl.p,        \
+               (unsigned *)ctx->gspan_tails.p, (GardnerSpanRec *)ctx->gspan_recs.p, (const GardnerSpanRow *)ctx->gspan_rows.p,               \
+               (const unsigned *)ctx->gspan_list2.p, span_rekey)
+                        if (span_sub == 8 && span_win2 == 512) PDT_SPAN_STAGE2(8, 512);
+                        else if (span_sub == 8) PDT_SPAN_STAGE2(8, 1024);
+                        else if (span_sub == 16 && span_win2 == 512) PDT_SPAN_STAGE2(4, 512);
+                        else if (span_sub == 16 && span_win2 == 1024) PDT_SPAN_STAGE2(4, 1024);
+                        else if (span_sub == 16) PDT_SPAN_STAGE2(4, 2048);
+                        else PDT_SPAN_STAGE2(2, 2048);
+#undef PDT_SPAN_STAGE2
+                        PDT_LAUNCH(64, k_gardner_span_spread, dim3((unsigned)n_tab), dim3(64), 0, st, GD, n_tab, (const GardnerSpanRow *)ctx->gspan_rows.p,
+                                           (const GardnerSpanRowInfo *)ctx->gspan_info.p, (const unsigned *)ctx->gspan_rep.p, span_rekey,
+                                           (unsigned *)ctx->gspan_tails.p, (GardnerSpanRec *)ctx->gspan_recs.p);
+                    }
                     PDT_LAUNCH(128, k_gardner_span_join, dim3((unsigned)n_tab), dim3(128), 0, st, GD, n_tab, (const unsigned *)ctx->gcand.p,
                                        (const GardnerBand *)ctx->gbands.p, (const unsigned *)ctx->gclist.p, (unsigned *)ctx->gtable.p,
                                        (const unsigned *)ctx->gspan_keys.p, (const unsigned *)ctx->gspan_tails.p,
diff --git a/project-desert-tortoise_amd/csrc/pdt_kernels_back.h b/project-desert-tortoise_amd/csrc/pdt_kernels_back.h
--- a/project-desert-tortoise_amd/csrc/pdt_kernels_back.h
+++ b/project-desert-tortoise_amd/csrc/pdt_kernels_back.h
@@ -1243,10 +1243,17 @@
 #define PDT_GSUB 1
 #define PDT_GSUB_WIN 2048
 #define PDT_GSUB_KEYS (64 / PDT_GSUB)
+#define PDT_GSPAN_REKEY_MAX 256
 struct GardnerSpanRow { unsigned off, n; };
 struct GardnerSpanItem { unsigned row, first, cnt; };
 struct GardnerSpanRec { float ns, prev, half; unsigned count; };
-struct GardnerSpanCtl { unsigned long long keys; unsigned items, cursor, overflow, pad_; };
+struct GardnerSpanCtl {
+    unsigned long long keys;
+    unsigned items, cursor, overflow, pad_;
+    unsigned long long both2;
+    unsigned cursor2, pad2_;
+};
+struct GardnerSpanRowInfo { unsigned states, items; };
 
 __device__ __forceinline__ void k_gardner_span_keys(GardnerDomain D, long long n_rows, const unsigned *__restrict__ cand_k,
                                                     GardnerBand *__restrict__ bands, const unsigned *__restrict__ clist,
@@ -1380,34 +1387,66 @@
             nout = 0;
         }
     };
+    constexpr bool PREFETCH = !EMIT;
+    struct __attribute__((packed, aligned(4))) Q { float v[4]; };
+    Q pre[PREFETCH ? NSUB : 1][PREFETCH ? WIN / 256 : 1];
+    bool have_pre = false;
 #pragma unroll 1
     for (;;) {
         __syncthreads();
         if (wbase + WIN <= n_cur) {
-            struct __attribute__((packed, aligned(4))) Q { float v[4]; };
+            if (PREFETCH) {
+                if (!have_pre) {
+#pragma unroll
+                    for (int u = 0; u < NSUB; u++)
+#pragma unroll
+                        for (int v = 0; v < WIN / 256; v++)
+                            pre[PREFETCH ? u : 0][PREFETCH ? v : 0] = *reinterpret_cast<const Q *>(in + c_sub[u] * C + wbase + (v * 64 + lane) * 4);
+                }
+                __builtin_amdgcn_sched_barrier(0);
+#pragma unroll
+                for (int u = 0; u < NSUB; u++)
+#pragma unroll
+                    for (int v = 0; v < WIN / 256; v++) {
+                        const Q r = pre[PREFETCH ? u : 0][PREFETCH ? v : 0];
+                        *reinterpret_cast<float4 *>(win + u * WIN + (v * 64 + lane) * 4) = make_float4(r.v[0], r.v[1], r.v[2], r.v[3]);
+                    }
+            } else {
+#pragma unroll
+                for (int u = 0; u < NSUB; u++) {
+                    const float *src = in + c_sub[u] * C + wbase;
+                    float *wu = win + u * WIN;
+#pragma unroll
+                    for (int v = 0; v < WIN / 256; v++) {
+                        const int t = (v * 64 + lane) * 4;
+                        const Q r = *reinterpret_cast<const Q *>(src + t);
+                        *reinterpret_cast<float4 *>(wu + t) = make_float4(r.v[0], r.v[1], r.v[2], r.v[3]);
+                    }
+                }
+            }
+        } else {
 #pragma unroll
             for (int u = 0; u < NSUB; u++) {
                 const float *src = in + c_sub[u] * C + wbase;
                 float *wu = win + u * WIN;
-#pragma unroll
-                for (int v = 0; v < WIN / 256; v++) {
-                    const int t = (v * 64 + lane) * 4;
-                    const Q r = *reinterpret_cast<const Q *>(src + t);
-                    *reinterpret_cast<float4 *>(wu + t) = make_float4(r.v[0], r.v[1], r.v[2], r.v[3]);
-                }
-            }
-        } else {
+                float r[WIN / 64];
+#pragma unroll
+                for (int v = 0; v < WIN / 64; v++) {
+                    const int t = v * 64 + lane;
+                    r[v] = (wbase + t < n_cur) ? src[t] : 0.0f;
+                }
+#pragma unroll
+                for (int v = 0; v < WIN / 64; v++) wu[v * 64 + lane] = r[v];
+            }
+            __syncthreads();
 #pragma unroll 1
-            for (int t = lane; t < NSUB * WIN; t += 64) {
-                const int u = t / WIN, tt = t - u * WIN;
+            for (int t = lane; t < NSUB * margin; t += 64) {
+                const int u = t / margin;
+                const int idx = n_cur + (t - u * margin), at = idx - wbase;
                 long long cu = c_sub[0];
 #pragma unroll
                 for (int q = 1; q < NSUB; q++) cu = (u == q) ? c_sub[q] : cu;
-                const int idx = wbase + tt;
-                float r = 0.0f;
-                if (idx < n_cur) r = in[cu * C + idx];
-                else if (idx < n_cur + margin) r = gardner_beyond(in, (const float *)nullptr, P, cu, (long long)n_cur, (long long)idx);
-                win[t] = r;
+                if (at < WIN) win[u * WIN + at] = gardner_beyond(in, (const float *)nullptr, P, cu, (long long)n_cur, (long long)idx);
             }
         }
         __syncthreads();
@@ -1415,6 +1454,17 @@
         const bool last_window = (wend - margin >= n_cur);
         const float stop = last_window ? nT : (float)(wend - margin);
         const float *wrel = win + mysub * WIN - wbase;
+        if (PREFETCH) {
+            const int nb = wend - margin - back;
+            have_pre = !last_window && nb + WIN <= n_cur;
+            if (have_pre) {
+#pragma unroll
+                for (int u = 0; u < NSUB; u++)
+#pragma unroll
+                    for (int v = 0; v < WIN / 256; v++)
+                        pre[PREFETCH ? u : 0][PREFETCH ? v : 0] = *reinterpret_cast<const Q *>(in + c_sub[u] * C + nb + (v * 64 + lane) * 4);
+            }
+        }
         if (wbase == 0) {
             const float rn = __builtin_rintf(L.ns);
             const unsigned i_cur = (unsigned)rn;
@@ -1476,29 +1526,33 @@
 }
 
 
-template <int WIN>
+template <int WIN, int NSUB, bool STAGE2>
 __device__ __forceinline__ void k_gardner_span_walk(const float *__restrict__ in, GardnerParams<float> P, GardnerDomain D,
                                                     const unsigned *__restrict__ keys, const GardnerSpanItem *__restrict__ items,
                                                     GardnerSpanCtl *__restrict__ ctl, unsigned *__restrict__ tails,
-                                                    GardnerSpanRec *__restrict__ recs )
-{
-    __shared__ __attribute__((aligned(16))) float win[PDT_GSUB * WIN];
+                                                    GardnerSpanRec *__restrict__ recs ,
+                                                    const GardnerSpanRow *__restrict__ rows, const unsigned *__restrict__ list2, int rekey)
+{
+    static_assert(STAGE2 || NSUB == 1, "stage 1 ends row by row: one row per wavefront");
+    constexpr int SUBW = 64 / NSUB;
+    __shared__ __attribute__((aligned(16))) float win[NSUB * WIN];
     __shared__ float s_ref[3];
     __shared__ unsigned s_next;
     const int lane = threadIdx.x;
-    const int mysub = lane / PDT_GSUB_KEYS, sublane = lane % PDT_GSUB_KEYS;
+    const int mysub = lane / SUBW, sublane = lane % SUBW;
     const float nT = (float)P.chunk_out;
-    const unsigned n_items = ctl->items;
+    const unsigned n_items = STAGE2 ? (unsigned)(ctl->both2 >> 32) : ctl->items;
+    unsigned *cursor = STAGE2 ? &ctl->cursor2 : &ctl->cursor;
     for (;;) {
         __syncthreads();
-        if (lane == 0) s_next = atomicAdd(&ctl->cursor, (unsigned)PDT_GSUB);
+        if (lane == 0) s_next = atomicAdd(cursor, (unsigned)NSUB);
         __syncthreads();
         const unsigned q0 = s_next;
         if (q0 >= n_items) break;
-        long long c_sub[PDT_GSUB];
+        long long c_sub[NSUB];
         GardnerSpanItem mine = items[q0];
 #pragma unroll
-        for (int u = 0; u < PDT_GSUB; u++) {
+        for (int u = 0; u < NSUB; u++) {
             const GardnerSpanItem it = (q0 + (unsigned)u < n_items) ? items[q0 + u] : items[q0];
             c_sub[u] = (long long)it.row * D.span + 1;
             if (mysub == u) {
@@ -1512,24 +1566,149 @@
         L.ns = L.prev = L.half = 0;
         long long my_c = 0;
 #pragma unroll
-        for (int u = 0; u < PDT_GSUB; u++) my_c = (mysub == u) ? c_sub[u] : my_c;
-        if (L.active) gardner_entry_from_candidate(in, P, D, my_c, (int)keys[mine.first + sublane], L.ns, L.prev, L.half);
+        for (int u = 0; u < NSUB; u++) my_c = (mysub == u) ? c_sub[u] : my_c;
+        int g_lo = 1, g_hi = D.span;
+        unsigned my_key = 0;
+        if (STAGE2) {
+            g_lo = rekey + 1;
+            if (L.active) {
+                my_key = list2[mine.first + sublane];
+                const GardnerSpanRec rc = recs[(size_t)my_key * (size_t)(D.span - 1) + (size_t)rekey];
+                L.ns = rc.ns; L.prev = rc.prev; L.half = rc.half; L.count = rc.count;
+            }
+        } else {
+            if (rekey > 0 && rows[mine.row].n <= (unsigned)PDT_GSPAN_REKEY_MAX) g_hi = rekey + 1;
+            my_key = mine.first + sublane;
+            if (L.active) gardner_entry_from_candidate(in, P, D, my_c, (int)keys[my_key], L.ns, L.prev, L.half);
+        }
         if (lane == 0) { s_ref[0] = L.ns; s_ref[1] = L.prev; s_ref[2] = L.half; }
         __syncthreads();
         if (!L.active) { L.ns = s_ref[0]; L.prev = s_ref[1]; L.half = s_ref[2]; }
-        for (int g = 1; g < D.span; g++) {
-            long long cc[PDT_GSUB];
-#pragma unroll
-            for (int u = 0; u < PDT_GSUB; u++) cc[u] = c_sub[u] + (g - 1);
+        GardnerSpanRec *my_recs = recs + (size_t)my_key * (size_t)(D.span - 1);
+        for (int g = g_lo; g < g_hi; g++) {
+            long long cc[NSUB];
+#pragma unroll
+            for (int u = 0; u < NSUB; u++) cc[u] = c_sub[u] + (g - 1);
             if (L.active) {
                 GardnerSpanRec rc;
                 rc.ns = L.ns; rc.prev = L.prev; rc.half = L.half; rc.count = L.count;
-                recs[(size_t)(mine.first + sublane) * (size_t)(D.span - 1) + (size_t)(g - 1)] = rc;
-            }
-            gardner_sub_chunk<WIN, PDT_GSUB, false>(win, in, P, cc, L, nullptr, nullptr, 0, 0);
+                my_recs[g - 1] = rc;
+            }
+            gardner_sub_chunk<WIN, NSUB, false>(win, in, P, cc, L, nullptr, nullptr, 0, 0);
             if (g + 1 < D.span) L.ns = L.ns - nT;
         }
-        if (L.active) tails[mine.first + sublane] = gardner_encode_exit(D, L.q_last, L.i_last, L.count);
+        if (L.active) {
+            if (g_hi < D.span) {
+                GardnerSpanRec rc;
+                rc.ns = L.ns; rc.prev = L.prev; rc.half = L.half; rc.count = L.count;
+                my_recs[g_hi - 1] = rc;
+            } else
+                tails[my_key] = gardner_encode_exit(D, L.q_last, L.i_last, L.count);
+        }
+    }
+}
+
+#define PDT_GSPAN_REKEY_ROWS 4
+__device__ __forceinline__ void k_gardner_span_rekey(GardnerDomain D, long long n_rows, const GardnerSpanRow *__restrict__ rows,
+                                                     const GardnerSpanRec *__restrict__ recs, int rekey, unsigned subw,
+                                                     unsigned *__restrict__ rep, unsigned *__restrict__ list2,
+                                                     GardnerSpanItem *__restrict__ items2, GardnerSpanCtl *__restrict__ ctl,
+                                                     GardnerSpanRowInfo *__restrict__ info)
+{
+    __shared__ unsigned s_state[PDT_GSPAN_REKEY_ROWS][3][PDT_GSPAN_REKEY_MAX];
+    __shared__ unsigned s_jj[PDT_GSPAN_REKEY_ROWS][PDT_GSPAN_REKEY_MAX], s_rk[PDT_GSPAN_REKEY_ROWS][PDT_GSPAN_REKEY_MAX];
+    __shared__ unsigned s_cnt[PDT_GSPAN_REKEY_ROWS][2];
+    __shared__ unsigned long long s_got;
+    const int lane = threadIdx.x & 63, w = threadIdx.x >> 6;
+    const long long r = (long long)blockIdx.x * PDT_GSPAN_REKEY_ROWS + w;
+    GardnerSpanRow rw;
+    rw.off = 0; rw.n = 0;
+    if (r < n_rows) rw = rows[r];
+    const bool staged = rw.n != ~0u && rw.n != 0u && rw.n <= (unsigned)PDT_GSPAN_REKEY_MAX;
+    const int n = staged ? (int)rw.n : 0;
+    unsigned *s_ns = s_state[w][0], *s_prev = s_state[w][1], *s_half = s_state[w][2], *s_j = s_jj[w], *s_rank = s_rk[w];
+    for (int i = lane; i < n; i += 64) {
+        const GardnerSpanRec rc = recs[(size_t)(rw.off + (unsigned)i) * (size_t)(D.span - 1) + (size_t)rekey];
+        s_ns[i] = __float_as_uint(rc.ns); s_prev[i] = __float_as_uint(rc.prev); s_half[i] = __float_as_uint(rc.half);
+    }
+    __syncthreads();
+    unsigned total = 0;
+    for (int i0 = 0; i0 < n; i0 += 64) {
+        const int i = i0 + lane;
+        const bool valid = i < n;
+        const int ii = valid ? i : 0;
+        const unsigned a = s_ns[ii], b = s_prev[ii], c = s_half[ii];
+        int j = ii;
+        const int j_end = (i0 + 64 < n) ? i0 + 64 : n;
+        for (int jj = 0; jj < j_end; jj++)
+            if (jj < j && s_ns[jj] == a && s_prev[jj] == b && s_half[jj] == c) j = jj;
+        const bool is_rep = valid && j == i;
+        const unsigned long long m = __ballot(is_rep);
+        if (valid) {
+            s_j[i] = (unsigned)j;
+            s_rank[i] = total + (unsigned)__popcll(m & ((1ull << lane) - 1ull));
+        }
+        total += (unsigned)__popcll(m);
+    }
+    const unsigned n_it = (total + subw - 1u) / subw;
+    if (lane == 0) {
+        s_cnt[w][0] = total; s_cnt[w][1] = n_it;
+        if (r < n_rows) {
+            GardnerSpanRowInfo ri;
+            ri.states = total; ri.items = n_it;
+            info[r] = ri;
+        }
+    }
+    __syncthreads();
+    if (threadIdx.x == 0) {
+        unsigned st = 0, it = 0;
+        for (int q = 0; q < PDT_GSPAN_REKEY_ROWS; q++) { st += s_cnt[q][0]; it += s_cnt[q][1]; }
+        s_got = (st | it) ? atomicAdd(&ctl->both2, (unsigned long long)st | ((unsigned long long)it << 32)) : 0ull;
+    }
+    __syncthreads();
+    unsigned base = (unsigned)s_got, ibase = (unsigned)(s_got >> 32);
+    for (int q = 0; q < w; q++) { base += s_cnt[q][0]; ibase += s_cnt[q][1]; }
+    for (int i = lane; i < n; i += 64) {
+        const unsigned j = s_j[i];
+        rep[rw.off + (unsigned)i] = rw.off + j;
+        if (j == (unsigned)i) list2[base + s_rank[i]] = rw.off + (unsigned)i;
+    }
+    for (unsigned q = lane; q < n_it; q += 64u) {
+        GardnerSpanItem it;
+        it.row = (unsigned)r;
+        it.first = base + subw * q;
+        it.cnt = (total - subw * q < subw) ? total - subw * q : subw;
+        items2[ibase + q] = it;
+    }
+}
+
+__device__ __forceinline__ void k_gardner_span_spread(GardnerDomain D, long long n_rows, const GardnerSpanRow *__restrict__ rows,
+                                                      const GardnerSpanRowInfo *__restrict__ info, const unsigned *__restrict__ rep,
+                                                      int rekey, unsigned *__restrict__ tails, GardnerSpanRec *__restrict__ recs)
+{
+    const long long r = blockIdx.x;
+    if (r >= n_rows) return;
+    if (info[r].states == 0u) return;
+    const GardnerSpanRow rw = rows[r];
+    const size_t per = (size_t)(D.span - 1);
+    for (unsigned i = threadIdx.x; i < rw.n; i += blockDim.x) {
+        const unsigned k = rw.off + i, rp = rep[k];
+        if (rp == k) continue;
+        GardnerSpanRec *mine = recs + (size_t)k * per;
+        const GardnerSpanRec *from = recs + (size_t)rp * per;
+        const unsigned diff = mine[rekey].count - from[rekey].count;
+        for (int g = rekey + 1; g < D.span - 1; g++) {
+            GardnerSpanRec rc = from[g];
+            rc.count += diff;
+            mine[g] = rc;
+        }
+        const unsigned tail = tails[rp];
+        unsigned out = PDT_GTAB_MISS;
+        if (tail != PDT_GTAB_MISS) {
+            const unsigned cnt = (tail >> D.idx_bits) + diff;
+            if (cnt > 0u && cnt < (1u << (32 - D.idx_bits)) - 1u) out = (tail & ((1u << D.idx_bits) - 1u)) | (cnt << D.idx_bits);
+        }
+        tails[k] = out;
     }
 }
 
diff --git a/project-desert-tortoise_amd/csrc/pdt_rt.h b/project-desert-tortoise_amd/csrc/pdt_rt.h
--- a/project-desert-tortoise_amd/csrc/pdt_rt.h
+++ b/project-desert-tortoise_amd/csrc/pdt_rt.h
@@ -250,7 +250,7 @@
     double overlap_split[8] = { 0, 0, 0, 0, 0, 0, 0, 0 };
     long long hbm_limit_mb = 0, window_piece = 0, burst_slab_rows = 0;
     int ingest_direct = -1, ingest_numa = -1;
-    int scout_syms = 0, gspan = 0, gspan_cap = 0, ingest_threads = 0, ingest_span_mb = 0, ingest_streams = 0, overlap_segments = 0, overlap_min_mb = 0, fir_wg_per_cu = 0, agc_tpb = 0, gseg = 0, pll_block = 0, fix_passes = 2;
+    int scout_syms = 0, gspan = 0, gspan_cap = 0, gspan_rekey = -1 , gspan_sub = 0, gspan_win2 = 0, gspan_fit = 0, ingest_threads = 0, ingest_span_mb = 0, ingest_streams = 0, overlap_segments = 0, overlap_min_mb = 0, fir_wg_per_cu = 0, agc_tpb = 0, gseg = 0, pll_block = 0, fix_passes = 2;
     bool fir_generic = false, mix_unfused = false, quality_inline = false, gemit_groups = false, agc_unfused = false, no_excl = false, gardner_onebuf = false, gardner_noring = false, gardner_sequential = false, seg_sequential = false, agc_lanes = false, overlap = true, debug_overlap = false, chain_one_range = false, ema_noguess = false, debug_sync = false, pll_noshort = false, pll_nockpt = false, pll_noconsensus = false, pll_notail = false, seg_plain = false, sync_block = false, gardner_nostride = false, manch_3pass = false, sync_serial = false;
     void load();
 };
@@ -336,7 +336,7 @@
     hipEvent_t ev0 = nullptr, ev1 = nullptr, ev_fork = nullptr, ev_join = nullptr;
     hipStream_t stream2 = nullptr;
 
-    DevBuf pcm, pll, lock, fir, agc, sym, symidx, bits, bitsym, hits, frames, taps, mag, seams_pll, seams_agc, scal, lockinfo, term, seams_ema, gtable, gentries, gcand, gmfirst, stiles, gsegmap, gsegstart, gbands, gclist, gneed, gchain, gspan_keys, gspan_tails, gspan_rows, gspan_items, gspan_ctl, gspan_recs, gcentries, gflags, agc_maps, pll_head, taps_rot, pll_scratch, tip, sync_scr, agc_raw, agc_ckpt, pll_ckpt;
+    DevBuf pcm, pll, lock, fir, agc, sym, symidx, bits, bitsym, hits, frames, taps, mag, seams_pll, seams_agc, scal, lockinfo, term, seams_ema, gtable, gentries, gcand, gmfirst, stiles, gsegmap, gsegstart, gbands, gclist, gneed, gchain, gspan_keys, gspan_tails, gspan_rows, gspan_items, gspan_ctl, gspan_recs, gspan_rep, gspan_list2, gspan_items2, gspan_info, gcentries, gflags, agc_maps, pll_head, taps_rot, pll_scratch, tip, sync_scr, agc_raw, agc_ckpt, pll_ckpt;
     bool counted = false;
     bool keep_agc_raw = false;
     bool keep_quality = false;
@@ -358,6 +358,7 @@
     long long gcand_key = -1;
     int gardner_mode = 0;
     long long gspan_nrows = 0;
+    int gspan_rekey = 0;
     const void *pcm_dev = nullptr;
     int pcm_fmt = 0;
 
```

New measurement: 54180, median of 6. 1.05x the previous value.
